# mhw32/multimodal-vae-public

Measured on AMD Instinct MI355X. Metric: images/sec (MVAE train step), higher is better.
Workload: dtype f32; 1 GPU; mnist MVAE train step, n-latents 64, batch 512 per GPU; global_batch=512, parallelism=dp1, launch=hipGraph replay

## Files before the change

### include/mvae_hip.h

```cpp
#ifndef MVAE_HIP_H
#define MVAE_HIP_H

#include <stddef.h>
#include <stdint.h>

#ifdef __cplusplus
extern "C" {
#endif

#define MVAE_OK          0
#define MVAE_ERR_ARG    (-1)
#define MVAE_ERR_LAUNCH (-2)
#define MVAE_ERR_WS     (-3)
#define MVAE_ERR_COMM   (-4)

#define MVAE_ACT_SWISH   1
#define MVAE_ACCUMULATE  2

#define MVAE_POE_VARIANT_A 0
#define MVAE_POE_VARIANT_B 1
#define MVAE_POE_NO_PRIOR  4
#define MVAE_MAX_EXPERTS  32

typedef void *mvae_stream_t;

int mvae_abi_version(void);
size_t mvae_gemm_ws_bytes(int rows_out, int cols_out, int reduce_len);
int mvae_linear_fwd(const float *x, int ldx, const float *w, const float *bias,
                    float *pre, float *act, int ldy,
                    const float *mask, float mask_scale,
                    int M, int N, int K, void *ws, size_t ws_bytes, mvae_stream_t stream);
int mvae_linear_dgrad(const float *dy, int lddy, const float *w,
                      float *dx, int lddx,
                      const float *pre_in, const float *mask, float mask_scale,
                      int M, int N, int K, int flags, void *ws, size_t ws_bytes,
                      mvae_stream_t stream);
int mvae_linear_wgrad(const float *dy, int lddy, const float *x, int ldx,
                      float *dw, float *db, int M, int N, int K, int flags,
                      void *ws, size_t ws_bytes, mvae_stream_t stream);

#define MVAE_WGRAD_BATCH_MAX 16
typedef struct {
    const float *dy; int lddy;
    const float *x; int ldx;
    float *dw;
    float *db;
    int M, N, K;
    int flags;
} mvae_wgrad_item;
int mvae_linear_wgrad_batched(const mvae_wgrad_item *items, int n_items, mvae_stream_t stream);

typedef struct {
    const float *grad_base;
    float *param_base;
    float *exp_avg_base;
    float *exp_avg_sq_base;
    const float *coef2;
    double beta1, beta2, eps;
    float grad_scale;
} mvae_adam_fuse;
int mvae_linear_wgrad_batched_adam(const mvae_wgrad_item *items, int n_items, const mvae_adam_fuse *adam,
                                   mvae_stream_t stream);

int mvae_linear_fwd_grouped(const float *x, int ldx, size_t x_gs, const float *w, size_t w_gs,
                            const float *bias, size_t bias_gs, float *pre, float *act, int ldy,
                            size_t y_gs, int G, int M, int N, int K, void *ws, size_t ws_bytes,
                            mvae_stream_t stream);
int mvae_linear_dgrad_grouped(const float *dy, int lddy, size_t dy_gs, const float *w, size_t w_gs,
                              float *dx, int lddx, size_t dx_gs, const float *pre_in, size_t pre_gs,
                              int G, int M, int N, int K, int flags, void *ws, size_t ws_bytes,
                              mvae_stream_t stream);
int mvae_linear_wgrad_grouped(const float *dy, int lddy, size_t dy_gs, const float *x, int ldx,
                              size_t x_gs, float *dw, size_t dw_gs, float *db, size_t db_gs, int G,
                              int M, int N, int K, int flags, void *ws, size_t ws_bytes,
                              mvae_stream_t stream);

int mvae_conv2d_k4_fwd(const float *x, const float *w, float *pre, float *act,
                       int B, int Cin, int H, int W, int Cout, int stride, int pad,
                       mvae_stream_t stream);
int mvae_conv2d_k4_dgrad(const float *dy, const float *w, float *dx, const float *pre_in,
                         int B, int Cin, int H, int W, int Cout, int stride, int pad,
                         void *ws, size_t ws_bytes, mvae_stream_t stream);
int mvae_conv2d_k4_wgrad(const float *dy, const float *x, float *dw,
                         int B, int Cin, int H, int W, int Cout, int stride, int pad,
                         int flags, void *ws, size_t ws_bytes, mvae_stream_t stream);
int mvae_convT2d_k4_fwd(const float *x, const float *w, float *pre, float *act,
                        int B, int Cin, int H, int W, int Cout, int stride, int pad,
                        void *ws, size_t ws_bytes, mvae_stream_t stream);
int mvae_convT2d_k4_dgrad(const float *dy, const float *w, float *dx, const float *pre_in,
                          int B, int Cin, int H, int W, int Cout, int stride, int pad,
                          mvae_stream_t stream);
int mvae_convT2d_k4_wgrad(const float *dy, const float *x, float *dw,
                          int B, int Cin, int H, int W, int Cout, int stride, int pad,
                          int flags, void *ws, size_t ws_bytes, mvae_stream_t stream);

typedef struct {
    const float *w; float *wr;
    int transposed, Cin, Cout, stride, pad;
} mvae_repack_item;
size_t mvae_conv_k4_repack_floats(int transposed, const float *w, int B, int Cin, int H, int W, int Cout,
                                  int stride, int pad);
int mvae_conv_k4_repack_batched(const mvae_repack_item *items, int n_items, mvae_stream_t stream);

#define MVAE_STATS_TILE_ELEMS 512
size_t mvae_convT2d_k4_stats_tiles(int B, int Cin, int H, int W, int Cout, int stride, int pad);
int mvae_convT2d_k4_fwd_stats(const float *x, const float *w, float *part, size_t part_floats,
                              int B, int Cin, int H, int W, int Cout, int stride, int pad,
                              void *ws, size_t ws_bytes, mvae_stream_t stream);

size_t mvae_bn_ws_bytes(int G, int C, int n_per_group);
int mvae_bn_train_fwd(const float *x, const float *gamma, const float *beta, float *y,
                      float *save_mean, float *save_invstd,
                      float *running_mean, float *running_var,
                      int G, int B, int C, int HW, float eps, float momentum,
                      int n_updates, const int *n_updates_dev ,
                      int flags, void *ws, size_t ws_bytes, mvae_stream_t stream);
int mvae_bn_train_bwd(const float *dy, const float *x, const float *gamma, const float *beta,
                      const float *save_mean, const float *save_invstd,
                      float *dx, float *dgamma, float *dbeta,
                      int G, int B, int C, int HW, int flags,
                      void *ws, size_t ws_bytes, mvae_stream_t stream);
int mvae_bn_stats_merge(const float *part, int tiles, int elems_per_tile, int G, int C,
                        float *save_mean, float *save_invstd, float *running_mean, float *running_var,
                        float eps, float momentum, int n_updates, const int *n_updates_dev, mvae_stream_t stream);
int mvae_bn_eval_fwd(const float *x, const float *gamma, const float *beta, float *y,
                     const float *running_mean, const float *running_var,
                     int N, int C, int HW, float eps, int flags, mvae_stream_t stream);

int mvae_swish_fwd(const float *x, float *y, size_t n, mvae_stream_t stream);
int mvae_swish_bwd(const float *dy, const float *x, float *dx, size_t n, mvae_stream_t stream);
int mvae_sigmoid_fwd(const float *x, float *y, size_t n, mvae_stream_t stream);
int mvae_affine_fwd(const float *x, const float *scale, const float *shift, float *y, size_t n, size_t period,
                    mvae_stream_t stream);
int mvae_embedding_swish_fwd(const void *idx, int idx_is_float, const float *w, float *act,
                             int R, int n_classes, int width, mvae_stream_t stream);
int mvae_embedding_swish_bwd(const void *idx, int idx_is_float, const float *w,
                             const float *dact, float *dw,
                             int R, int n_classes, int width, int flags, mvae_stream_t stream);
int mvae_embedding_swish_fwd_grouped(const void *idx, int idx_is_float, size_t idx_gs, const float *w,
                                     size_t w_gs, float *act, size_t act_gs, int G, int R,
                                     int n_classes, int width, mvae_stream_t stream);
int mvae_embedding_swish_bwd_grouped(const void *idx, int idx_is_float, size_t idx_gs, const float *w,
                                     size_t w_gs, const float *dact, size_t dact_gs, float *dw, int G,
                                     int R, int n_classes, int width, int flags, mvae_stream_t stream);

typedef struct {
    const float *mu[MVAE_MAX_EXPERTS];
    const float *logvar[MVAE_MAX_EXPERTS];
} mvae_experts_t;
typedef struct {
    float *dmu[MVAE_MAX_EXPERTS];
    float *dlogvar[MVAE_MAX_EXPERTS];
} mvae_expert_grads_t;

int mvae_poe_fwd(const mvae_experts_t *experts, int ld, int E,
                 const uint32_t *masks_dev, int T,
                 const float *noise, float *mu, float *logvar, float *z, float *kl,
                 int B, int D, int variant, mvae_stream_t stream);
int mvae_poe_fwd_draw(const mvae_experts_t *experts, int ld, int E,
                      const uint32_t *masks_dev, int T,
                      float *noise_out, uint64_t seed, const uint64_t *counter_dev, uint64_t counter_offset,
                      float *mu, float *logvar, float *z, float *kl,
                      int B, int D, int variant, mvae_stream_t stream);
int mvae_poe_bwd(const mvae_experts_t *experts, int ld, int E,
                 const uint32_t *masks_dev, int T,
                 const float *noise, const float *mu, const float *logvar,
                 const float *dz, const float *dmu, const float *dlogvar,
                 const float *dkl, int dkl_per_term ,
                 const mvae_expert_grads_t *grads, int ldg,
                 int B, int D, int variant, mvae_stream_t stream);

int mvae_poe_bwd_split(const mvae_experts_t *experts, int ld, int E,
                       const uint32_t *masks_dev, int T,
                       const float *noise, const float *mu, const float *logvar,
                       const float *dz_a, const int *slot_a, const float *dz_b, const int *slot_b,
                       const float *dkl, int dkl_per_term,
                       const mvae_expert_grads_t *grads, int ldg,
                       int B, int D, int variant, mvae_stream_t stream);

int mvae_reparam_fwd(const float *mu, const float *logvar, const float *eps, float *z, size_t n,
                     mvae_stream_t stream);
int mvae_reparam_bwd(const float *dz, const float *logvar, const float *eps,
                     float *dmu, float *dlogvar, size_t n, mvae_stream_t stream);

int mvae_kl_rows_fwd(const float *mu, const float *logvar, float *kl, int B, int D,
                     mvae_stream_t stream);
int mvae_kl_rows_bwd(const float *mu, const float *logvar, const float *dkl,
                     float *dmu, float *dlogvar, int B, int D, mvae_stream_t stream);

int mvae_bce_rowsum_fwd(const float *logits, const float *target, const float *colw,
                        float *rowsum, const float *drow_dev, float *dlogits ,
                        int R, int P, int rows_per_group, int target_rows,
                        int target_div, int target_row_stride, int target_col_stride,
                        mvae_stream_t stream);
int mvae_bce_rowsum_bwd(const float *logits, const float *target, const float *colw,
                        const float *drow_dev, float *dlogits,
                        int R, int P, int rows_per_group, int target_rows,
                        int target_div, int target_row_stride, int target_col_stride,
                        mvae_stream_t stream);
int mvae_ce_fwd(const float *logits, const int64_t *label, float *row,
                const float *drow_dev, float *dlogits ,
                int R, int K, int rows_per_group, int label_rows, mvae_stream_t stream);
int mvae_ce_bwd(const float *logits, const int64_t *label, const float *drow_dev,
                float *dlogits, int R, int K, int rows_per_group, int label_rows,
                mvae_stream_t stream);
int mvae_linear_bce_fwd(const float *x, int ldx, const float *w, const float *bias, const float *target,
                        int target_rows, int target_row_stride, const float *drow_dev, int rows_per_group,
                        float *dlogits, int ldy, float *logits, float *partial, int M, int N, int K,
                        mvae_stream_t stream);
int mvae_linear_ce_fwd(const float *x, int ldx, const float *w, const float *bias, const int64_t *label,
                       int label_rows, const float *drow_dev, int rows_per_group, float *dlogits, int ldy,
                       float *logits, float *row, int M, int N, int K, mvae_stream_t stream);
#define MVAE_ELBO_MAX_PARTS 4
#define MVAE_ELBO_MAX_TERMS 40
typedef struct {
    const float *rows;
    const float *coef;
    const int *term_of;
    int first_term, groups, rows_per_group;
} mvae_elbo_part;
int mvae_elbo_reduce(const mvae_elbo_part *parts, int n_parts, float *elbo, int T, float *zero, size_t zero_n,
                     uint64_t *counter_dev, uint64_t counter_inc, mvae_stream_t stream);
int mvae_group_sums(const float *rows, const float *coef_dev, float *out, float *total_out,
                    int G, int rows_per_group, int flags, mvae_stream_t stream);

int mvae_randn(float *out, size_t n, uint64_t seed, uint64_t *counter_dev, mvae_stream_t stream);
int mvae_bernoulli(float *out, size_t n, float keep_prob, uint64_t seed, uint64_t *counter_dev,
                   mvae_stream_t stream);
int mvae_philox_fill(float *out, size_t n, int bernoulli, float keep_prob, uint64_t seed,
                     const uint64_t *counter_dev, uint64_t counter_offset, mvae_stream_t stream);
int mvae_adam_step(float *param, const float *grad, float *exp_avg, float *exp_avg_sq,
                   size_t n, double lr, double beta1, double beta2, double eps, float grad_scale,
                   int64_t *step_dev, mvae_stream_t stream);
int mvae_adam_apply(float *param, const float *grad, float *exp_avg, float *exp_avg_sq,
                    size_t n, double lr, double beta1, double beta2, double eps, float grad_scale,
                    const int64_t *step_dev, mvae_stream_t stream);
int mvae_adam_apply_at(float *param, const float *grad, float *exp_avg, float *exp_avg_sq,
                       size_t n, double lr, double beta1, double beta2, double eps, float grad_scale,
                       const int64_t *step_dev, int64_t step_add, mvae_stream_t stream);
int mvae_adam_prepare(int64_t *step_dev, int64_t delta, double lr, double beta1, double beta2, float *coef2,
                      mvae_stream_t stream);
int mvae_counter_add(int64_t *counter_dev, int64_t delta, mvae_stream_t stream);
int mvae_adam_apply_coef(float *param, const float *grad, float *exp_avg, float *exp_avg_sq, size_t n,
                         const float *coef2, double beta1, double beta2, double eps, float grad_scale,
                         mvae_stream_t stream);

int mvae_trace_marker(int tag, mvae_stream_t stream);
int mvae_fill(float *out, size_t n, float value, mvae_stream_t stream);
int mvae_ingest(const float *image_src, float *image_dst, size_t image_floats,
                const void *label_src, void *label_dst, size_t label_bytes,
                const void *table_src_host, void *table_dst, size_t table_bytes, mvae_stream_t stream);

int mvae_block_gather(const float *src, const int *idx_dev, float *dst, int n_dst, size_t block_elems,
                      mvae_stream_t stream);
int mvae_block_scatter_add(const float *src, const int *idx_dev, float *dst, int n_src, int n_dst,
                           size_t block_elems, mvae_stream_t stream);
int mvae_scatter_sums(const float *vals, const float *coef_dev, const int *idx_dev, float *out,
                      float *total_out, int n, int flags, mvae_stream_t stream);

int mvae_dropout_fanout_fwd(const float *h, const float *masks, float *out, float scale,
                            int G, int B, int N, mvae_stream_t stream);
int mvae_dropout_fanin_bwd(const float *dout, const float *masks, float *dh, float scale,
                           int G, int B, int N, mvae_stream_t stream);
int mvae_bce_elem_fwd(const float *logits, const float *target, float *out, size_t n,
                      mvae_stream_t stream);
int mvae_bce_elem_bwd(const float *logits, const float *target, const float *g,
                      float *dlogits, float *dtarget, size_t n, mvae_stream_t stream);

int mvae_resample_ksize(int in_size, int out_size);
int mvae_resample_coeffs(int in_size, int out_size, int *kk_host, int *bounds_host);
int mvae_resize_crop_u8_to_f32(const uint8_t *src, float *dst, int B, int H, int W, int out_h,
                               int out_w, int S, int crop_top, int crop_left, const int *kx_dev,
                               const int *bx_dev, int ksx, const int *ky_dev, const int *by_dev,
                               int ksy, int y0, int y1, mvae_stream_t stream);
int mvae_u8_to_f32(const uint8_t *src, float *dst, size_t n, mvae_stream_t stream);

int mvae_gru_cell_fwd(const float *gi, int ldgi, const float *gh, int ldgh, const float *h_prev, int ldh,
                      float *h_new, int ldo, float *gates , int B, int H, mvae_stream_t stream);
int mvae_gru_cell_bwd(const float *dh_new, int lddh, const float *dh_extra , int ldde,
                      const float *gates, const float *h_prev, int ldh, float *dgi, float *dgh, float *dh_prev,
                      int B, int H, mvae_stream_t stream);
int mvae_embedding_fwd(const int64_t *idx, int idx_stride, const float *w, float *out, int ldo, int R,
                       int n_classes, int width, int flags, mvae_stream_t stream);
int mvae_embedding_bwd(const int64_t *idx, int idx_stride, const float *w, const float *dout, int ldd, float *dw,
                       int R, int n_classes, int width, int flags, mvae_stream_t stream);
int mvae_copy2d(const float *src, int lds, float *dst, int ldd, const float *mask , int ldm,
                float scale, int rows, int cols, int flags, mvae_stream_t stream);
int mvae_argmax_rows(const float *x, int ldx, int64_t *out, int R, int K, mvae_stream_t stream);

#define MVAE_COMM_ID_BYTES 128
typedef struct mvae_comm mvae_comm_t;
int mvae_comm_use_library(const char *librccl_path);
int mvae_comm_rccl_version(void);
int mvae_comm_unique_id(void *id_out, size_t id_bytes);
int mvae_comm_init(mvae_comm_t **comm, const void *id, size_t id_bytes, int rank, int world, int device);
int mvae_comm_rank(const mvae_comm_t *comm);
int mvae_comm_world(const mvae_comm_t *comm);
const char *mvae_comm_last_error(const mvae_comm_t *comm);
int mvae_comm_broadcast(mvae_comm_t *comm, void *buf, size_t bytes, int root, mvae_stream_t stream);
int mvae_comm_allreduce_async(mvae_comm_t *comm, float *buf, size_t count, mvae_stream_t stream, int *ticket);
int mvae_comm_wait(mvae_comm_t *comm, int ticket , mvae_stream_t stream);
int mvae_comm_async_error(mvae_comm_t *comm);
int mvae_comm_synchronize(mvae_comm_t *comm, mvae_stream_t stream, int timeout_ms);
int mvae_comm_destroy(mvae_comm_t *comm);

#ifdef MVAE_TUNING
void mvae_debug_set_tiling(int wm, int wn, int splits);
void mvae_debug_set_kwaves(int kw);
void mvae_debug_set_small(int off, int waves);
void mvae_debug_set_split_target(long blocks);
void mvae_debug_set_knockout(int mode);
#endif

#ifdef __cplusplus
}
#endif
#endif
```

### multimodal-vae-public_amd/_lib.py

```python
import ctypes
import os
from ctypes import c_double, c_float, c_int, c_size_t, c_uint64, c_void_p

_HERE = os.path.dirname(os.path.abspath(__file__))
LIB_PATH = os.path.join(_HERE, 'libmvae_hip.so')

MVAE_OK = 0
ERRORS = {-1: 'MVAE_ERR_ARG (bad shape / null pointer / unsupported stride)',
          -2: 'MVAE_ERR_LAUNCH (hip kernel launch failed)',
          -3: 'MVAE_ERR_WS (workspace too small)',
          -4: 'MVAE_ERR_COMM (RCCL not loadable, or an RCCL / HIP runtime call of mvae_comm_* failed)'}
COMM_ID_BYTES = 128
ACT_SWISH = 1
ACCUMULATE = 2
POE_NO_PRIOR = 4
POE_VARIANT = {'A': 0, 'B': 1, 'A-noprior': 0 | POE_NO_PRIOR, 'B-noprior': 1 | POE_NO_PRIOR}
MAX_EXPERTS = 32
STATS_TILE_ELEMS = 512
MAX_TERMS = 40


class Experts(ctypes.Structure):
    _fields_ = [('mu', c_void_p * MAX_EXPERTS), ('logvar', c_void_p * MAX_EXPERTS)]


class ElboPart(ctypes.Structure):
    _fields_ = [('rows', c_void_p), ('coef', c_void_p), ('term_of', c_void_p), ('first_term', c_int),
                ('groups', c_int), ('rows_per_group', c_int)]


ELBO_MAX_PARTS = 4


class WgradItem(ctypes.Structure):
    _fields_ = [('dy', c_void_p), ('lddy', c_int), ('x', c_void_p), ('ldx', c_int), ('dw', c_void_p),
                ('db', c_void_p), ('M', c_int), ('N', c_int), ('K', c_int), ('flags', c_int)]


WGRAD_BATCH_MAX = 16


class AdamFuse(ctypes.Structure):
    _fields_ = [('grad_base', c_void_p), ('param_base', c_void_p), ('exp_avg_base', c_void_p),
                ('exp_avg_sq_base', c_void_p), ('coef2', c_void_p), ('beta1', ctypes.c_double),
                ('beta2', ctypes.c_double), ('eps', ctypes.c_double), ('grad_scale', ctypes.c_float)]


class RepackItem(ctypes.Structure):
    _fields_ = [('w', c_void_p), ('wr', c_void_p), ('transposed', c_int), ('Cin', c_int), ('Cout', c_int),
                ('stride', c_int), ('pad', c_int)]


REPACK_MAX = 16


class ExpertGrads(ctypes.Structure):
    _fields_ = [('dmu', c_void_p * MAX_EXPERTS), ('dlogvar', c_void_p * MAX_EXPERTS)]


P = c_void_p
_SIGNATURES = {
    'mvae_abi_version': (c_int, []),
    'mvae_gemm_ws_bytes': (c_size_t, [c_int, c_int, c_int]),
    'mvae_linear_fwd': (c_int, [P, c_int, P, P, P, P, c_int, P, c_float, c_int, c_int, c_int, P, c_size_t, P]),
    'mvae_linear_bce_fwd': (c_int, [P, c_int, P, P, P, c_int, c_int, P, c_int, P, c_int, P, P, c_int, c_int, c_int, P]),
    'mvae_linear_ce_fwd': (c_int, [P, c_int, P, P, P, c_int, P, c_int, P, c_int, P, P, c_int, c_int, c_int, P]),
    'mvae_linear_dgrad': (c_int, [P, c_int, P, P, c_int, P, P, c_float, c_int, c_int, c_int, c_int, P, c_size_t, P]),
    'mvae_linear_wgrad': (c_int, [P, c_int, P, c_int, P, P, c_int, c_int, c_int, c_int, P, c_size_t, P]),
    'mvae_linear_fwd_grouped': (c_int, [P, c_int, c_size_t, P, c_size_t, P, c_size_t, P, P, c_int, c_size_t,
                                        c_int, c_int, c_int, c_int, P, c_size_t, P]),
    'mvae_linear_dgrad_grouped': (c_int, [P, c_int, c_size_t, P, c_size_t, P, c_int, c_size_t, P, c_size_t,
                                          c_int, c_int, c_int, c_int, c_int, P, c_size_t, P]),
    'mvae_linear_wgrad_grouped': (c_int, [P, c_int, c_size_t, P, c_int, c_size_t, P, c_size_t, P, c_size_t,
                                          c_int, c_int, c_int, c_int, c_int, P, c_size_t, P]),
    'mvae_conv2d_k4_fwd': (c_int, [P, P, P, P] + [c_int] * 7 + [P]),
    'mvae_conv2d_k4_dgrad': (c_int, [P, P, P, P] + [c_int] * 7 + [P, c_size_t, P]),
    'mvae_conv2d_k4_wgrad': (c_int, [P, P, P] + [c_int] * 8 + [P, c_size_t, P]),
    'mvae_convT2d_k4_fwd': (c_int, [P, P, P, P] + [c_int] * 7 + [P, c_size_t, P]),
    'mvae_convT2d_k4_dgrad': (c_int, [P, P, P, P] + [c_int] * 7 + [P]),
    'mvae_convT2d_k4_wgrad': (c_int, [P, P, P] + [c_int] * 8 + [P, c_size_t, P]),
    'mvae_bn_ws_bytes': (c_size_t, [c_int, c_int, c_int]),
    'mvae_bn_train_fwd': (c_int, [P] * 8 + [c_int] * 4 + [c_float, c_float, c_int, P, c_int, P, c_size_t, P]),
    'mvae_bn_train_bwd': (c_int, [P] * 9 + [c_int] * 5 + [P, c_size_t, P]),
    'mvae_bn_eval_fwd': (c_int, [P] * 6 + [c_int] * 3 + [c_float, c_int, P]),
    'mvae_swish_fwd': (c_int, [P, P, c_size_t, P]),
    'mvae_swish_bwd': (c_int, [P, P, P, c_size_t, P]),
    'mvae_sigmoid_fwd': (c_int, [P, P, c_size_t, P]),
    'mvae_affine_fwd': (c_int, [P, P, P, P, c_size_t, c_size_t, P]),
    'mvae_embedding_swish_fwd': (c_int, [P, c_int, P, P, c_int, c_int, c_int, P]),
    'mvae_embedding_swish_bwd': (c_int, [P, c_int, P, P, P, c_int, c_int, c_int, c_int, P]),
    'mvae_embedding_swish_fwd_grouped': (c_int, [P, c_int, c_size_t, P, c_size_t, P, c_size_t, c_int, c_int, c_int,
                                                 c_int, P]),
    'mvae_embedding_swish_bwd_grouped': (c_int, [P, c_int, c_size_t, P, c_size_t, P, c_size_t, P, c_int, c_int,
                                                 c_int, c_int, c_int, P]),
    'mvae_resample_ksize': (c_int, [c_int, c_int]),
    'mvae_resample_coeffs': (c_int, [c_int, c_int, P, P]),
    'mvae_resize_crop_u8_to_f32': (c_int, [P, P] + [c_int] * 8 + [P, P, c_int, P, P, c_int, c_int, c_int, P]),
    'mvae_u8_to_f32': (c_int, [P, P, c_size_t, P]),
    'mvae_poe_fwd': (c_int, [ctypes.POINTER(Experts), c_int, c_int, P, c_int, P, P, P, P, P,
                             c_int, c_int, c_int, P]),
    'mvae_poe_fwd_draw': (c_int, [ctypes.POINTER(Experts), c_int, c_int, P, c_int, P, c_uint64, P, c_uint64, P, P, P, P,
                                  c_int, c_int, c_int, P]),
    'mvae_poe_bwd': (c_int, [ctypes.POINTER(Experts), c_int, c_int, P, c_int, P, P, P, P, P, P, P, c_int,
                             ctypes.POINTER(ExpertGrads), c_int, c_int, c_int, c_int, P]),
    'mvae_poe_bwd_split': (c_int, [ctypes.POINTER(Experts), c_int, c_int, P, c_int, P, P, P, P,
                                   ctypes.POINTER(c_int), P, ctypes.POINTER(c_int), P, c_int,
                                   ctypes.POINTER(ExpertGrads), c_int, c_int, c_int, c_int, P]),
    'mvae_kl_rows_fwd': (c_int, [P, P, P, c_int, c_int, P]),
    'mvae_kl_rows_bwd': (c_int, [P, P, P, P, P, c_int, c_int, P]),
    'mvae_bce_rowsum_fwd': (c_int, [P, P, P, P, P, P] + [c_int] * 7 + [P]),
    'mvae_bce_rowsum_bwd': (c_int, [P, P, P, P, P] + [c_int] * 7 + [P]),
    'mvae_ce_fwd': (c_int, [P, P, P, P, P, c_int, c_int, c_int, c_int, P]),
    'mvae_ce_bwd': (c_int, [P, P, P, P, c_int, c_int, c_int, c_int, P]),
    'mvae_group_sums': (c_int, [P, P, P, P, c_int, c_int, c_int, P]),
    'mvae_conv_k4_repack_floats': (c_size_t, [c_int, P, c_int, c_int, c_int, c_int, c_int, c_int, c_int]),
    'mvae_conv_k4_repack_batched': (c_int, [ctypes.POINTER(RepackItem), c_int, P]),
    'mvae_convT2d_k4_stats_tiles': (c_size_t, [c_int] * 7),
    'mvae_convT2d_k4_fwd_stats': (c_int, [P, P, P, c_size_t] + [c_int] * 7 + [P, c_size_t, P]),
    'mvae_bn_stats_merge': (c_int, [P, c_int, c_int, c_int, c_int, P, P, P, P, c_float, c_float, c_int, P, P]),
    'mvae_linear_wgrad_batched': (c_int, [ctypes.POINTER(WgradItem), c_int, P]),
    'mvae_linear_wgrad_batched_adam': (c_int, [ctypes.POINTER(WgradItem), c_int, ctypes.POINTER(AdamFuse), P]),
    'mvae_adam_prepare': (c_int, [P, ctypes.c_int64, c_double, c_double, c_double, P, P]),
    'mvae_elbo_reduce': (c_int, [ctypes.POINTER(ElboPart), c_int, P, c_int, P, c_size_t, P, c_uint64, P]),
    'mvae_philox_fill': (c_int, [P, c_size_t, c_int, c_float, c_uint64, P, c_uint64, P]),
    'mvae_randn': (c_int, [P, c_size_t, c_uint64, P, P]),
    'mvae_bernoulli': (c_int, [P, c_size_t, c_float, c_uint64, P, P]),
    'mvae_adam_step': (c_int, [P, P, P, P, c_size_t, c_double, c_double, c_double, c_double, c_float, P, P]),
    'mvae_adam_apply': (c_int, [P, P, P, P, c_size_t, c_double, c_double, c_double, c_double, c_float, P, P]),
    'mvae_adam_apply_at': (c_int, [P, P, P, P, c_size_t, c_double, c_double, c_double, c_double, c_float, P,
                                   ctypes.c_int64, P]),
    'mvae_adam_apply_coef': (c_int, [P, P, P, P, c_size_t, P, c_double, c_double, c_double, c_float, P]),
    'mvae_counter_add': (c_int, [P, ctypes.c_int64, P]),
    'mvae_trace_marker': (c_int, [c_int, P]),
    'mvae_fill': (c_int, [P, c_size_t, c_float, P]),
    'mvae_ingest': (c_int, [P, P, c_size_t, P, P, c_size_t, P, P, c_size_t, P]),
    'mvae_reparam_fwd': (c_int, [P, P, P, P, c_size_t, P]),
    'mvae_reparam_bwd': (c_int, [P, P, P, P, P, c_size_t, P]),
    'mvae_dropout_fanout_fwd': (c_int, [P, P, P, c_float, c_int, c_int, c_int, P]),
    'mvae_dropout_fanin_bwd': (c_int, [P, P, P, c_float, c_int, c_int, c_int, P]),
    'mvae_block_gather': (c_int, [P, P, P, c_int, c_size_t, P]),
    'mvae_block_scatter_add': (c_int, [P, P, P, c_int, c_int, c_size_t, P]),
    'mvae_scatter_sums': (c_int, [P, P, P, P, P, c_int, c_int, P]),
    'mvae_bce_elem_fwd': (c_int, [P, P, P, c_size_t, P]),
    'mvae_bce_elem_bwd': (c_int, [P, P, P, P, P, c_size_t, P]),
    'mvae_gru_cell_fwd': (c_int, [P, c_int, P, c_int, P, c_int, P, c_int, P, c_int, c_int, P]),
    'mvae_gru_cell_bwd': (c_int, [P, c_int, P, c_int, P, P, c_int, P, P, P, c_int, c_int, P]),
    'mvae_embedding_fwd': (c_int, [P, c_int, P, P, c_int, c_int, c_int, c_int, c_int, P]),
    'mvae_embedding_bwd': (c_int, [P, c_int, P, P, c_int, P, c_int, c_int, c_int, c_int, P]),
    'mvae_copy2d': (c_int, [P, c_int, P, c_int, P, c_int, c_float, c_int, c_int, c_int, P]),
    'mvae_argmax_rows': (c_int, [P, c_int, P, c_int, c_int, P]),
    'mvae_comm_use_library': (c_int, [ctypes.c_char_p]),
    'mvae_comm_rccl_version': (c_int, []),
    'mvae_comm_unique_id': (c_int, [P, c_size_t]),
    'mvae_comm_init': (c_int, [ctypes.POINTER(P), P, c_size_t, c_int, c_int, c_int]),
    'mvae_comm_rank': (c_int, [P]),
    'mvae_comm_world': (c_int, [P]),
    'mvae_comm_last_error': (ctypes.c_char_p, [P]),
    'mvae_comm_broadcast': (c_int, [P, P, c_size_t, c_int, P]),
    'mvae_comm_allreduce_async': (c_int, [P, P, c_size_t, P, ctypes.POINTER(c_int)]),
    'mvae_comm_wait': (c_int, [P, c_int, P]),
    'mvae_comm_async_error': (c_int, [P]),
    'mvae_comm_synchronize': (c_int, [P, P, c_int]),
    'mvae_comm_destroy': (c_int, [P]),
}

_TUNING_SIGNATURES = {
    'mvae_debug_set_tiling': (None, [c_int, c_int, c_int]),
    'mvae_debug_set_kwaves': (None, [c_int]),
    'mvae_debug_set_small': (None, [c_int, c_int]),
    'mvae_debug_set_split_target': (None, [ctypes.c_long]),
    'mvae_debug_set_knockout': (None, [c_int]),
}
TUNING_LIB_PATH = os.path.join(_HERE, 'libmvae_hip_tuning.so')

_lib = None


def exported_symbols():
    return sorted(_SIGNATURES)


def lib():
    global _lib
    if _lib is None:
        path = os.environ.get('MVAE_HIP_LIB') or LIB_PATH
        if not os.path.exists(path):
            raise RuntimeError(
                'libmvae_hip.so is not built (%s missing): run `make -C %s/csrc`; there is no '
                'CPU fallback for the MVAE HIP path.' % (path, _HERE))
        handle = ctypes.CDLL(path)
        for name, (res, args) in _SIGNATURES.items():
            fn = getattr(handle, name)
            fn.restype = res
            fn.argtypes = args
        for name, (res, args) in _TUNING_SIGNATURES.items():
            fn = getattr(handle, name, None)
            if fn is not None:
                fn.restype = res
                fn.argtypes = args
        if handle.mvae_abi_version() != 6:
            raise RuntimeError('libmvae_hip.so ABI version mismatch')
        _lib = handle
    return _lib


def check(rc, what):
    if rc != MVAE_OK:
        raise RuntimeError('%s failed: %s' % (what, ERRORS.get(rc, 'error %d' % rc)))
```

### multimodal-vae-public_amd/csrc/poe.hip

```cpp
#include "common.h"
#include "philox.h"

namespace {

constexpr int POE_THREADS = 128;
constexpr int POE_MAX_TERMS = 40;
constexpr float POE_EPS = 1e-8f;

struct PoeArgs {
    mvae_experts_t ex;
    int ld, E, T, B, D, variant;
    int no_prior;
    int chunk;
    uint64_t seed; const uint64_t *counter; uint64_t counter_offset; int draw;
};

__device__ __forceinline__ float poe_precision(float lv, int variant) {
    float var = expf(lv) + POE_EPS;
    if (variant == MVAE_POE_VARIANT_A) var = var + POE_EPS;
    return 1.0f / var;
}

__global__ __launch_bounds__(POE_THREADS) void poe_fwd_kernel(PoeArgs a, const uint32_t *masks,
                                                              float *noise, float *mu, float *logvar,
                                                              float *z, float *kl) {
    extern __shared__ float lds[];
    const int lane = threadIdx.x & 63;
    const int b = blockIdx.x * (POE_THREADS / 64) + (threadIdx.x >> 6);
    if (b >= a.B) return;
    float *mine = lds + threadIdx.x;
    float *klacc = lds + (size_t)a.E * 2 * POE_THREADS + threadIdx.x;
    const float t0 = a.no_prior ? 0.f : poe_precision(0.f, a.variant);
    const int t_lo = blockIdx.y * a.chunk, t_hi = min(a.T, t_lo + a.chunk);
    uint32_t used = 0;
    for (int t = t_lo; t < t_hi; ++t) { klacc[(t - t_lo) * POE_THREADS] = 0.f; used |= masks[t]; }
    const uint64_t launch = a.draw ? *a.counter + a.counter_offset : 0;
    for (int d = lane; d < a.D; d += 64) {
        const size_t oe = (size_t)b * a.ld + d;
        for (int e = 0; e < a.E; ++e) {
            if (!((used >> e) & 1u)) continue;
            const float te = poe_precision(a.ex.logvar[e][oe], a.variant);
            mine[(e * 2 + 0) * POE_THREADS] = te;
            mine[(e * 2 + 1) * POE_THREADS] = a.ex.mu[e][oe] * te;
        }
        for (int t = t_lo; t < t_hi; ++t) {
            uint32_t mask = masks[t];
            float sum_t = t0, sum_mt = 0.f * t0;
            for (int e = 0; mask; ++e, mask >>= 1) {
                if (!(mask & 1u)) continue;
                sum_mt += mine[(e * 2 + 1) * POE_THREADS];
                sum_t += mine[(e * 2 + 0) * POE_THREADS];
            }
            const float pmu = sum_mt / sum_t;
            const float pvar = 1.0f / sum_t;
            const float plv = (a.variant == MVAE_POE_VARIANT_A) ? logf(pvar + POE_EPS) : logf(pvar);
            const size_t o = ((size_t)t * a.B + b) * a.D + d;
            mu[o] = pmu;
            logvar[o] = plv;
            if (a.draw) {
                const float eps = philox_normal_at(o, launch, a.seed);
                noise[o] = eps;
                z[o] = eps * expf(0.5f * plv) + pmu;
            } else if (z) {
                z[o] = noise ? noise[o] * expf(0.5f * plv) + pmu : pmu;
            }
            klacc[(t - t_lo) * POE_THREADS] += 1.0f + plv - pmu * pmu - expf(plv);
        }
    }
    if (kl) {
        for (int t = t_lo; t < t_hi; ++t) {
            const float s = wave_sum(klacc[(t - t_lo) * POE_THREADS]);
            if (lane == 0) kl[(size_t)t * a.B + b] = -0.5f * s;
        }
    }
}

struct PoeDzMap { signed char slot_a[MVAE_ELBO_MAX_TERMS], slot_b[MVAE_ELBO_MAX_TERMS]; };

__global__ __launch_bounds__(POE_THREADS) void poe_bwd_kernel(PoeArgs a, const uint32_t *masks,
                                                              const float *noise, const float *mu,
                                                              const float *logvar, const float *dz,
                                                              const float *dz_b, PoeDzMap dzm,
                                                              const float *dmu, const float *dlogvar,
                                                              const float *dkl, int dkl_stride,
                                                              mvae_expert_grads_t gr, int ldg) {
    extern __shared__ float lds[];
    const int lane = threadIdx.x & 63;
    const int b = blockIdx.x * (POE_THREADS / 64) + (threadIdx.x >> 6);
    if (b >= a.B) return;
    float *mine = lds + threadIdx.x;
    const int e_lo = blockIdx.y * a.chunk, e_hi = min(a.E, e_lo + a.chunk);
    const uint32_t own = (e_hi - e_lo >= 32 ? 0xffffffffu : ((1u << (e_hi - e_lo)) - 1u)) << e_lo;
    for (int d = lane; d < a.D; d += 64) {
        for (int t = 0; t < a.T; ++t) {
            if (!(masks[t] & own)) continue;
            const size_t o = ((size_t)t * a.B + b) * a.D + d;
            const float pmu = mu[o], plv = logvar[o];
            float gmu = dmu ? dmu[o] : 0.f;
            float glv = dlogvar ? dlogvar[o] : 0.f;
            if (dz) {
                float g;
                if (dz_b) {
                    const int sa = dzm.slot_a[t], sb = dzm.slot_b[t];
                    g = sa >= 0 ? dz[((size_t)sa * a.B + b) * a.D + d] : 0.f;
                    if (sb >= 0) g += dz_b[((size_t)sb * a.B + b) * a.D + d];
                } else {
                    g = dz[o];
                }
                gmu += g;
                if (noise) glv += g * noise[o] * 0.5f * expf(0.5f * plv);
            }
            if (dkl) {
                const float ks = dkl_stride ? dkl[(size_t)t * dkl_stride + b] : dkl[t];
                gmu += ks * pmu;
                glv += ks * (-0.5f) * (1.0f - expf(plv));
            }
            float s, dlv_ds;
            if (a.variant == MVAE_POE_VARIANT_A) {
                const float v = expf(plv) - POE_EPS;
                s = 1.0f / v;
                dlv_ds = -(v * v) / (v + POE_EPS);
            } else {
                s = expf(-plv);
                dlv_ds = -1.0f / s;
            }
            mine[(t * 3 + 0) * POE_THREADS] = gmu / s;
            mine[(t * 3 + 1) * POE_THREADS] = glv * dlv_ds;
            mine[(t * 3 + 2) * POE_THREADS] = pmu;
        }
        for (int e = e_lo; e < e_hi; ++e) {
            const size_t o = (size_t)b * a.ld + d;
            const float me = a.ex.mu[e][o], lve = a.ex.logvar[e][o];
            const float ex = expf(lve);
            const float te = poe_precision(lve, a.variant);
            float gm = 0.f, gt = 0.f;
            bool any = false;
            for (int t = 0; t < a.T; ++t) {
                if (!((masks[t] >> e) & 1u)) continue;
                any = true;
                const float at = mine[(t * 3 + 0) * POE_THREADS];
                gm += at * te;
                gt += at * (me - mine[(t * 3 + 2) * POE_THREADS]) + mine[(t * 3 + 1) * POE_THREADS];
            }
            const size_t og = (size_t)b * ldg + d;
            gr.dmu[e][og] = any ? gm : 0.f;
            gr.dlogvar[e][og] = any ? gt * (-(te * te) * ex) : 0.f;
        }
    }
}

__global__ __launch_bounds__(POE_THREADS) void kl_rows_fwd_kernel(const float *mu, const float *logvar, float *kl,
                                                                  int B, int D) {
    const int lane = threadIdx.x & 63;
    const int b = blockIdx.x * (POE_THREADS / 64) + (threadIdx.x >> 6);
    if (b >= B) return;
    float s = 0.f;
    for (int d = lane; d < D; d += 64) {
        const float m = mu[(size_t)b * D + d], lv = logvar[(size_t)b * D + d];
        s += 1.0f + lv - m * m - expf(lv);
    }
    s = wave_sum(s);
    if (lane == 0) kl[b] = -0.5f * s;
}

__global__ __launch_bounds__(256) void kl_rows_bwd_kernel(const float *mu, const float *logvar, const float *dkl,
                                                          float *dmu, float *dlogvar, int B, int D) {
    const size_t n = (size_t)B * D;
    for (size_t i = (size_t)blockIdx.x * 256 + threadIdx.x; i < n; i += (size_t)gridDim.x * 256) {
        const float g = dkl[i / D];
        dmu[i] = g * mu[i];
        dlogvar[i] = g * (-0.5f) * (1.0f - expf(logvar[i]));
    }
}

#ifndef MVAE_POE_CHUNK
#define MVAE_POE_CHUNK 3
#endif
#ifndef MVAE_POE_CHUNK_SMALL
#define MVAE_POE_CHUNK_SMALL 1
#endif
inline int poe_chunk(int n) {
    if (n <= 0) return 1;
    if (n <= 4) return MVAE_POE_CHUNK_SMALL > 0 ? MVAE_POE_CHUNK_SMALL : n;
    return MVAE_POE_CHUNK <= 0 ? n : MVAE_POE_CHUNK;
}

inline bool poe_args_ok(const mvae_experts_t *ex, int ld, int E, int T, int B, int D, int variant) {
    if (!ex || E < 0 || E > MVAE_MAX_EXPERTS || T <= 0 || T > POE_MAX_TERMS || B <= 0 || D <= 0 || ld < D)
        return false;
    const int base = variant & ~MVAE_POE_NO_PRIOR;
    if (base != MVAE_POE_VARIANT_A && base != MVAE_POE_VARIANT_B) return false;
    if ((variant & MVAE_POE_NO_PRIOR) && E < 1) return false;
    for (int e = 0; e < E; ++e)
        if (!ex->mu[e] || !ex->logvar[e]) return false;
    return true;
}

}

MVAE_EXPORT int mvae_poe_fwd(const mvae_experts_t *experts, int ld, int E, const uint32_t *masks_dev, int T,
                             const float *noise, float *mu, float *logvar, float *z, float *kl, int B, int D,
                             int variant, mvae_stream_t stream) {
    if (!poe_args_ok(experts, ld, E, T, B, D, variant) || !masks_dev || !mu || !logvar) return MVAE_ERR_ARG;
    PoeArgs a;
    a.ex = *experts; a.ld = ld; a.E = E; a.T = T; a.B = B; a.D = D;
    a.variant = variant & ~MVAE_POE_NO_PRIOR; a.no_prior = (variant & MVAE_POE_NO_PRIOR) ? 1 : 0;
    a.seed = 0; a.counter = nullptr; a.counter_offset = 0; a.draw = 0;
    const int rows = POE_THREADS / 64;
    a.chunk = poe_chunk(T);
    const size_t lds_bytes = ((size_t)E * 2 + a.chunk) * POE_THREADS * sizeof(float);
    hipLaunchKernelGGL(poe_fwd_kernel, dim3((B + rows - 1) / rows, (T + a.chunk - 1) / a.chunk), dim3(POE_THREADS), lds_bytes, (hipStream_t)stream, a,
                       masks_dev, const_cast<float *>(noise), mu, logvar, z, kl);
    return mvae_launch_status();
}

MVAE_EXPORT int mvae_poe_fwd_draw(const mvae_experts_t *experts, int ld, int E, const uint32_t *masks_dev, int T,
                                  float *noise_out, uint64_t seed, const uint64_t *counter_dev,
                                  uint64_t counter_offset, float *mu, float *logvar, float *z, float *kl, int B,
                                  int D, int variant, mvae_stream_t stream) {
    if (!poe_args_ok(experts, ld, E, T, B, D, variant) || !masks_dev || !mu || !logvar || !z || !noise_out ||
        !counter_dev)
        return MVAE_ERR_ARG;
    PoeArgs a;
    a.ex = *experts; a.ld = ld; a.E = E; a.T = T; a.B = B; a.D = D;
    a.variant = variant & ~MVAE_POE_NO_PRIOR; a.no_prior = (variant & MVAE_POE_NO_PRIOR) ? 1 : 0;
    a.seed = seed; a.counter = counter_dev; a.counter_offset = counter_offset; a.draw = 1;
    const int rows = POE_THREADS / 64;
    a.chunk = poe_chunk(T);
    const size_t lds_bytes = ((size_t)E * 2 + a.chunk) * POE_THREADS * sizeof(float);
    hipLaunchKernelGGL(poe_fwd_kernel, dim3((B + rows - 1) / rows, (T + a.chunk - 1) / a.chunk), dim3(POE_THREADS), lds_bytes, (hipStream_t)stream, a,
                       masks_dev, noise_out, mu, logvar, z, kl);
    return mvae_launch_status();
}

MVAE_EXPORT int mvae_poe_bwd(const mvae_experts_t *experts, int ld, int E, const uint32_t *masks_dev, int T,
                             const float *noise, const float *mu, const float *logvar, const float *dz,
                             const float *dmu, const float *dlogvar, const float *dkl, int dkl_per_term,
                             const mvae_expert_grads_t *grads, int ldg, int B, int D, int variant,
                             mvae_stream_t stream) {
    const int dkl_stride = dkl_per_term ? 0 : B;
    if (!poe_args_ok(experts, ld, E, T, B, D, variant) || !masks_dev || !mu || !logvar || !grads || ldg < D)
        return MVAE_ERR_ARG;
    for (int e = 0; e < E; ++e)
        if (!grads->dmu[e] || !grads->dlogvar[e]) return MVAE_ERR_ARG;
    PoeArgs a;
    a.ex = *experts; a.ld = ld; a.E = E; a.T = T; a.B = B; a.D = D;
    a.variant = variant & ~MVAE_POE_NO_PRIOR; a.no_prior = (variant & MVAE_POE_NO_PRIOR) ? 1 : 0;
    a.seed = 0; a.counter = nullptr; a.counter_offset = 0; a.draw = 0;
    const int rows = POE_THREADS / 64;
    const size_t lds_bytes = (size_t)T * 3 * POE_THREADS * sizeof(float);
    PoeDzMap none = {};
    a.chunk = poe_chunk(E);
    hipLaunchKernelGGL(poe_bwd_kernel, dim3((B + rows - 1) / rows, E ? (E + a.chunk - 1) / a.chunk : 1), dim3(POE_THREADS), lds_bytes,
                       (hipStream_t)stream, a, masks_dev, noise, mu, logvar, dz, (const float *)nullptr, none, dmu,
                       dlogvar, dkl, dkl_stride, *grads, ldg);
    return mvae_launch_status();
}

MVAE_EXPORT int mvae_poe_bwd_split(const mvae_experts_t *experts, int ld, int E, const uint32_t *masks_dev, int T,
                                   const float *noise, const float *mu, const float *logvar, const float *dz_a,
                                   const int *slot_a, const float *dz_b, const int *slot_b, const float *dkl,
                                   int dkl_per_term, const mvae_expert_grads_t *grads, int ldg, int B, int D,
                                   int variant, mvae_stream_t stream) {
    const int dkl_stride = dkl_per_term ? 0 : B;
    if (!poe_args_ok(experts, ld, E, T, B, D, variant) || !masks_dev || !mu || !logvar || !grads || ldg < D ||
        !dz_a || !dz_b || !slot_a || !slot_b || T > MVAE_ELBO_MAX_TERMS)
        return MVAE_ERR_ARG;
    for (int e = 0; e < E; ++e)
        if (!grads->dmu[e] || !grads->dlogvar[e]) return MVAE_ERR_ARG;
    PoeDzMap m;
    for (int t = 0; t < T; ++t) {
        if (slot_a[t] < -1 || slot_a[t] >= T || slot_b[t] < -1 || slot_b[t] >= T) return MVAE_ERR_ARG;
        m.slot_a[t] = (signed char)slot_a[t]; m.slot_b[t] = (signed char)slot_b[t];
    }
    PoeArgs a;
    a.ex = *experts; a.ld = ld; a.E = E; a.T = T; a.B = B; a.D = D;
    a.variant = variant & ~MVAE_POE_NO_PRIOR; a.no_prior = (variant & MVAE_POE_NO_PRIOR) ? 1 : 0;
    a.seed = 0; a.counter = nullptr; a.counter_offset = 0; a.draw = 0;
    const int rows = POE_THREADS / 64;
    const size_t lds_bytes = (size_t)T * 3 * POE_THREADS * sizeof(float);
    a.chunk = poe_chunk(E);
    hipLaunchKernelGGL(poe_bwd_kernel, dim3((B + rows - 1) / rows, E ? (E + a.chunk - 1) / a.chunk : 1), dim3(POE_THREADS), lds_bytes,
                       (hipStream_t)stream, a, masks_dev, noise, mu, logvar, dz_a, dz_b, m, (const float *)nullptr,
                       (const float *)nullptr, dkl, dkl_stride, *grads, ldg);
    return mvae_launch_status();
}

MVAE_EXPORT int mvae_kl_rows_fwd(const float *mu, const float *logvar, float *kl, int B, int D,
                                 mvae_stream_t stream) {
    if (!mu || !logvar || !kl || B <= 0 || D <= 0) return MVAE_ERR_ARG;
    const int rows = POE_THREADS / 64;
    hipLaunchKernelGGL(kl_rows_fwd_kernel, dim3((B + rows - 1) / rows), dim3(POE_THREADS), 0, (hipStream_t)stream,
                       mu, logvar, kl, B, D);
    return mvae_launch_status();
}

MVAE_EXPORT int mvae_kl_rows_bwd(const float *mu, const float *logvar, const float *dkl, float *dmu,
                                 float *dlogvar, int B, int D, mvae_stream_t stream) {
    if (!mu || !logvar || !dkl || !dmu || !dlogvar || B <= 0 || D <= 0) return MVAE_ERR_ARG;
    size_t blocks = ((size_t)B * D + 255) / 256;
    if (blocks > 4096) blocks = 4096;
    hipLaunchKernelGGL(kl_rows_bwd_kernel, dim3((int)blocks), dim3(256), 0, (hipStream_t)stream, mu, logvar, dkl,
                       dmu, dlogvar, B, D);
    return mvae_launch_status();
}
```

### multimodal-vae-public_amd/engine.py

```python
import contextlib
import os

import torch

from . import kernels as K
from . import layers as L

KEEP = 0.9


def _snapshot(model, optimizer, counter):
    bufs = [b.clone() for b in model.buffers()]
    pend = [(m, m._nbt_pending) for m in model.modules() if isinstance(m, L._BatchNormMixin)]
    opt = None
    if getattr(optimizer, '_arena', None) is not None:
        opt = (optimizer._m.clone(), optimizer._v.clone(), optimizer._step_dev.clone(), optimizer._host_step)
    return (model.arena.flat.clone(), bufs, pend, opt, counter.clone())


def _restore(model, optimizer, counter, snap):
    flat, bufs, pend, opt, ctr = snap
    model.arena.flat.copy_(flat)
    for b, s in zip(model.buffers(), bufs):
        b.copy_(s)
    for m, n in pend:
        m._nbt_pending = n
    counter.copy_(ctr)
    if getattr(optimizer, '_arena', None) is not None:
        if opt is None:
            optimizer._m.zero_(); optimizer._v.zero_(); optimizer._step_dev.zero_()
            optimizer._host_step = 0
        else:
            optimizer._m.copy_(opt[0]); optimizer._v.copy_(opt[1]); optimizer._step_dev.copy_(opt[2])
            optimizer._host_step = opt[3]


class StepTables(object):

    def __init__(self, n_words, device, slots=4):
        import numpy as np
        self.dev = torch.zeros(n_words, dtype=torch.int32, device=device)
        self._host, self._np, self._events = [], [], []
        for _ in range(slots):
            h = torch.zeros(n_words, dtype=torch.int32)
            if torch.cuda.is_available():
                h = h.pin_memory()
            self._host.append(h)
            self._np.append(h.numpy())
            self._events.append(None)
        self._i = 0
        self.defer = False
        self._pending = False
        self._np_float = [a.view(np.float32) for a in self._np]

    def ints(self, lo, n):
        return self.dev[lo:lo + n]

    def floats(self, lo, n):
        return self.dev[lo:lo + n].view(torch.float32)

    def begin(self):
        k = self._i % len(self._host)
        if self._events[k] is not None:
            self._events[k].synchronize()
        return self._np[k], self._np_float[k]

    def commit(self):
        if self.defer:
            self._pending = True
            return
        k = self._i % len(self._host)
        self.dev.copy_(self._host[k], non_blocking=True)
        self._mark(k)

    def _mark(self, k):
        if torch.cuda.is_available():
            if self._events[k] is None:
                self._events[k] = torch.cuda.Event()
            self._events[k].record()
        self._i += 1
        self._pending = False

    def pending_slot(self):
        return self._host[self._i % len(self._host)] if self._pending else None

    def sent(self):
        self._mark(self._i % len(self._host))


class _StepBase(object):

    def _init_common(self, model, batch_size, seed):
        model.finalize()
        self.model = model
        self.B = int(batch_size)
        self.D = model.n_latents
        self.dev = next(model.parameters()).device
        self.seed = int(seed) or 1
        self.counter = torch.zeros(1, dtype=torch.int64, device=self.dev)
        self.on_bucket_ready = None
        self.n_buckets = 2
        self._graphs = None
        self._comm = None
        self._bucket0_done = False
        n_streams = os.environ.get('MVAE_STREAMS', 'auto')
        wg_batched_auto = False
        if n_streams == 'auto':
            mods = list(model.modules())
            has_conv = any(isinstance(m, (L.Conv2d, L.ConvTranspose2d)) for m in mods)
            has_bn = any(isinstance(m, L._BatchNormMixin) for m in mods)
            n_streams = 4 if (has_conv and not has_bn and os.environ.get('MVAE_FUSE_ADAM', '0') != '1') else 2
            if n_streams == 2 and os.environ.get('MVAE_FUSE_ADAM', '0') != '1' and os.environ.get('MVAE_PAIR_ENC', '0') != '1':
                n_streams, wg_batched_auto = 3, True
        self._streams_auto = os.environ.get('MVAE_STREAMS', 'auto') == 'auto' and int(n_streams) > 2
        n_streams = int(n_streams)
        self.side = torch.cuda.Stream(device=self.dev) if n_streams >= 2 else None
        self.batch_wgrad = os.environ.get('MVAE_BATCH_WGRAD', '1') != '0'
        self.poe_draw = os.environ.get('MVAE_POE_DRAW', '1') != '0'
        self.wgrad_on_side = os.environ.get('MVAE_WGRAD_SIDE', '1') != '0' and self.side is not None
        self.use_ingest = os.environ.get('MVAE_INGEST', '1') != '0'
        self.main_first = os.environ.get('MVAE_MAIN_FIRST', '1') != '0'
        self.main_first_dec = os.environ.get('MVAE_MAIN_FIRST_DEC', '1')
        fold = os.environ.get('MVAE_LOSS_FOLD', '1')
        self.fold_image = fold in ('1', 'image')
        self.fold_label = fold in ('1', 'label')
        self.dp_side_launch = os.environ.get('MVAE_DP_SIDE_LAUNCH', '1') != '0'
        self._bucket1_done = False
        self._draw_in_poe = False
        self.batch_repack = os.environ.get('MVAE_BATCH_REPACK', '1') != '0'
        self._conv_mods = [m for m in model.modules() if isinstance(m, (L.Conv2d, L.ConvTranspose2d))]
        self.wg_main = torch.cuda.Stream(device=self.dev) if n_streams >= 3 else None
        self.wg_batched = os.environ.get('MVAE_WG_BATCHED', '1' if wg_batched_auto else '0') == '1'
        self.wg_side = torch.cuda.Stream(device=self.dev) if n_streams >= 4 else self.wg_main
        self._wg_pending = []
        self._forked = False
        self.fuse_adam = False
        self._fusion = None

    @contextlib.contextmanager
    def _branch(self, after=None):
        if self.side is None:
            yield
            return
        if after is None:
            self.side.wait_stream(torch.cuda.current_stream(self.dev))
        else:
            self.side.wait_event(after)
        self._forked = True
        with torch.cuda.stream(self.side):
            yield

    def _fork_point(self):
        if self.side is None or not self.main_first:
            return None
        ev = torch.cuda.Event()
        ev.record()
        self._carry.setdefault('fork_events', []).append(ev)
        return ev

    def _deferred(self):
        if self.wg_main is not None and not self.wg_batched:
            return []
        return L.WgradBatch(adam=self._fusion) if self.batch_wgrad else None

    def _launch_deferred(self, fns, stream):
        if isinstance(fns, L.WgradBatch) and not (self.wg_batched and stream is not None and len(fns)
                                                 and self._comm is None and self.on_bucket_ready is None):
            fns.flush()
            return
        if not fns:
            return
        stream.wait_stream(torch.cuda.current_stream(self.dev))
        with torch.cuda.stream(stream):
            if isinstance(fns, L.WgradBatch):
                fns.flush()
            else:
                for fn in fns:
                    fn()
        self._carry.setdefault('deferred', []).append(fns)
        if stream not in self._wg_pending:
            self._wg_pending.append(stream)

    def _join_wgrad(self):
        main = torch.cuda.current_stream(self.dev)
        for s in self._wg_pending:
            main.wait_stream(s)
        self._wg_pending = []

    def _join(self):
        if self._forked:
            main = torch.cuda.current_stream(self.dev)
            main.wait_stream(self.side)
            self._forked = False

    def configure_buckets(self, n):
        if n not in (1, 2, 3):
            raise ValueError('1, 2 or 3 gradient buckets')
        if n == 3 and self.model.arena.tail_range is None:
            raise ValueError('three buckets need an arena tail')
        self.n_buckets = n

    def _phases_b(self):
        if self.n_buckets == 3:
            return [lambda: self._phase_b('upper'), lambda: self._phase_b('lower')]
        return [lambda: self._phase_b('all')]

    def forward_backward(self, image, label):
        self._step_begin()
        try:
            self._phase_a(image, label)
            if self.on_bucket_ready is not None and self.n_buckets > 1:
                self.on_bucket_ready(0)
            for k, part in enumerate(self._phases_b()):
                part()
                if self.on_bucket_ready is not None:
                    self.on_bucket_ready(k + 1 if self.n_buckets > 1 else 0)
        finally:
            self._step_end()
        return self.elbo

    def _step_begin(self):
        if self.batch_repack:
            L.repack_weights(self._conv_mods)

    def _step_end(self):
        if self.batch_repack:
            L.repack_done(self._conv_mods)

    def step(self, image, label, annealing_factor, noise=None):
        self.model.zero_grad(set_to_none=True)
        self.set_coefficients(annealing_factor)
        if noise is not None:
            self.set_noise(noise)
        else:
            self.draw_noise()
        return self.forward_backward(image, label)

    def capture(self, optimizer, image_shape, label_example, warmup=3, comm=None):
        if comm is not None and getattr(self, '_streams_auto', False) and self.wg_main is not None:
            self.wg_main = self.wg_side = None

        dev = self.dev
        self.static_image = torch.zeros((self.B,) + tuple(image_shape), dtype=torch.float32, device=dev)
        self.static_label = torch.zeros_like(label_example, device=dev)
        self.set_coefficients(1.0)
        self._comm = comm
        hook, self.on_bucket_ready = self.on_bucket_ready, None
        snap = _snapshot(self.model, optimizer, self.counter)
        side = torch.cuda.Stream(device=dev)
        side.wait_stream(torch.cuda.current_stream())
        bns = [m for m in self.model.modules() if isinstance(m, L._BatchNormMixin)]
        in_graph = comm is not None and getattr(comm, 'in_graph', False)
        with torch.cuda.stream(side):
            for it in range(warmup):
                before = [m._nbt_pending for m in bns]
                if in_graph:
                    self._dp_step(optimizer)
                else:
                    self._single_gpu_step(optimizer)
                self._bn_inc = [(m, m._nbt_pending - b) for m, b in zip(bns, before)]
        torch.cuda.current_stream().wait_stream(side)
        torch.cuda.synchronize(dev)
        if comm is None:
            g = torch.cuda.CUDAGraph()
            with torch.cuda.graph(g):
                self._single_gpu_step(optimizer)
            self._graphs = (g,)
        elif in_graph:
            g = torch.cuda.CUDAGraph()
            with torch.cuda.graph(g):
                self._dp_step(optimizer)
            self._graphs = (g,)
            self._optimizer = optimizer
        else:
            pool = torch.cuda.graph_pool_handle()
            graphs = [torch.cuda.CUDAGraph()]
            try:
                with torch.cuda.graph(graphs[0], pool=pool):
                    self._body_a()
                for part in self._phases_b():
                    g = torch.cuda.CUDAGraph()
                    with torch.cuda.graph(g, pool=pool):
                        part()
                    graphs.append(g)
            finally:
                self._step_end()
            self._graphs = tuple(graphs)
            self._optimizer = optimizer
        _restore(self.model, optimizer, self.counter, snap)
        torch.cuda.synchronize(dev)
        self.on_bucket_ready = hook
        return self._graphs

    def _single_gpu_step(self, optimizer):
        early = (os.environ.get('MVAE_EARLY_COUNTER', '1') != '0' and self.side is not None
                 and hasattr(optimizer, 'step_counted'))
        self._adam_counter = optimizer.step_counter() if early else None
        self._optimizer_early = optimizer if early else None
        fuse = (early and self.fuse_adam and self.batch_wgrad and self.wg_main is None
                and hasattr(optimizer, 'fusion') and optimizer.grad_scale == 1.0)
        self._fusion = optimizer.fusion() if fuse else None
        if self._fusion is not None:
            self._fusion.begin()
            self._adam_prepare = lambda: optimizer.prepare_counted(self._fusion)
        self._adam_split = None
        if (early and self._fusion is None and os.environ.get('MVAE_SPLIT_ADAM', '0') == '1'
                and hasattr(optimizer, 'step_counted_range') and getattr(self, 'supports_split_adam', False)):
            from .parallel import bucket_ranges
            ranges = bucket_ranges(self.model, self.model.arena)
            if len(ranges) >= 2:
                self._adam_split = (optimizer, ranges[0][1], self.model.arena.numel)
        try:
            self._body_a()
            self._phase_b('all')
            if self._adam_split is not None and self._carry.get('adam_dec_done'):
                optimizer.step_counted_range(self._adam_split[1], self._adam_split[2], last=True)
            elif early:
                optimizer.step_counted(self._fusion) if self._fusion is not None else optimizer.step_counted()
            else:
                optimizer.step()
        finally:
            self._step_end()
            self._adam_counter = None
            self._fusion = None
            self._adam_split = None

    def _dp_step(self, optimizer):
        comm = self._comm
        self._adam_counter = None
        self._bucket0_done = self._bucket1_done = False
        if hasattr(comm, 'reset'):
            comm.reset()
        try:
            self._body_a()
            if self.n_buckets > 1 and not self._bucket0_done:
                comm.launch(0)
            for k, part in enumerate(self._phases_b()):
                part()
                bucket = k + 1 if self.n_buckets > 1 else 0
                if not (bucket == 1 and self._bucket1_done):
                    comm.launch(bucket)
        finally:
            self._step_end()
        self._join()
        comm.finish(optimizer)

    def _poe_forward(self, mus, lvs, mu, lv, z, kl):
        if self._draw_in_poe:
            K.poe_fwd_draw(mus, lvs, self.masks_dev, self.noise, self.seed, self.counter, 0, mu, lv, z, kl,
                           self.model.POE_VARIANT)
        else:
            K.poe_fwd(mus, lvs, self.masks_dev, self.noise, mu, lv, z, kl, self.model.POE_VARIANT)

    def _side_launch_ok(self):
        return (self.dp_side_launch and self.side is not None and self._comm is not None
                and getattr(self._comm, 'in_graph', False) and self.on_bucket_ready is None)

    def _upper_done(self):
        if self._side_launch_ok() and self.n_buckets == 3:
            ev = torch.cuda.Event()
            ev.record()
            with torch.cuda.stream(self.side):
                self.side.wait_event(ev)
                self._comm.launch(1)
            self._carry.setdefault('events', ())
            self._carry['events'] += (ev,)
            self._bucket1_done = True
            self._forked = True
        else:
            self._join()

    def _early_counter(self):
        if getattr(self, '_adam_counter', None) is not None:
            if self._fusion is not None:
                self._adam_prepare()
            elif hasattr(self._optimizer_early, 'prepare_plain'):
                self._optimizer_early.prepare_plain()
            else:
                K.counter_add(self._adam_counter, 1)

    def _body_a(self):
        self.model.zero_grad(set_to_none=True)
        self._step_begin()
        self.draw_noise()
        self._phase_a(self.static_image, self.static_label)

    def _bump_bn_counters(self):
        for m, inc in self._bn_inc:
            m._nbt_pending += inc

    def replay(self, image, label, annealing_factor):
        self._bump_bn_counters()
        if self.use_ingest and K.ingest_ok(image, self.static_image, label, self.static_label):
            self.tables.defer = True
            try:
                self.set_coefficients(annealing_factor)
            finally:
                self.tables.defer = False
            slot = self.tables.pending_slot()
            K.ingest(image, self.static_image, label, self.static_label, slot, self.tables.dev)
            self.tables.sent()
        else:
            self.static_image.copy_(image, non_blocking=True)
            self.static_label.copy_(label, non_blocking=True)
            self.set_coefficients(annealing_factor)
        if self._comm is None or getattr(self._comm, 'in_graph', False):
            self._graphs[0].replay()
        else:
            for k, g in enumerate(self._graphs):
                g.replay()
                if self.n_buckets > 1:
                    self._comm.launch(k)
                elif k == len(self._graphs) - 1:
                    self._comm.launch(0)
            self._comm.finish(self._optimizer)
        return self.elbo


class BimodalStep(_StepBase):
    supports_split_adam = True
    """Fused step for ``mnist`` / ``fashionmnist`` / ``celeba`` MVAEs."""

    def __init__(self, model, batch_size, lambda_image=1.0, lambda_label=1.0, seed=0):
        self._init_common(model, batch_size, seed)
        self.lambda_image = float(lambda_image)
        self.lambda_label = float(lambda_label)
        self.has_dropout = L.n_dropout(model.image_encoder.plan()) > 0
        self.has_bn = bool(model.HAS_BN)
        B, dev = self.B, self.dev
        if self.has_dropout:
            self.term_masks = [0b101, 0b010, 0b100]
            self.ref_order = [0, 1, 2]
            self.trunk = L.compile_plan(model.image_encoder.trunk_modules())
            self.head = L.compile_plan(model.image_encoder.head_modules())
        else:
            self.term_masks = [0b01, 0b11, 0b10]
            self.ref_order = [1, 0, 2]
        self.T = 3
        if self.has_bn:
            self.img_terms, self.lbl_terms = (0, 2), (0, 3)
            self.img_has_loss = [1, 1, 0]
            self.lbl_has_loss = [1, 0, 1]
        else:
            self.img_terms, self.lbl_terms = (0, 2), (1, 2)
            self.img_has_loss = [1, 1, 0]
            self.lbl_has_loss = [0, 1, 1]
        self.masks_dev = torch.tensor(self.term_masks, dtype=torch.int32, device=dev)
        self.pair_dec = self._pairable_decoder_layers() if os.environ.get('MVAE_PAIR', '0') == '1' else 0
        self.pair_enc = self._pairable_encoder_layers() if os.environ.get('MVAE_PAIR_ENC', '0') == '1' else 0
        self.split_dz = os.environ.get('MVAE_SPLIT_DZ', '1') != '0'
        self.counter_rides = os.environ.get('MVAE_COUNTER_RIDES', 'encoder')
        self.fuse_adam = (os.environ.get('MVAE_FUSE_ADAM', '0') == '1' and self.split_dz and not self.pair_dec)
        self.tables = StepTables(3 * self.T, dev)
        self.coef = self.tables.floats(0, 3 * self.T).reshape(3, self.T)
        self.noise = torch.empty(self.T, B, self.D, dtype=torch.float32, device=dev)
        self.drop_masks = torch.empty(2, B, 512, dtype=torch.float32, device=dev) if self.has_dropout else None
        self.elbo = torch.zeros(self.T + 1, dtype=torch.float32, device=dev)

    def _pairable_decoder_layers(self):
        if self.has_bn or self.img_terms[1] != self.lbl_terms[1]:
            return 0
        pi, pl = self.model.image_decoder.plan(), self.model.label_decoder.plan()
        n = 0
        for a, b in zip(pi, pl):
            if not (a.kind == 'lin' and b.kind == 'lin' and a.act and b.act and a.drop == 0 and b.drop == 0
                    and a.mod.weight.shape == b.mod.weight.shape
                    and (a.mod.bias is None) == (b.mod.bias is None)):
                break
            n += 1
        return n if n < min(len(pi), len(pl)) else 0

    def _pairable_encoder_layers(self):
        if self.has_bn or self.has_dropout or self.side is None or not self.batch_wgrad or self.wg_main is not None:
            return 0
        pi, pl = self.model.image_encoder.plan(), self.model.label_encoder.plan()
        n = 0
        while n < min(len(pi), len(pl)):
            a, b = pi[-1 - n], pl[-1 - n]
            if not (a.kind == b.kind and a.kind in ('lin', 'lin2') and a.act == b.act and a.drop == 0 and b.drop == 0):
                break
            wa, ba = L._lin_weights(a)
            wb, bb = L._lin_weights(b)
            if wa.shape != wb.shape or (ba is None) != (bb is None):
                break
            n += 1
        head_i = [op for op in pi[:len(pi) - n] if op.kind != 'view']
        head_l = pl[:len(pl) - n]
        ok = (n >= 1 and len(head_i) == 1 and head_i[0].kind == 'lin' and head_i[0].act and head_i[0].drop == 0
              and len(head_l) == 1 and head_l[0].kind == 'emb')
        return n if ok else 0

    def _pair_enc_now(self):
        return self.pair_enc and self.n_buckets != 3

    def _encoders_paired_fwd(self, image, lbl_in):
        m, B, P, dev, c = self.model, self.B, self.pair_enc, self.dev, self._carry
        pi, pl = m.image_encoder.plan(), m.label_encoder.plan()
        ni, nl = len(pi) - P, len(pl) - P
        h_l, tape_l = L.forward_tape(pl[:nl], lbl_in)
        h_i, tape_i = L.forward_tape(pi[:ni], image)
        h, layers = (h_i, h_l), []
        for j in range(P):
            wbs = [L._lin_weights(pi[ni + j]), L._lin_weights(pl[nl + j])]
            w = (wbs[0][0].detach(), wbs[1][0].detach())
            b = (None, None) if wbs[0][1] is None else (wbs[0][1].detach(), wbs[1][1].detach())
            N = w[0].shape[0]
            pre = torch.empty(2, B, N, dtype=torch.float32, device=dev)
            if pi[ni + j].act:
                act = torch.empty(2, B, N, dtype=torch.float32, device=dev)
                K.linear_fwd_pair(h, w, b, (pre[0], pre[1]), (act[0], act[1]))
                layers.append((h, pre, w))
                h = (act[0], act[1])
            else:
                K.linear_fwd_pair(h, w, b, (pre[0], pre[1]), (None, None))
                layers.append((h, None, w))
                h = (pre[0], pre[1])
        c['enc_pair'] = (layers, tape_i, tape_l, ni, nl)
        return h

    def _encoders_paired_bwd(self, g_img, g_lbl):
        m, B, P, dev, c = self.model, self.B, self.pair_enc, self.dev, self._carry
        pi, pl = m.image_encoder.plan(), m.label_encoder.plan()
        layers, tape_i, tape_l, ni, nl = c['enc_pair']
        wb = L.WgradBatch(adam=self._fusion)
        g = (g_img, g_lbl)
        keep = [g]
        first_i = [k for k, op in enumerate(pi[:ni]) if op.kind == 'lin'][0]
        for j in range(P - 1, -1, -1):
            x, _, w = layers[j]
            wb.add_linear(pi[ni + j], g[0], x[0])
            wb.add_linear(pl[nl + j], g[1], x[1])
            K_in = w[0].shape[1]
            dx = torch.empty(2, B, K_in, dtype=torch.float32, device=dev)
            if j > 0:
                pre_in = layers[j - 1][1]
                pin = (pre_in[0], pre_in[1])
            else:
                if getattr(self, '_unit_pre', None) is None or self._unit_pre.shape != (B, K_in):
                    self._unit_pre = torch.full((B, K_in), 1e4, dtype=torch.float32, device=dev)
                pin = (tape_i[first_i][1], self._unit_pre)
            K.linear_dgrad_pair(g, w, (dx[0], dx[1]), pin)
            g = (dx[0], dx[1])
            keep.append(dx)
        wb.add_linear(pi[first_i], g[0], tape_i[first_i][0])
        wb.flush()
        emb = pl[0].mod
        dw, acc = L.grad_target(emb.weight)
        K.embedding_swish_bwd(tape_l[0][0], emb.weight.detach(), g[1].contiguous(), dw, accumulate=acc)
        c['enc_pair_keep'] = (keep, wb)

    def _decoders_paired(self, z, image, label, lbl_in):
        m, B, D, P = self.model, self.B, self.D, self.pair_dec
        dev = self.dev
        (i0, ni), (l0, nl) = self.img_terms, self.lbl_terms
        R = ni * B
        plans = (m.image_decoder.plan(), m.label_decoder.plan())
        h = (z[i0:i0 + ni].reshape(R, D), z[l0:l0 + nl].reshape(R, D))
        layers = []
        for j in range(P):
            wb = [L._lin_weights(pl[j]) for pl in plans]
            w = (wb[0][0].detach(), wb[1][0].detach())
            b = (None, None) if wb[0][1] is None else (wb[0][1].detach(), wb[1][1].detach())
            N = w[0].shape[0]
            pre = torch.empty(2, R, N, dtype=torch.float32, device=dev)
            act = torch.empty(2, R, N, dtype=torch.float32, device=dev)
            K.linear_fwd_pair(h, w, b, (pre[0], pre[1]), (act[0], act[1]))
            layers.append((h, pre, w))
            h = (act[0], act[1])
        N_last = h[0].shape[1]
        gbuf = torch.empty(2, R, N_last, dtype=torch.float32, device=dev)
        with self._branch():
            logits_lbl, tape_tl = L.forward_tape(plans[1][P:], h[1], groups=nl)
            rows_lbl = torch.empty(nl * B, dtype=torch.float32, device=dev)
            dlog_lbl = torch.empty_like(logits_lbl)
            if m.LABEL_KIND == 'class':
                K.ce_fwd(logits_lbl, label, rows_lbl, drow=self.coef[1, l0:l0 + nl], dlogits=dlog_lbl,
                         rows_per_group=B, label_rows=B)
            else:
                K.bce_rowsum_fwd(logits_lbl, lbl_in, rows_lbl, drow=self.coef[1, l0:l0 + nl],
                                 dlogits=dlog_lbl, rows_per_group=B, target_rows=B)
            L.backward_tape(plans[1][P:], tape_tl, dlog_lbl, need_input_grad=True, groups=nl,
                            input_grad_out=gbuf[1], input_grad_accumulate=False)
        logits_img, tape_ti = L.forward_tape(plans[0][P:], h[0], groups=ni)
        npix = logits_img[0].numel()
        li = logits_img.reshape(ni * B, npix)
        rows_img = torch.empty(ni * B, dtype=torch.float32, device=dev)
        dlog_img = torch.empty_like(li)
        K.bce_rowsum_fwd(li, image.reshape(B, npix), rows_img, drow=self.coef[0, i0:i0 + ni], dlogits=dlog_img,
                         rows_per_group=B, target_rows=B)
        L.backward_tape(plans[0][P:], tape_ti, dlog_img.reshape(logits_img.shape), need_input_grad=True,
                        groups=ni, input_grad_out=gbuf[0], input_grad_accumulate=False)
        self._join()
        g = torch.empty_like(gbuf)
        K.swish_bwd(gbuf, layers[P - 1][1], g)
        keep = [layers, gbuf, logits_lbl, tape_tl, dlog_lbl, logits_img, tape_ti, dlog_img, g]
        for j in range(P - 1, -1, -1):
            x, _, w = layers[j]
            targets = []
            for pl in plans:
                mod = pl[j].mod
                dw, acc = L.grad_target(mod.weight)
                db, acc_b = (None, acc) if mod.bias is None else L.grad_target(mod.bias)
                if acc != acc_b:
                    raise RuntimeError('Linear weight/bias gradients out of sync')
                targets.append((dw, db, acc))
            if targets[0][2] != targets[1][2]:
                raise RuntimeError('paired gradients out of sync')
            K.linear_wgrad_pair((g[0], g[1]), x, (targets[0][0], targets[1][0]), (targets[0][1], targets[1][1]),
                                accumulate=targets[0][2])
            if j > 0:
                pre_in = layers[j - 1][1]
                dx = torch.empty(2, R, w[0].shape[1], dtype=torch.float32, device=dev)
                K.linear_dgrad_pair((g[0], g[1]), w, (dx[0], dx[1]), (pre_in[0], pre_in[1]))
                keep.append(g)
                g = dx
        keep.append(g)
        return g[0], g[1], rows_img, rows_lbl, keep

    def _fold_plan(self, plan, kind):
        op = plan[-1]
        if not (op.kind == 'lin' and not op.act and op.drop == 0):
            return False
        return kind == 'bce' or op.mod.weight.shape[0] <= 32

    def _decode_with_loss(self, plan, zin, groups, kind, target, drow, which):
        B = self.B
        N = plan[-1].mod.weight.shape[0]
        if kind == 'bce':
            nparts = K.bce_partials(N)
            rows = torch.empty(groups * B * nparts, dtype=torch.float32, device=self.dev)
            tgt = target.reshape(B, N)

            def fold(x, w, b, out, logits=None, rows=rows):
                K.linear_bce_fwd(x, w, b, tgt, drow, out, rows, B, B, logits=logits)
            rpg = B * nparts
        else:
            rows = torch.empty(groups * B, dtype=torch.float32, device=self.dev)

            def fold(x, w, b, out, logits=None, rows=rows):
                K.linear_ce_fwd(x, w, b, target, drow, out, rows, B, B, logits=logits)
            rpg = B
        dlog, tape = L.forward_tape(plan, zin, groups=groups, loss_fold=fold)
        self._carry.setdefault('folded', {})[which] = (fold, plan[-1], tape[-1][0], dlog.shape, rows.numel())
        return dlog, tape, rows, rpg

    def recon_logits(self):
        logits_lbl, _, _, logits_img, _, _ = self._carry['keep'][-1]
        out = {'image': logits_img, 'label': logits_lbl}
        for which, (fold, op, x, shape, nrows) in self._carry.get('folded', {}).items():
            w, b = L._lin_weights(op)
            lg = torch.empty(shape, dtype=torch.float32, device=self.dev)
            fold(x, w.detach(), None if b is None else b.detach(), torch.empty_like(lg), logits=lg,
                 rows=torch.empty(nrows, dtype=torch.float32, device=self.dev))
            out[which] = lg
        return out['image'], out['label']

    def set_coefficients(self, annealing_factor):
        B = float(self.B)
        _, c = self.tables.begin()
        c = c.reshape(3, self.T)
        for t in range(self.T):
            c[0, t] = self.lambda_image / B if self.img_has_loss[t] else 0.0
            c[1, t] = self.lambda_label / B if self.lbl_has_loss[t] else 0.0
            c[2, t] = float(annealing_factor) / B
        self.tables.commit()

    def set_noise(self, noise):
        self._draw_in_poe = False
        for t in range(self.T):
            self.noise[t].copy_(noise['eps'][self.ref_order[t]].to(self.dev, non_blocking=True))
        if self.has_dropout:
            self.drop_masks[0].copy_(noise['mask'][0].to(self.dev))
            self.drop_masks[1].copy_(noise['mask'][1].to(self.dev))

    def draw_noise(self):
        self._draw_in_poe = self.poe_draw
        if not self.poe_draw:
            K.philox_fill(self.noise, self.seed, self.counter, 0)
        if self.has_dropout:
            K.philox_fill(self.drop_masks, self.seed ^ 0x9E3779B97F4A7C15, self.counter, 1, keep_prob=KEEP)

    def terms_in_reference_order(self, elbo):
        idx = [self.ref_order.index(r) for r in range(self.T)] + [self.T]
        return elbo[idx]

    def _phase_a(self, image, label):
        m, B, D, T = self.model, self.B, self.D, self.T
        if image.shape[0] != B:
            raise ValueError('engine was built for batch %d, got %d' % (B, image.shape[0]))
        c = self._carry = {}
        image = image.contiguous()
        n_up = 2
        lbl_in = label if m.LABEL_KIND == 'class' else label.float().contiguous()

        def encode_label(after=None):
            with self._branch(after):
                heads, c['tape_lbl'] = L.forward_tape(m.label_encoder.plan(), lbl_in, bn_updates=n_up)
                if self.counter_rides == 'encoder' or self.pair_dec:
                    self._early_counter()
            return heads
        paired = self._pair_enc_now()
        fork = None if paired else self._fork_point()
        if paired:
            heads_img, heads_lbl = self._encoders_paired_fwd(image, lbl_in)
            img_experts = [heads_img]
        elif fork is None:
            heads_lbl = encode_label()
        if paired:
            pass
        elif self.has_dropout:
            h, c['tape_trunk'] = L.forward_tape(self.trunk, image, groups=1, bn_updates=n_up)
            hd = torch.empty(2 * B, h.shape[1], dtype=torch.float32, device=self.dev)
            K.dropout_fanout_fwd(h, self.drop_masks, hd, 1.0 / KEEP)
            heads_img, c['tape_head'] = L.forward_tape(self.head, hd)
            img_experts = [heads_img[:B], heads_img[B:]]
        else:
            heads_img, c['tape_img'] = L.forward_tape(m.image_encoder.plan(), image, bn_updates=n_up)
            img_experts = [heads_img]
        if fork is not None:
            heads_lbl = encode_label(fork)
        self._join()
        experts = img_experts + [heads_lbl]
        mus = [e[:, :D] for e in experts]
        lvs = [e[:, D:] for e in experts]
        mu = torch.empty(T, B, D, dtype=torch.float32, device=self.dev)
        lv = torch.empty_like(mu)
        z = torch.empty_like(mu)
        kl = torch.empty(T, B, dtype=torch.float32, device=self.dev)
        self._poe_forward(mus, lvs, mu, lv, z, kl)
        self.last_latents = (mu, lv, z)
        i0, ni = self.img_terms
        l0, nl = self.lbl_terms
        if self.pair_dec:
            g_img, g_lbl, rows_img, rows_lbl, keep_dec = self._decoders_paired(z, image, label, lbl_in)
            rpg_img = rpg_lbl = B
        else:
            def label_branch(after=None):
                with self._branch(after):
                    if paired or self.counter_rides == 'decoder':
                        self._early_counter()
                    zl = z[l0:l0 + nl].reshape(nl * B, D)
                    lbl_kind = 'class' if m.LABEL_KIND == 'class' else 'bce'
                    rpg_lbl = B
                    if self.fold_label and self._fold_plan(m.label_decoder.plan(), lbl_kind):
                        logits_lbl = None
                        dlog_lbl, tape_dl, rows_lbl, rpg_lbl = self._decode_with_loss(
                            m.label_decoder.plan(), zl, nl, lbl_kind, label if lbl_kind == 'class' else lbl_in,
                            self.coef[1, l0:l0 + nl], 'label')
                    else:
                        logits_lbl, tape_dl = L.forward_tape(m.label_decoder.plan(), zl, groups=nl)
                        rows_lbl = torch.empty(nl * B, dtype=torch.float32, device=self.dev)
                        dlog_lbl = torch.empty_like(logits_lbl)
                        if m.LABEL_KIND == 'class':
                            K.ce_fwd(logits_lbl, label, rows_lbl, drow=self.coef[1, l0:l0 + nl], dlogits=dlog_lbl,
                                     rows_per_group=B, label_rows=B)
                        else:
                            K.bce_rowsum_fwd(logits_lbl, lbl_in, rows_lbl, drow=self.coef[1, l0:l0 + nl],
                                             dlogits=dlog_lbl, rows_per_group=B, target_rows=B)
                    wl = self._deferred()
                    if self.split_dz:
                        dz_lbl = torch.empty(nl * B, D, dtype=torch.float32, device=self.dev)
                        L.backward_tape(m.label_decoder.plan(), tape_dl, dlog_lbl, groups=nl, need_input_grad=True,
                                        input_grad_out=dz_lbl, deferred=wl)
                        g_lbl = dz_lbl
                    else:
                        g_lbl = L.backward_tape(m.label_decoder.plan(), tape_dl, dlog_lbl, groups=nl,
                                                defer_input_grad=True, deferred=wl)
                    ev_lbl = None
                    dp_side = self._side_launch_ok() and self.n_buckets >= 2
                    if self.wgrad_on_side and self.side is not None and isinstance(wl, L.WgradBatch) \
                            and (dp_side or (self._comm is None and self.on_bucket_ready is None)):
                        ev_lbl = torch.cuda.Event()
                        ev_lbl.record()
                    self._launch_deferred(wl, self.wg_side)
                return logits_lbl, tape_dl, dlog_lbl, rows_lbl, rpg_lbl, g_lbl, ev_lbl, dp_side

            def image_branch():
                zi = z[i0:i0 + ni].reshape(ni * B, D)
                fold_img = self.fold_image and self._fold_plan(m.image_decoder.plan(), 'bce')
                rpg_img = B
                if fold_img:
                    logits_img = None
                    dlog_img, tape_di, rows_img, rpg_img = self._decode_with_loss(
                        m.image_decoder.plan(), zi, ni, 'bce', image, self.coef[0, i0:i0 + ni], 'image')
                else:
                    logits_img, tape_di = L.forward_tape(m.image_decoder.plan(), zi, groups=ni)
                if self.has_bn and ni < T:
                    L.forward_tape(m.image_decoder.plan(), z[i0 + ni:].reshape((T - ni) * B, D), groups=T - ni,
                                   stats_only=True)
                if not fold_img:
                    P = logits_img[0].numel()
                    li = logits_img.reshape(ni * B, P)
                    rows_img = torch.empty(ni * B, dtype=torch.float32, device=self.dev)
                    dlog_img = torch.empty_like(li)
                    K.bce_rowsum_fwd(li, image.reshape(B, P), rows_img, drow=self.coef[0, i0:i0 + ni], dlogits=dlog_img,
                                     rows_per_group=B, target_rows=B)
                    dlog_img = dlog_img.reshape(logits_img.shape)
                wi = self._deferred()
                if self.split_dz:
                    dz_img = torch.empty(ni * B, D, dtype=torch.float32, device=self.dev)
                    L.backward_tape(m.image_decoder.plan(), tape_di, dlog_img, groups=ni,
                                    need_input_grad=True, input_grad_out=dz_img, deferred=wi)
                    g_img = dz_img
                else:
                    g_img = L.backward_tape(m.image_decoder.plan(), tape_di, dlog_img,
                                            groups=ni, defer_input_grad=True, deferred=wi)
                return logits_img, tape_di, dlog_img, rows_img, rpg_img, g_img, wi

            dec_first = self.main_first_dec == '1' or (self.main_first_dec == 'auto' and any(
                op.kind in ('conv', 'convT') for op in m.image_decoder.plan()))
            fork = self._fork_point() if dec_first else None
            if fork is None:
                logits_lbl, tape_dl, dlog_lbl, rows_lbl, rpg_lbl, g_lbl, ev_lbl, dp_side = label_branch()
            logits_img, tape_di, dlog_img, rows_img, rpg_img, g_img, wi = image_branch()
            if fork is not None:
                logits_lbl, tape_dl, dlog_lbl, rows_lbl, rpg_lbl, g_lbl, ev_lbl, dp_side = label_branch(fork)
            if ev_lbl is not None and isinstance(wi, L.WgradBatch):
                ev_img = torch.cuda.Event()
                ev_img.record()
                c['wgrad_on_side_keep'] = list(wi)
                with torch.cuda.stream(self.side):
                    self.side.wait_event(ev_img)
                    wi.flush()
                    if getattr(self, '_adam_split', None) is not None:
                        ev_dec = torch.cuda.Event()
                        ev_dec.record()
                        c['ev_dec_grads'] = ev_dec
                    if dp_side:
                        self._comm.launch(0)
                        self._bucket0_done = True
                torch.cuda.current_stream(self.dev).wait_event(ev_lbl)
                c['events'] = (ev_lbl, ev_img)
            else:
                self._launch_deferred(wi, self.wg_main)
                self._join()
            keep_dec = (logits_lbl, tape_dl, dlog_lbl, logits_img, tape_di, dlog_img)
        elbo_parts = [(kl, self.coef[2], None, 0, T, B),
                      (rows_img, self.coef[0, i0:i0 + ni], None, i0, ni, rpg_img),
                      (rows_lbl, self.coef[1, l0:l0 + nl], None, l0, nl, rpg_lbl)]
        counter_inc = 2 if self.has_dropout else 1
        if self.split_dz and not self.pair_dec:
            dz = None
            c['dz_split'] = (g_img, [t - i0 if i0 <= t < i0 + ni else -1 for t in range(T)],
                             g_lbl, [t - l0 if l0 <= t < l0 + nl else -1 for t in range(T)])
            c['elbo_late'] = (elbo_parts, counter_inc)
        else:
            dz = torch.empty(T, B, D, dtype=torch.float32, device=self.dev)
            K.elbo_reduce(elbo_parts, self.elbo, T, zero=dz, counter_dev=self.counter, counter_inc=counter_inc)
            L.first_linear_dgrad(m.image_decoder.plan(), g_img, dz[i0:i0 + ni].reshape(ni * B, D), True)
            L.first_linear_dgrad(m.label_decoder.plan(), g_lbl, dz[l0:l0 + nl].reshape(nl * B, D), True)
        c.update(mus=mus, lvs=lvs, mu=mu, lv=lv, dz=dz, heads_img=heads_img, heads_lbl=heads_lbl,
                 keep=(z, kl, rows_lbl, g_lbl, rows_img, g_img, lbl_in, keep_dec))
        if self._comm is not None or self.on_bucket_ready is not None:
            self._join_wgrad()

    def _late_elbo(self):
        late = self._carry.pop('elbo_late', None)
        if late is not None:
            K.elbo_reduce(late[0], self.elbo, self.T, counter_dev=self.counter, counter_inc=late[1])

    def _phase_b(self, part='all'):
        m, B, D = self.model, self.B, self.D
        c = self._carry
        if part in ('all', 'upper'):
            heads_img, heads_lbl = c['heads_img'], c['heads_lbl']
            g_heads_img = torch.empty_like(heads_img)
            g_heads_lbl = torch.empty_like(heads_lbl)
            g_list = ([g_heads_img[:B], g_heads_img[B:]] if self.has_dropout else [g_heads_img]) + [g_heads_lbl]
            if c.get('dz_split') is not None:
                dza, sa, dzb, sb = c['dz_split']
                K.poe_bwd_split(c['mus'], c['lvs'], self.masks_dev, self.noise, c['mu'], c['lv'], dza, sa, dzb, sb,
                                self.coef[2], [gg[:, :D] for gg in g_list], [gg[:, D:] for gg in g_list],
                                m.POE_VARIANT, dkl_per_term=True)
            else:
                K.poe_bwd(c['mus'], c['lvs'], self.masks_dev, self.noise, c['mu'], c['lv'], c['dz'], None, None,
                          self.coef[2], [gg[:, :D] for gg in g_list], [gg[:, D:] for gg in g_list], m.POE_VARIANT,
                          dkl_per_term=True)
            c['keep_b'] = (g_heads_img, g_heads_lbl)
        if part == 'all' and 'enc_pair' in c:
            self._encoders_paired_bwd(*c['keep_b'])
            self._late_elbo()
            self._join()
            self._join_wgrad()
            return
        if part == 'all':
            wl, wi = self._deferred(), self._deferred()

            def label_encoder_backward(after=None):
                with self._branch(after):
                    L.backward_tape(m.label_encoder.plan(), c['tape_lbl'], g_heads_lbl, deferred=wl)
                    if isinstance(wl, L.WgradBatch):
                        wl.flush()
            fork = self._fork_point()
            if fork is None:
                label_encoder_backward()
            if self.has_dropout:
                d_hd = L.backward_tape(self.head, c['tape_head'], g_heads_img, need_input_grad=True, deferred=wi)
                d_h = torch.empty(B, d_hd.shape[1], dtype=torch.float32, device=self.dev)
                K.dropout_fanin_bwd(d_hd, self.drop_masks, d_h, 1.0 / KEEP)
                L.backward_tape(self.trunk, c['tape_trunk'], d_h, deferred=wi)
            else:
                L.backward_tape(m.image_encoder.plan(), c['tape_img'], g_heads_img, deferred=wi)
            if isinstance(wi, L.WgradBatch):
                if (os.environ.get('MVAE_TAIL_LANES', '1') == '1' and self.wg_batched and self.wg_main is not None
                        and self._comm is None and self.on_bucket_ready is None):
                    lane, keep, k = L.WgradBatch(adam=wi.adam), [], 0
                    for e in list(wi):
                        if not isinstance(e, tuple):
                            (lane if k % 2 else keep).append(e)
                            k += 1
                        else:
                            keep.append(e)
                    wi[:] = keep
                    self._launch_deferred(lane, self.wg_main)
                wi.flush()
                wi = None
            if fork is not None:
                label_encoder_backward(fork)
            self._late_elbo()
            if getattr(self, '_adam_split', None) is not None and c.get('ev_dec_grads') is not None:
                opt, split, _ = self._adam_split
                torch.cuda.current_stream(self.dev).wait_event(c['ev_dec_grads'])
                opt.step_counted_range(0, split)
                c['adam_dec_done'] = True
            self._join()
            if wi is not None:
                fns = wi + wl
                n = len(fns)
                self._launch_deferred(fns[:n // 3], self.wg_main)
                self._launch_deferred(fns[n // 3:2 * n // 3], self.wg_side)
                for fn in fns[2 * n // 3:]:
                    fn()
                c.setdefault('deferred', []).append(fns)
            self._join_wgrad()
            return
        plan, tape = (self.trunk, c['tape_trunk']) if self.has_dropout else (m.image_encoder.plan(), c['tape_img'])
        cut = L.tail_cut(plan, m.arena_tail())
        if part == 'upper':
            with self._branch():
                L.backward_tape(m.label_encoder.plan(), c['tape_lbl'], c['keep_b'][1])
            g = c['keep_b'][0]
            if self.has_dropout:
                d_hd = L.backward_tape(self.head, c['tape_head'], g, need_input_grad=True)
                g = torch.empty(B, d_hd.shape[1], dtype=torch.float32, device=self.dev)
                K.dropout_fanin_bwd(d_hd, self.drop_masks, g, 1.0 / KEEP)
                c['keep_b'] += (d_hd,)
            c['g_cut'] = L.backward_tape(plan[cut:], tape[cut:], g, need_input_grad=True)
            self._late_elbo()
            self._upper_done()
        else:
            L.backward_tape(plan[:cut], tape[:cut], c['g_cut'])


N_ATTRS = 18


def unrank_combination(n, k, index):
    from math import comb
    if not 0 <= index < comb(n, k):
        raise IndexError('combination index %d out of range for C(%d,%d)' % (index, n, k))
    members, first = [], 0
    for slot in range(k, 0, -1):
        while True:
            block = comb(n - first - 1, slot - 1)
            if index < block:
                break
            index -= block
            first += 1
        members.append(first)
        first += 1
    return members


def sample_subsets(rng, n_modalities=19, size=1):
    import numpy as np
    from math import comb
    n = int(n_modalities)
    if size <= 0:
        return np.zeros((0, n), dtype=bool)
    sizes = rng.choice(np.arange(2, n), size, replace=True)
    counts = np.bincount(sizes, minlength=n)
    out = []
    for k in range(n):
        if counts[k] > 0:
            for r in rng.choice(comb(n, k), size=int(counts[k]), replace=False):
                row = np.zeros(n, dtype=bool)
                row[unrank_combination(n, k, int(r))] = True
                out.append(row)
    return np.stack(out)


class Celeba19Step(_StepBase):

    def __init__(self, model, batch_size, lambda_image=1.0, lambda_attrs=1.0, approx_m=1, seed=0,
                 combo_seed=681307, faithful_bn_stats=True, rng=None):
        import numpy as np
        self._init_common(model, batch_size, seed)
        self.lambda_image, self.lambda_attrs = float(lambda_image), float(lambda_attrs)
        self.M = int(approx_m)
        self.T = 2 + N_ATTRS + self.M
        self.n_img = 2 + self.M
        self.S = self.M + 2
        if self.n_img + N_ATTRS >= 32 or self.T > 40:
            raise ValueError('approx_m too large for the PoE kernel limits (experts <= 31, terms <= 40): approx_m <= 11')
        self.faithful = bool(faithful_bn_stats)
        self.rng = rng if rng is not None else np.random.RandomState(combo_seed)
        B, D, dev, T, S = self.B, self.D, self.dev, self.T, self.S
        enc = model.image_encoder
        self.trunk = L.compile_plan(enc.trunk_modules())
        self.head = L.compile_plan(enc.head_modules())
        self.enc_plans = [e.plan() for e in model.attr_encoders]
        self.dec_plans = [d.plan() for d in model.attr_decoders]
        self.grouped = os.environ.get('MVAE_GROUPED', '1') != '0'
        if self.grouped:
            self.enc_group = L.GroupedPlans(self.enc_plans)
            self.dec_group = L.GroupedPlans(self.dec_plans)
        self.tables = tb = StepTables(T + 1 + 3 * T + N_ATTRS * S, dev)
        self._off = (0, T, T + 1, T + 1 + 3 * T)
        self.masks_dev = tb.ints(0, T)
        self.nimg_dev = tb.ints(T, 1)
        self.coef = tb.floats(T + 1, 3 * T).reshape(3, T)
        self.coef_attr = tb.floats(T + 1 + 3 * T, N_ATTRS * S)
        self._beta = 1.0
        term_of = torch.zeros(N_ATTRS, S, dtype=torch.int32)
        for i in range(N_ATTRS):
            term_of[i, 0] = 0
            for j in range(self.M):
                term_of[i, 1 + j] = 2 + N_ATTRS + j
            term_of[i, S - 1] = 2 + i
        self.term_of_slot = term_of.reshape(-1).to(dev)
        self.noise = torch.empty(T, B, D, dtype=torch.float32, device=dev)
        self.drop_masks = torch.ones(self.n_img, B, 512, dtype=torch.float32, device=dev)
        self.elbo = torch.zeros(T + 1, dtype=torch.float32, device=dev)
        self.combos = None
        first = np.zeros((self.M, 1 + N_ATTRS), dtype=bool)
        first[:, 0] = True
        first[np.arange(self.M), 1 + np.arange(self.M) % N_ATTRS] = True
        self.set_terms(first)

    def set_terms(self, combos, commit=True):
        import numpy as np
        self.combos = np.asarray(combos, dtype=bool).reshape(self.M, 1 + N_ATTRS)
        self.n_img_present = 2 + int(self.combos[:, 0].sum())
        if commit:
            self.set_coefficients(self._beta)

    def set_coefficients(self, annealing_factor):
        import numpy as np
        B, T, S, M, n_img = float(self.B), self.T, self.S, self.M, self.n_img
        combos = self.combos
        self._beta = float(annealing_factor)
        wi, wf = self.tables.begin()
        o_mask, o_nimg, o_coef, o_attr = self._off
        attr_bits = (combos[:, 1:].astype(np.int64) << (n_img + np.arange(N_ATTRS))).sum(axis=1)
        m = np.zeros(T, dtype=np.int64)
        m[0] = 1 | (((1 << N_ATTRS) - 1) << n_img)
        m[1] = 1 << 1
        m[2:2 + N_ATTRS] = 1 << (n_img + np.arange(N_ATTRS))
        m[2 + N_ATTRS:] = attr_bits + np.where(combos[:, 0], 1 << (2 + np.arange(M)), 0)
        wi[o_mask:o_mask + T] = m.astype(np.int32)
        wi[o_nimg] = self.n_img_present
        c = wf[o_coef:o_coef + 3 * T].reshape(3, T)
        c[:] = 0.0
        c[0, 0] = c[0, 1] = self.lambda_image / B
        c[0, 2 + N_ATTRS:] = np.where(combos[:, 0], 1.0 / B, 0.0)
        c[2, :] = self._beta / B
        ca = wf[o_attr:o_attr + N_ATTRS * S].reshape(N_ATTRS, S)
        ca[:, 0] = self.lambda_attrs / B
        ca[:, 1:1 + M] = np.where(combos[:, 1:].T, 1.0 / B, 0.0)
        ca[:, S - 1] = 1.0 / B
        self.tables.commit()

    def set_noise(self, noise):
        self._draw_in_poe = False
        for t in range(self.T):
            self.noise[t].copy_(noise['eps'][t].to(self.dev, non_blocking=True))
        img_terms = [0, 1] + [2 + N_ATTRS + j for j in range(self.M)]
        for k, t in enumerate(img_terms):
            mk = noise['mask'][t]
            if mk is not None:
                self.drop_masks[k].copy_(mk.to(self.dev))
            else:
                self.drop_masks[k].fill_(1.0)

    def draw_noise(self):
        self._draw_in_poe = self.poe_draw
        if not self.poe_draw:
            K.philox_fill(self.noise, self.seed, self.counter, 0)
        K.philox_fill(self.drop_masks, self.seed ^ 0x9E3779B97F4A7C15, self.counter, 1, keep_prob=KEEP)

    def step(self, image, attrs, annealing_factor, noise=None, combos=None):
        self.set_terms(combos if combos is not None else sample_subsets(self.rng, 1 + N_ATTRS, self.M), commit=False)
        return _StepBase.step(self, image, attrs, annealing_factor, noise=noise)

    def replay(self, image, attrs, annealing_factor, combos=None):
        self.set_terms(combos if combos is not None else sample_subsets(self.rng, 1 + N_ATTRS, self.M), commit=False)
        return _StepBase.replay(self, image, attrs, annealing_factor)

    def terms_in_reference_order(self, elbo):
        return elbo

    def _bump_bn_counters(self):
        trunk = set(id(op.mod) for op in self.trunk if op.kind == 'bn')
        for m, inc in self._bn_inc:
            m._nbt_pending += self.n_img_present if id(m) in trunk else inc

    def _phase_a(self, image, attrs):
        m, B, D, T, S, M, n_img = self.model, self.B, self.D, self.T, self.S, self.M, self.n_img
        dev = self.dev
        c = self._carry = {}
        image = image.contiguous()
        attrs = attrs.float().contiguous()
        heads_attr, c['tape_enc'] = [], []
        with self._branch():
            if self.grouped:
                heads_all, c['tape_enc'] = L.forward_tape_grouped(self.enc_group, attrs)
                heads_attr = [heads_all[i] for i in range(N_ATTRS)]
            else:
                for i in range(N_ATTRS):
                    ha, tp = L.forward_tape(self.enc_plans[i], attrs[:, i])
                    heads_attr.append(ha); c['tape_enc'].append(tp)
            self._early_counter()
        h, c['tape_trunk'] = L.forward_tape(self.trunk, image, bn_updates=self.n_img_present,
                                            bn_updates_dev=self.nimg_dev)
        hd = torch.empty(n_img * B, h.shape[1], dtype=torch.float32, device=dev)
        K.dropout_fanout_fwd(h, self.drop_masks, hd, 1.0 / KEEP)
        heads_img, c['tape_head'] = L.forward_tape(self.head, hd)
        self._join()
        experts = [heads_img[k * B:(k + 1) * B] for k in range(n_img)] + heads_attr
        mus = [e[:, :D] for e in experts]
        lvs = [e[:, D:] for e in experts]
        mu = torch.empty(T, B, D, dtype=torch.float32, device=dev)
        lv = torch.empty_like(mu); z = torch.empty_like(mu)
        kl = torch.empty(T, B, dtype=torch.float32, device=dev)
        self._poe_forward(mus, lvs, mu, lv, z, kl)
        self.last_latents = (mu, lv, z)
        t_s = 2 + N_ATTRS
        with self._branch():
            zcat = torch.empty(N_ATTRS, S * B, D, dtype=torch.float32, device=dev)
            K.block_gather(z, self.term_of_slot, zcat, B * D)
            logits_attr = torch.empty(N_ATTRS * S, B, dtype=torch.float32, device=dev)
            tape_dec = []
            if self.grouped:
                _, tape_dec = L.forward_tape_grouped(self.dec_group, zcat, final_out=logits_attr)
            else:
                for i in range(N_ATTRS):
                    _, tp = L.forward_tape(self.dec_plans[i], zcat[i], final_out=logits_attr[i * S:(i + 1) * S])
                    tape_dec.append(tp)
            rows_attr = torch.empty(N_ATTRS * S, dtype=torch.float32, device=dev)
            dlog_attr = torch.empty_like(logits_attr)
            K.bce_rowsum_fwd(logits_attr, attrs, rows_attr, drow=self.coef_attr, dlogits=dlog_attr,
                             rows_per_group=1, target_rows=N_ATTRS, target_div=S, target_strides=(1, N_ATTRS))
            dzcat = torch.empty_like(zcat)
            if self.grouped:
                L.backward_tape_grouped(self.dec_group, tape_dec, dlog_attr.reshape(N_ATTRS, S * B, 1),
                                        need_input_grad=True, input_grad_out=dzcat)
            else:
                for i in range(N_ATTRS):
                    L.backward_tape(self.dec_plans[i], tape_dec[i], dlog_attr[i * S:(i + 1) * S].reshape(S * B, 1),
                                    need_input_grad=True, input_grad_out=dzcat[i], input_grad_accumulate=False)
        dplan = m.image_decoder.plan()
        logit_a, tape_a = L.forward_tape(dplan, z[0:2].reshape(2 * B, D), groups=2)
        if self.faithful:
            L.forward_tape(dplan, z[2:t_s].reshape(N_ATTRS * B, D), groups=N_ATTRS, stats_only=True)
        if M > 0:
            logit_c, tape_c = L.forward_tape(dplan, z[t_s:T].reshape(M * B, D), groups=M)
        P = logit_a[0].numel()
        img_flat = image.reshape(B, P)
        rows_a = torch.empty(2 * B, dtype=torch.float32, device=dev)
        dlog_a = torch.empty(2 * B, P, dtype=torch.float32, device=dev)
        K.bce_rowsum_fwd(logit_a.reshape(2 * B, P), img_flat, rows_a, drow=self.coef[0, 0:2], dlogits=dlog_a,
                         rows_per_group=B, target_rows=B)
        rows_c = dlog_c = None
        if M > 0:
            rows_c = torch.empty(M * B, dtype=torch.float32, device=dev)
            dlog_c = torch.empty(M * B, P, dtype=torch.float32, device=dev)
            K.bce_rowsum_fwd(logit_c.reshape(M * B, P), img_flat, rows_c, drow=self.coef[0, t_s:T],
                             dlogits=dlog_c, rows_per_group=B, target_rows=B)
        dz = torch.empty(T, B, D, dtype=torch.float32, device=dev)
        K.fill_(dz, 0.0)
        L.backward_tape(dplan, tape_a, dlog_a.reshape(logit_a.shape), need_input_grad=True, groups=2,
                        input_grad_out=dz[0:2].reshape(2 * B, D), input_grad_accumulate=True)
        if M > 0:
            L.backward_tape(dplan, tape_c, dlog_c.reshape(logit_c.shape), need_input_grad=True, groups=M,
                            input_grad_out=dz[t_s:T].reshape(M * B, D), input_grad_accumulate=True)
        self._join()
        K.block_scatter_add(dzcat, self.term_of_slot, dz, T, B * D)
        parts = [(kl, self.coef[2], None, 0, T, B), (rows_a, self.coef[0, 0:2], None, 0, 2, B)]
        if M > 0:
            parts.append((rows_c, self.coef[0, t_s:T], None, t_s, M, B))
        parts.append((rows_attr, self.coef_attr, self.term_of_slot, 0, N_ATTRS * S, 1))
        K.elbo_reduce(parts, self.elbo, T, counter_dev=self.counter, counter_inc=2)
        c.update(mus=mus, lvs=lvs, mu=mu, lv=lv, dz=dz, heads_img=heads_img, heads_attr=heads_attr,
                 keep=(z, kl, zcat, logits_attr, tape_dec, rows_attr, dlog_attr, dzcat, attrs, image,
                       rows_a, rows_c, dlog_a, dlog_c))

    def _phase_b(self, part='all'):
        m, B, D, n_img = self.model, self.B, self.D, self.n_img
        c = self._carry
        if part in ('all', 'upper'):
            g_img = torch.empty_like(c['heads_img'])
            g_attr_all = torch.empty(N_ATTRS, B, 2 * D, dtype=torch.float32, device=self.dev)
            g_attr = [g_attr_all[i] for i in range(N_ATTRS)]
            g_list = [g_img[k * B:(k + 1) * B] for k in range(n_img)] + g_attr
            K.poe_bwd(c['mus'], c['lvs'], self.masks_dev, self.noise, c['mu'], c['lv'], c['dz'], None, None,
                      self.coef[2], [g[:, :D] for g in g_list], [g[:, D:] for g in g_list], m.POE_VARIANT,
                      dkl_per_term=True)
            with self._branch():
                if self.grouped:
                    L.backward_tape_grouped(self.enc_group, c['tape_enc'], g_attr_all)
                else:
                    for i in range(N_ATTRS):
                        L.backward_tape(self.enc_plans[i], c['tape_enc'][i], g_attr[i])
            d_hd = L.backward_tape(self.head, c['tape_head'], g_img, need_input_grad=True)
            d_h = torch.empty(B, d_hd.shape[1], dtype=torch.float32, device=self.dev)
            K.dropout_fanin_bwd(d_hd, self.drop_masks, d_h, 1.0 / KEEP)
            c['keep_b'] = (g_img, g_attr_all, d_hd, d_h)
            if part == 'all':
                L.backward_tape(self.trunk, c['tape_trunk'], d_h)
            else:
                cut = L.tail_cut(self.trunk, m.arena_tail())
                c['g_cut'] = L.backward_tape(self.trunk[cut:], c['tape_trunk'][cut:], d_h, need_input_grad=True)
            if part == 'upper':
                self._upper_done()
            else:
                self._join()
        else:
            cut = L.tail_cut(self.trunk, m.arena_tail())
            L.backward_tape(self.trunk[:cut], c['tape_trunk'][:cut], c['g_cut'])
```

### multimodal-vae-public_amd/kernels.py

```python
import ctypes

import torch

from . import _lib
from ._lib import ACCUMULATE, ACT_SWISH, check

_WS = {}
_WS_MIN_BYTES = 64 << 20


def _stream():
    return ctypes.c_void_p(torch.cuda.current_stream().cuda_stream)


def _ptr(t):
    return ctypes.c_void_p(t.data_ptr()) if t is not None else None


def _need_gpu(*tensors):
    for t in tensors:
        if t is not None and not t.is_cuda:
            raise RuntimeError('multimodal-vae-public_amd: the HIP path needs GPU tensors (got %s); '
                               'there is no CPU fallback' % t.device)

# ... 196 lines not shown
    if _pair_stride(pre, 'pre') != _pair_stride(act, 'act') and pre[0] is not None and act[0] is not None:
        raise RuntimeError('pre and act pairs must be laid out alike')
    ws, wsb = _ws_args(2 * _lib.lib().mvae_gemm_ws_bytes(M, N, K), x[0].device)
    check(_lib.lib().mvae_linear_fwd_grouped(_ptr(x[0]), x[0].stride(0), _pair_stride(x, 'x'), _ptr(w[0]),
                                             _pair_stride(w, 'w'), _ptr(b[0]), _pair_stride(b, 'bias'),
                                             _ptr(pre[0]), _ptr(act[0]), _rows2d(out[0], 'out').stride(0),
                                             _pair_stride(out, 'out'), 2, M, N, K, ws, wsb, _stream()),
          'mvae_linear_fwd_grouped')


def linear_dgrad_pair(dy, w, dx, pre_in=(None, None), accumulate=False):
    _need_gpu(*dy, *w, *dx, *pre_in)
    M, N = _rows2d(dy[0], 'dy').shape
    K = w[0].shape[1]
    if pre_in[0] is not None and not (pre_in[0].is_contiguous() and pre_in[0].shape == (M, K)):
        raise RuntimeError('pre_in must be contiguous [M, K]')
    ws, wsb = _ws_args(2 * _lib.lib().mvae_gemm_ws_bytes(M, K, N), dy[0].device)
    check(_lib.lib().mvae_linear_dgrad_grouped(_ptr(dy[0]), dy[0].stride(0), _pair_stride(dy, 'dy'), _ptr(w[0]),
                                               _pair_stride(w, 'w'), _ptr(dx[0]), _rows2d(dx[0], 'dx').stride(0),
                                               _pair_stride(dx, 'dx'), _ptr(pre_in[0]), _pair_stride(pre_in, 'pre_in'),
                                               2, M, N, K, ACCUMULATE if accumulate else 0, ws, wsb, _stream()),
          'mvae_linear_dgrad_grouped')


def linear_wgrad_pair(dy, x, dw, db=(None, None), accumulate=False):
    _need_gpu(*dy, *x, *dw, *db)
    M, N = _rows2d(dy[0], 'dy').shape
    K = _rows2d(x[0], 'x').shape[1]
    ws, wsb = _ws_args(2 * _lib.lib().mvae_gemm_ws_bytes(N, K, M), dy[0].device)
    check(_lib.lib().mvae_linear_wgrad_grouped(_ptr(dy[0]), dy[0].stride(0), _pair_stride(dy, 'dy'), _ptr(x[0]),
                                               x[0].stride(0), _pair_stride(x, 'x'), _ptr(dw[0]),
                                               _pair_stride(dw, 'dw'), _ptr(db[0]), _pair_stride(db, 'db'), 2, M, N, K,
                                               ACCUMULATE if accumulate else 0, ws, wsb, _stream()),
          'mvae_linear_wgrad_grouped')


def embedding_swish_fwd_grouped(idx, w0, w_gs, act):
    _need_gpu(idx, w0, act)
    if idx.dtype != torch.float32 or idx.dim() != 2 or idx.stride(1) != 1 or not act.is_contiguous():
        raise RuntimeError('grouped embedding wants a float [rows, groups] index and a contiguous output')
    R, G = idx.shape
    check(_lib.lib().mvae_embedding_swish_fwd_grouped(_ptr(idx), idx.stride(0), 1, _ptr(w0), w_gs, _ptr(act),
                                                      act.stride(0), G, R, w0.shape[0], w0.shape[1], _stream()),
          'mvae_embedding_swish_fwd_grouped')


def embedding_swish_bwd_grouped(idx, w0, w_gs, dact, dw0, accumulate=False):
    _need_gpu(idx, w0, dact, dw0)
    if idx.dtype != torch.float32 or idx.dim() != 2 or idx.stride(1) != 1 or not dact.is_contiguous():
        raise RuntimeError('grouped embedding wants a float [rows, groups] index and a contiguous gradient')
    R, G = idx.shape
    check(_lib.lib().mvae_embedding_swish_bwd_grouped(_ptr(idx), idx.stride(0), 1, _ptr(w0), w_gs, _ptr(dact),
                                                      dact.stride(0), _ptr(dw0), G, R, w0.shape[0], w0.shape[1],
                                                      ACCUMULATE if accumulate else 0, _stream()),
          'mvae_embedding_swish_bwd_grouped')


def _conv_call(name, a, b, c, d, B, Cin, H, W, Cout, stride, pad, repack=False, wr=None):
    if repack and wr is not None:
        _need_gpu(wr); _f32c(wr)
        check(getattr(_lib.lib(), name)(_ptr(a), None, _ptr(c), _ptr(d), B, Cin, H, W, Cout, stride, pad,
                                        _ptr(wr), wr.numel() * 4, _stream()), name)
    elif repack:
        ws, wsb = _ws_args(Cout * Cin * 16 * 4, a.device)
        check(getattr(_lib.lib(), name)(_ptr(a), _ptr(b), _ptr(c), _ptr(d), B, Cin, H, W, Cout, stride, pad,
                                        ws, wsb, _stream()), name)
    else:
        check(getattr(_lib.lib(), name)(_ptr(a), _ptr(b), _ptr(c), _ptr(d), B, Cin, H, W, Cout, stride, pad,
                                        _stream()), name)


def conv2d_fwd(x, w, pre, act, stride, pad):
    _need_gpu(x, w, pre, act); _f32c(x, w, pre, act)
    B, Cin, H, W = x.shape
    _conv_call('mvae_conv2d_k4_fwd', x, w, pre, act, B, Cin, H, W, w.shape[0], stride, pad)


def conv2d_dgrad(dy, w, dx, pre_in, stride, pad, wr=None):
    _need_gpu(dy, w, dx, pre_in); _f32c(dy, w, dx, pre_in)
    B, Cin, H, W = dx.shape
    _conv_call('mvae_conv2d_k4_dgrad', dy, w, dx, pre_in, B, Cin, H, W, w.shape[0], stride, pad, repack=True, wr=wr)


def conv_repack_floats(transposed, w, B, Cin, H, W, Cout, stride, pad):
    return int(_lib.lib().mvae_conv_k4_repack_floats(1 if transposed else 0, _ptr(w), B, Cin, H, W, Cout, stride, pad))


def conv_repack_batched(items):
    items = list(items)
    for lo in range(0, len(items), _lib.REPACK_MAX):
        chunk = items[lo:lo + _lib.REPACK_MAX]
        arr = (_lib.RepackItem * len(chunk))()
        for q, (w, wr, tr, Cin, Cout, s, p) in enumerate(chunk):
            _need_gpu(w, wr); _f32c(w, wr)
            if wr.numel() < Cin * Cout * 16:
                raise RuntimeError('repack buffer too small')
            arr[q] = _lib.RepackItem(_ptr(w), _ptr(wr), 1 if tr else 0, Cin, Cout, s, p)
        check(_lib.lib().mvae_conv_k4_repack_batched(arr, len(chunk), _stream()), 'mvae_conv_k4_repack_batched')


def conv2d_wgrad(dy, x, dw, stride, pad, accumulate=False):
    _need_gpu(dy, x, dw); _f32c(dy, x, dw)
    B, Cin, H, W = x.shape
    Cout = dw.shape[0]
    nbytes = _lib.lib().mvae_gemm_ws_bytes(Cout, Cin * 16, B * dy.shape[2] * dy.shape[3])
    ws, wsb = _ws_args(nbytes, dy.device)
    check(_lib.lib().mvae_conv2d_k4_wgrad(_ptr(dy), _ptr(x), _ptr(dw), B, Cin, H, W, Cout, stride, pad,
                                          ACCUMULATE if accumulate else 0, ws, wsb, _stream()),
          'mvae_conv2d_k4_wgrad')


def convT2d_fwd(x, w, pre, act, stride, pad, wr=None):
    _need_gpu(x, w, pre, act); _f32c(x, w, pre, act)
    B, Cin, H, W = x.shape
    _conv_call('mvae_convT2d_k4_fwd', x, w, pre, act, B, Cin, H, W, w.shape[1], stride, pad, repack=True, wr=wr)


def convT2d_stats_tiles(x, w, stride, pad):
    B, Cin, H, W = x.shape
    return int(_lib.lib().mvae_convT2d_k4_stats_tiles(B, Cin, H, W, w.shape[1], stride, pad))


def convT2d_fwd_stats(x, w, stride, pad, wr=None):
    _need_gpu(x, w, wr); _f32c(x, w, wr)
    B, Cin, H, W = x.shape
    Cout = w.shape[1]
    tiles = convT2d_stats_tiles(x, w, stride, pad)
    if tiles <= 0:
        raise RuntimeError('statistics-only transposed conv: shape %s -> %d channels not covered' % (tuple(x.shape), Cout))
    part = torch.empty(tiles, Cout, 2, dtype=torch.float32, device=x.device)
    if wr is not None:
        ws, wsb, wp = _ptr(wr), wr.numel() * 4, None
    else:
        ws, wsb = _ws_args(Cin * Cout * 16 * 4, x.device)
        wp = _ptr(w)
    check(_lib.lib().mvae_convT2d_k4_fwd_stats(_ptr(x), wp, _ptr(part), part.numel(), B, Cin, H, W, Cout, stride, pad,
                                               ws, wsb, _stream()), 'mvae_convT2d_k4_fwd_stats')
    return part


def bn_stats_merge(part, G, save_mean, save_invstd, running_mean, running_var, eps=1e-5, momentum=0.1, n_updates=1,
                   n_updates_dev=None):
    _need_gpu(part, save_mean, save_invstd, running_mean, running_var)
    _f32c(part, save_mean, save_invstd, running_mean, running_var)
    tiles, C = part.shape[0], part.shape[1]
    check(_lib.lib().mvae_bn_stats_merge(_ptr(part), tiles, _lib.STATS_TILE_ELEMS, G, C, _ptr(save_mean), _ptr(save_invstd),
                                         _ptr(running_mean), _ptr(running_var), eps, momentum, n_updates,
                                         _ptr(n_updates_dev), _stream()), 'mvae_bn_stats_merge')


def convT2d_dgrad(dy, w, dx, pre_in, stride, pad):
    _need_gpu(dy, w, dx, pre_in); _f32c(dy, w, dx, pre_in)
    B, Cin, H, W = dx.shape
    _conv_call('mvae_convT2d_k4_dgrad', dy, w, dx, pre_in, B, Cin, H, W, w.shape[1], stride, pad)


def convT2d_wgrad(dy, x, dw, stride, pad, accumulate=False):
    _need_gpu(dy, x, dw); _f32c(dy, x, dw)
    B, Cin, H, W = x.shape
    Cout = dw.shape[1]
    nbytes = _lib.lib().mvae_gemm_ws_bytes(Cin, Cout * 16, B * H * W)
    ws, wsb = _ws_args(nbytes, dy.device)
    check(_lib.lib().mvae_convT2d_k4_wgrad(_ptr(dy), _ptr(x), _ptr(dw), B, Cin, H, W, Cout, stride, pad,
                                           ACCUMULATE if accumulate else 0, ws, wsb, _stream()),
          'mvae_convT2d_k4_wgrad')


def bn_train_fwd(x, gamma, beta, y, save_mean, save_invstd, running_mean, running_var, G,
                 eps=1e-5, momentum=0.1, n_updates=1, swish=True, n_updates_dev=None):
    _need_gpu(x, gamma, beta, y, save_mean, save_invstd, running_mean, running_var)
    _f32c(x, gamma, beta, y, save_mean, save_invstd, running_mean, running_var)
    GB, C = x.shape[0], x.shape[1]
    HW = x.numel() // (GB * C)
    B = GB // G
    nbytes = _lib.lib().mvae_bn_ws_bytes(G, C, B * HW)
    ws, wsb = _ws_args(nbytes, x.device)
    check(_lib.lib().mvae_bn_train_fwd(_ptr(x), _ptr(gamma), _ptr(beta), _ptr(y), _ptr(save_mean),
                                       _ptr(save_invstd), _ptr(running_mean), _ptr(running_var),
                                       G, B, C, HW, eps, momentum, n_updates, _ptr(n_updates_dev),
                                       ACT_SWISH if swish else 0,
                                       ws, wsb, _stream()), 'mvae_bn_train_fwd')


def bn_train_bwd(dy, x, gamma, beta, save_mean, save_invstd, dx, dgamma, dbeta, G, swish=True,
                 accumulate=False):
    _need_gpu(dy, x, gamma, beta, save_mean, save_invstd, dx, dgamma, dbeta)
    _f32c(dy, x, gamma, beta, save_mean, save_invstd, dx, dgamma, dbeta)
    GB, C = x.shape[0], x.shape[1]
    HW = x.numel() // (GB * C)
    B = GB // G
    nbytes = _lib.lib().mvae_bn_ws_bytes(G, C, B * HW)
    ws, wsb = _ws_args(nbytes, x.device)
    flags = (ACT_SWISH if swish else 0) | (ACCUMULATE if accumulate else 0)
    check(_lib.lib().mvae_bn_train_bwd(_ptr(dy), _ptr(x), _ptr(gamma), _ptr(beta), _ptr(save_mean),
                                       _ptr(save_invstd), _ptr(dx), _ptr(dgamma), _ptr(dbeta),
                                       G, B, C, HW, flags, ws, wsb, _stream()), 'mvae_bn_train_bwd')


def bn_eval_fwd(x, gamma, beta, y, running_mean, running_var, eps=1e-5, swish=True):
    _need_gpu(x, gamma, beta, y, running_mean, running_var)
    _f32c(x, gamma, beta, y, running_mean, running_var)
    N, C = x.shape[0], x.shape[1]
    HW = x.numel() // (N * C)
    check(_lib.lib().mvae_bn_eval_fwd(_ptr(x), _ptr(gamma), _ptr(beta), _ptr(y), _ptr(running_mean),
                                      _ptr(running_var), N, C, HW, eps, ACT_SWISH if swish else 0,
                                      _stream()), 'mvae_bn_eval_fwd')


def reparam_fwd(mu, logvar, eps, z):
    _need_gpu(mu, logvar, eps, z); _f32c(mu, logvar, eps, z)
    check(_lib.lib().mvae_reparam_fwd(_ptr(mu), _ptr(logvar), _ptr(eps), _ptr(z), mu.numel(), _stream()),
          'mvae_reparam_fwd')


def sigmoid_fwd(x, y):
    _need_gpu(x, y); _f32c(x, y)
    check(_lib.lib().mvae_sigmoid_fwd(_ptr(x), _ptr(y), x.numel(), _stream()), 'mvae_sigmoid_fwd')


def affine_fwd(x, scale, shift, y):
    _need_gpu(x, scale, shift, y); _f32c(x, scale, shift, y)
    if scale.numel() != shift.numel() or x.numel() % scale.numel():
        raise RuntimeError('affine_fwd: scale/shift must have equal sizes dividing x')
    check(_lib.lib().mvae_affine_fwd(_ptr(x), _ptr(scale), _ptr(shift), _ptr(y), x.numel(), scale.numel(),
                                     _stream()), 'mvae_affine_fwd')


def swish_fwd(x, y):
    _need_gpu(x, y); _f32c(x, y)
    check(_lib.lib().mvae_swish_fwd(_ptr(x), _ptr(y), x.numel(), _stream()), 'mvae_swish_fwd')


def swish_bwd(dy, x, dx):
    _need_gpu(dy, x, dx); _f32c(dy, x, dx)
    check(_lib.lib().mvae_swish_bwd(_ptr(dy), _ptr(x), _ptr(dx), x.numel(), _stream()), 'mvae_swish_bwd')


def _index_kind(idx):
    if idx.dim() != 1:
        raise RuntimeError('embedding index must be 1-D')
    if idx.dtype == torch.int64:
        if idx.numel() > 1 and idx.stride(0) != 1:
            raise RuntimeError('int64 embedding index must be contiguous')
        return 0
    if idx.dtype == torch.float32:
        return max(int(idx.stride(0)), 1)
    raise RuntimeError('embedding index must be int64 or float32, got %s' % idx.dtype)


def block_gather(src, idx_dev, dst, block_elems):
    _need_gpu(src, idx_dev, dst); _f32c(src, dst)
    check(_lib.lib().mvae_block_gather(_ptr(src), _ptr(idx_dev), _ptr(dst), idx_dev.numel(), block_elems,
                                       _stream()), 'mvae_block_gather')


def block_scatter_add(src, idx_dev, dst, n_dst, block_elems):
    _need_gpu(src, idx_dev, dst); _f32c(src, dst)
    check(_lib.lib().mvae_block_scatter_add(_ptr(src), _ptr(idx_dev), _ptr(dst), idx_dev.numel(), n_dst,
                                            block_elems, _stream()), 'mvae_block_scatter_add')


def scatter_sums(vals, coef, idx_dev, out, total, accumulate_total=True):
    _need_gpu(vals, coef, idx_dev, out, total); _f32c(vals, coef, out, total)
    check(_lib.lib().mvae_scatter_sums(_ptr(vals), _ptr(coef), _ptr(idx_dev), _ptr(out), _ptr(total),
                                       vals.numel(), ACCUMULATE if accumulate_total else 0, _stream()),
          'mvae_scatter_sums')


def embedding_swish_fwd(idx, w, act):
    _need_gpu(idx, w, act); _f32c(w, act)
    check(_lib.lib().mvae_embedding_swish_fwd(_ptr(idx), _index_kind(idx), _ptr(w), _ptr(act), idx.numel(),
                                              w.shape[0], w.shape[1], _stream()),
          'mvae_embedding_swish_fwd')


def embedding_swish_bwd(idx, w, dact, dw, accumulate=False):
    _need_gpu(idx, w, dact, dw); _f32c(w, dact, dw)
    check(_lib.lib().mvae_embedding_swish_bwd(_ptr(idx), _index_kind(idx), _ptr(w), _ptr(dact), _ptr(dw),
                                              idx.numel(), w.shape[0], w.shape[1],
                                              ACCUMULATE if accumulate else 0, _stream()),
          'mvae_embedding_swish_bwd')


def _experts(mus, lvs):
    ex = _lib.Experts()
    for i, (m, v) in enumerate(zip(mus, lvs)):
        ex.mu[i] = m.data_ptr()
        ex.logvar[i] = v.data_ptr()
    return ex


def _expert_ld(mus, lvs):
    if len(mus) > _lib.MAX_EXPERTS:
        raise RuntimeError('at most %d experts' % _lib.MAX_EXPERTS)
    ld = mus[0].stride(0) if mus else 0
    for t in list(mus) + list(lvs):
        _need_gpu(t)
        if t.dtype != torch.float32 or t.dim() != 2 or t.stride(1) != 1 or t.stride(0) != ld:
            raise RuntimeError('expert mu/logvar must be fp32 [B,D] views with unit column stride and '
                               'a common row stride')
    return ld


_ALL_EXPERTS = {}


def all_experts_mask(n_experts, device):
    if not 1 <= n_experts <= _lib.MAX_EXPERTS:
        raise RuntimeError('1..%d experts, got %d' % (_lib.MAX_EXPERTS, n_experts))
    capturing = torch.cuda.is_current_stream_capturing()
    key = (n_experts, str(device))
    if not capturing and key in _ALL_EXPERTS:
        return _ALL_EXPERTS[key]
    bits = (1 << n_experts) - 1
    m = torch.full((1,), bits - (1 << 32) if bits >= (1 << 31) else bits, dtype=torch.int32, device=device)
    m._mvae_mask_ok = m._version
    if not capturing:
        _ALL_EXPERTS[key] = m
    return m


def _check_no_prior_masks(masks_dev, variant, n_experts):
    if not str(variant).endswith('-noprior') or masks_dev.numel() > 64 or torch.cuda.is_current_stream_capturing():
        return
    if getattr(masks_dev, '_mvae_mask_ok', None) == masks_dev._version:
        return
    live = (1 << n_experts) - 1
    for t, m in enumerate(masks_dev.tolist()):
        if (m & live) == 0:
            raise RuntimeError('PoE without the built-in prior: term %d selects no expert (mask %#x)' % (t, m & 0xffffffff))
    try:
        masks_dev._mvae_mask_ok = masks_dev._version
    except AttributeError:
        pass


def poe_fwd(mus, lvs, masks_dev, noise, mu, logvar, z, kl, variant):
    ld = _expert_ld(mus, lvs)
    _need_gpu(masks_dev, noise, mu, logvar, z, kl); _f32c(noise, mu, logvar, z, kl)
    T, B, D = mu.shape
    ex = _experts(mus, lvs)
    _check_no_prior_masks(masks_dev, variant, len(mus))
    check(_lib.lib().mvae_poe_fwd(ctypes.byref(ex), ld, len(mus), _ptr(masks_dev), T, _ptr(noise), _ptr(mu),
                                  _ptr(logvar), _ptr(z), _ptr(kl), B, D, _lib.POE_VARIANT[variant],
                                  _stream()), 'mvae_poe_fwd')


def poe_fwd_draw(mus, lvs, masks_dev, noise_out, seed, counter_dev, counter_offset, mu, logvar, z, kl, variant):
    ld = _expert_ld(mus, lvs)
    _need_gpu(masks_dev, noise_out, counter_dev, mu, logvar, z, kl); _f32c(noise_out, mu, logvar, z, kl)
    T, B, D = mu.shape
    ex = _experts(mus, lvs)
    check(_lib.lib().mvae_poe_fwd_draw(ctypes.byref(ex), ld, len(mus), _ptr(masks_dev), T, _ptr(noise_out), seed,
                                       _ptr(counter_dev), int(counter_offset), _ptr(mu), _ptr(logvar), _ptr(z),
                                       _ptr(kl), B, D, _lib.POE_VARIANT[variant], _stream()), 'mvae_poe_fwd_draw')


def poe_bwd(mus, lvs, masks_dev, noise, mu, logvar, dz, dmu, dlogvar, dkl, g_mus, g_lvs, variant,
            dkl_per_term=False):
    ld = _expert_ld(mus, lvs)
    ldg = _expert_ld(g_mus, g_lvs)
    _need_gpu(masks_dev, noise, mu, logvar, dz, dmu, dlogvar, dkl)
    _f32c(noise, mu, logvar, dz, dmu, dlogvar, dkl)
    T, B, D = mu.shape
    ex = _experts(mus, lvs)
    gr = _lib.ExpertGrads()
    for i, (m, v) in enumerate(zip(g_mus, g_lvs)):
        gr.dmu[i] = m.data_ptr()
        gr.dlogvar[i] = v.data_ptr()
    check(_lib.lib().mvae_poe_bwd(ctypes.byref(ex), ld, len(mus), _ptr(masks_dev), T, _ptr(noise), _ptr(mu),
                                  _ptr(logvar), _ptr(dz), _ptr(dmu), _ptr(dlogvar), _ptr(dkl),
                                  1 if dkl_per_term else 0, ctypes.byref(gr), ldg, B, D, _lib.POE_VARIANT[variant], _stream()),
          'mvae_poe_bwd')


def poe_bwd_split(mus, lvs, masks_dev, noise, mu, logvar, dz_a, slots_a, dz_b, slots_b, dkl, g_mus, g_lvs, variant,
                  dkl_per_term=False):
    ld = _expert_ld(mus, lvs)
    ldg = _expert_ld(g_mus, g_lvs)
    _need_gpu(masks_dev, noise, mu, logvar, dz_a, dz_b, dkl)
    _f32c(noise, mu, logvar, dz_a, dz_b, dkl)
    T, B, D = mu.shape
    if len(slots_a) != T or len(slots_b) != T:
        raise RuntimeError('one slot per term')
    for dz, slots in ((dz_a, slots_a), (dz_b, slots_b)):
        if dz.numel() != (max(slots) + 1) * B * D:
            raise RuntimeError('latent-gradient buffer does not match its slots')
    ex = _experts(mus, lvs)
    gr = _lib.ExpertGrads()
    for i, (m, v) in enumerate(zip(g_mus, g_lvs)):
        gr.dmu[i] = m.data_ptr()
        gr.dlogvar[i] = v.data_ptr()
    sa = (ctypes.c_int * T)(*[int(x) for x in slots_a])
    sb = (ctypes.c_int * T)(*[int(x) for x in slots_b])
    check(_lib.lib().mvae_poe_bwd_split(ctypes.byref(ex), ld, len(mus), _ptr(masks_dev), T, _ptr(noise), _ptr(mu),
                                        _ptr(logvar), _ptr(dz_a), sa, _ptr(dz_b), sb, _ptr(dkl),
                                        1 if dkl_per_term else 0, ctypes.byref(gr), ldg, B, D,
                                        _lib.POE_VARIANT[variant], _stream()), 'mvae_poe_bwd_split')


def kl_rows_fwd(mu, logvar, kl):
    _need_gpu(mu, logvar, kl); _f32c(mu, logvar, kl)
    check(_lib.lib().mvae_kl_rows_fwd(_ptr(mu), _ptr(logvar), _ptr(kl), mu.shape[0], mu.shape[1], _stream()),
          'mvae_kl_rows_fwd')


def kl_rows_bwd(mu, logvar, dkl, dmu, dlogvar):
    _need_gpu(mu, logvar, dkl, dmu, dlogvar); _f32c(mu, logvar, dkl, dmu, dlogvar)
    check(_lib.lib().mvae_kl_rows_bwd(_ptr(mu), _ptr(logvar), _ptr(dkl), _ptr(dmu), _ptr(dlogvar),
                                      mu.shape[0], mu.shape[1], _stream()), 'mvae_kl_rows_bwd')


def bce_rowsum_fwd(logits, target, rowsum, colw=None, drow=None, dlogits=None, rows_per_group=None,
                   target_rows=None, target_div=1, target_strides=None):
    _need_gpu(logits, target, rowsum, colw, drow, dlogits); _f32c(logits, target, rowsum, colw, drow, dlogits)
    R, P = logits.shape
    t_rs, t_cs = target_strides if target_strides is not None else (P, 1)
    check(_lib.lib().mvae_bce_rowsum_fwd(_ptr(logits), _ptr(target), _ptr(colw), _ptr(rowsum), _ptr(drow),
                                         _ptr(dlogits), R, P, rows_per_group or R,
                                         target_rows or target.shape[0], target_div, t_rs, t_cs, _stream()),
          'mvae_bce_rowsum_fwd')


def bce_rowsum_bwd(logits, target, drow, dlogits, colw=None, rows_per_group=None, target_rows=None,
                   target_div=1, target_strides=None):
    _need_gpu(logits, target, drow, dlogits, colw); _f32c(logits, target, drow, dlogits, colw)
    R, P = logits.shape
    t_rs, t_cs = target_strides if target_strides is not None else (P, 1)
    check(_lib.lib().mvae_bce_rowsum_bwd(_ptr(logits), _ptr(target), _ptr(colw), _ptr(drow), _ptr(dlogits),
                                         R, P, rows_per_group or R, target_rows or target.shape[0],
                                         target_div, t_rs, t_cs, _stream()), 'mvae_bce_rowsum_bwd')


def ce_fwd(logits, label, row, drow=None, dlogits=None, rows_per_group=None, label_rows=None):
    _need_gpu(logits, label, row, drow, dlogits); _f32c(logits, row, drow, dlogits)
    if label.dtype != torch.int64 or not label.is_contiguous():
        raise RuntimeError('labels must be contiguous int64')
    R, K = logits.shape
    check(_lib.lib().mvae_ce_fwd(_ptr(logits), _ptr(label), _ptr(row), _ptr(drow), _ptr(dlogits), R, K,
                                 rows_per_group or R, label_rows or label.shape[0], _stream()),
          'mvae_ce_fwd')


def ce_bwd(logits, label, drow, dlogits, rows_per_group=None, label_rows=None):
    _need_gpu(logits, label, drow, dlogits); _f32c(logits, drow, dlogits)
    R, K = logits.shape
    check(_lib.lib().mvae_ce_bwd(_ptr(logits), _ptr(label), _ptr(drow), _ptr(dlogits), R, K,
                                 rows_per_group or R, label_rows or label.shape[0], _stream()),
          'mvae_ce_bwd')


def group_sums(rows, coef, out, total, G, rows_per_group, accumulate=False):
    _need_gpu(rows, coef, out, total); _f32c(rows, coef, out, total)
    check(_lib.lib().mvae_group_sums(_ptr(rows), _ptr(coef), _ptr(out), _ptr(total), G, rows_per_group,
                                     ACCUMULATE if accumulate else 0, _stream()), 'mvae_group_sums')


def elbo_reduce(parts, elbo, T, zero=None, counter_dev=None, counter_inc=0):
    if not 0 < len(parts) <= _lib.ELBO_MAX_PARTS:
        raise RuntimeError('1..%d ELBO parts per launch' % _lib.ELBO_MAX_PARTS)
    arr = (_lib.ElboPart * len(parts))()
    for q, (rows, coef, term_of, first, groups, rpg) in enumerate(parts):
        _need_gpu(rows, coef, term_of); _f32c(rows, coef)
        if rows.numel() < groups * rpg:
            raise RuntimeError('ELBO part %d: %d values for %d x %d' % (q, rows.numel(), groups, rpg))
        arr[q] = _lib.ElboPart(_ptr(rows), _ptr(coef), _ptr(term_of), int(first), int(groups), int(rpg))
    _need_gpu(elbo, zero, counter_dev); _f32c(elbo, zero)
    check(_lib.lib().mvae_elbo_reduce(arr, len(parts), _ptr(elbo), int(T), _ptr(zero),
                                      0 if zero is None else zero.numel(), _ptr(counter_dev), int(counter_inc),
                                      _stream()), 'mvae_elbo_reduce')


def philox_fill(out, seed, counter_dev, offset=0, keep_prob=None):
    _need_gpu(out, counter_dev); _f32c(out)
    check(_lib.lib().mvae_philox_fill(_ptr(out), out.numel(), 0 if keep_prob is None else 1,
                                      0.0 if keep_prob is None else float(keep_prob), seed, _ptr(counter_dev),
                                      int(offset), _stream()), 'mvae_philox_fill')



def randn_(out, seed, counter_dev):
    _need_gpu(out, counter_dev); _f32c(out)
    check(_lib.lib().mvae_randn(_ptr(out), out.numel(), seed, _ptr(counter_dev), _stream()), 'mvae_randn')


def bernoulli_(out, keep_prob, seed, counter_dev):
    _need_gpu(out, counter_dev); _f32c(out)
    check(_lib.lib().mvae_bernoulli(_ptr(out), out.numel(), keep_prob, seed, _ptr(counter_dev), _stream()),
          'mvae_bernoulli')


def adam_step(param, grad, exp_avg, exp_avg_sq, step_dev, lr, beta1=0.9, beta2=0.999, eps=1e-8,
              grad_scale=1.0):
    _need_gpu(param, grad, exp_avg, exp_avg_sq, step_dev); _f32c(param, grad, exp_avg, exp_avg_sq)
    check(_lib.lib().mvae_adam_step(_ptr(param), _ptr(grad), _ptr(exp_avg), _ptr(exp_avg_sq), param.numel(),
                                    lr, beta1, beta2, eps, grad_scale, _ptr(step_dev), _stream()),
          'mvae_adam_step')


def adam_apply(param, grad, exp_avg, exp_avg_sq, step_dev, lr, beta1=0.9, beta2=0.999, eps=1e-8, grad_scale=1.0):
    _need_gpu(param, grad, exp_avg, exp_avg_sq, step_dev); _f32c(param, grad, exp_avg, exp_avg_sq)
    check(_lib.lib().mvae_adam_apply(_ptr(param), _ptr(grad), _ptr(exp_avg), _ptr(exp_avg_sq), param.numel(),
                                     lr, beta1, beta2, eps, grad_scale, _ptr(step_dev), _stream()),
          'mvae_adam_apply')


def adam_apply_at(param, grad, exp_avg, exp_avg_sq, step_dev, step_add, lr, beta1=0.9, beta2=0.999, eps=1e-8,
                  grad_scale=1.0):
    _need_gpu(param, grad, exp_avg, exp_avg_sq, step_dev); _f32c(param, grad, exp_avg, exp_avg_sq)
    check(_lib.lib().mvae_adam_apply_at(_ptr(param), _ptr(grad), _ptr(exp_avg), _ptr(exp_avg_sq), param.numel(),
                                        lr, beta1, beta2, eps, grad_scale, _ptr(step_dev), int(step_add), _stream()),
          'mvae_adam_apply_at')


def adam_apply_coef(param, grad, exp_avg, exp_avg_sq, coef2, beta1=0.9, beta2=0.999, eps=1e-8, grad_scale=1.0):
    _need_gpu(param, grad, exp_avg, exp_avg_sq, coef2); _f32c(param, grad, exp_avg, exp_avg_sq, coef2)
    check(_lib.lib().mvae_adam_apply_coef(_ptr(param), _ptr(grad), _ptr(exp_avg), _ptr(exp_avg_sq), param.numel(),
                                          _ptr(coef2), beta1, beta2, eps, grad_scale, _stream()), 'mvae_adam_apply_coef')


def adam_prepare(step_dev, delta, lr, beta1, beta2, coef2):
    _need_gpu(step_dev, coef2); _f32c(coef2)
    check(_lib.lib().mvae_adam_prepare(_ptr(step_dev), int(delta), lr, beta1, beta2, _ptr(coef2), _stream()),
          'mvae_adam_prepare')


def trace_marker(tag=0):
    check(_lib.lib().mvae_trace_marker(int(tag), _stream()), 'mvae_trace_marker')


def counter_add(counter_dev, delta):
    _need_gpu(counter_dev)
    check(_lib.lib().mvae_counter_add(_ptr(counter_dev), int(delta), _stream()), 'mvae_counter_add')


def fill_(out, value):
    _need_gpu(out); _f32c(out)
    check(_lib.lib().mvae_fill(_ptr(out), out.numel(), float(value), _stream()), 'mvae_fill')


def ingest(image_src, image_dst, label_src, label_dst, table_host, table_dst):
    _need_gpu(image_src, image_dst, label_src, label_dst, table_dst)
    if not table_host.is_pinned():
        raise RuntimeError('ingest: the table source must be pinned host memory')
    for a, b in ((image_src, image_dst), (label_src, label_dst), (table_host, table_dst)):
        if a.dtype != b.dtype or a.numel() != b.numel() or not (a.is_contiguous() and b.is_contiguous()):
            raise RuntimeError('ingest: source and destination must be contiguous and alike')
    check(_lib.lib().mvae_ingest(_ptr(image_src), _ptr(image_dst), image_src.numel(),
                                 _ptr(label_src), _ptr(label_dst), label_src.numel() * label_src.element_size(),
                                 _ptr(table_host), _ptr(table_dst), table_host.numel() * table_host.element_size(),
                                 _stream()), 'mvae_ingest')


def ingest_ok(image_src, image_dst, label_src, label_dst):
    return (image_src.is_cuda and label_src.is_cuda and image_src.dtype == torch.float32 == image_dst.dtype
            and label_src.dtype == label_dst.dtype and image_src.is_contiguous() and label_src.is_contiguous()
            and image_src.numel() == image_dst.numel() and label_src.numel() == label_dst.numel()
            and image_src.numel() % 4 == 0 and (label_src.numel() * label_src.element_size()) % 4 == 0
            and image_src.data_ptr() % 16 == 0 and image_dst.data_ptr() % 16 == 0)


def dropout_fanout_fwd(h, masks, out, scale):
    _need_gpu(h, masks, out); _f32c(h, masks, out)
    G, B, N = masks.shape
    check(_lib.lib().mvae_dropout_fanout_fwd(_ptr(h), _ptr(masks), _ptr(out), scale, G, B, N, _stream()),
          'mvae_dropout_fanout_fwd')


def dropout_fanin_bwd(dout, masks, dh, scale):
    _need_gpu(dout, masks, dh); _f32c(dout, masks, dh)
    G, B, N = masks.shape
    check(_lib.lib().mvae_dropout_fanin_bwd(_ptr(dout), _ptr(masks), _ptr(dh), scale, G, B, N, _stream()),
          'mvae_dropout_fanin_bwd')


def bce_elem_fwd(logits, target, out):
    _need_gpu(logits, target, out); _f32c(logits, target, out)
    check(_lib.lib().mvae_bce_elem_fwd(_ptr(logits), _ptr(target), _ptr(out), logits.numel(), _stream()),
          'mvae_bce_elem_fwd')


def bce_elem_bwd(logits, target, g, dlogits, dtarget=None):
    _need_gpu(logits, target, g, dlogits, dtarget); _f32c(logits, target, g, dlogits, dtarget)
    check(_lib.lib().mvae_bce_elem_bwd(_ptr(logits), _ptr(target), _ptr(g), _ptr(dlogits), _ptr(dtarget),
                                       logits.numel(), _stream()), 'mvae_bce_elem_bwd')


def _rows(t, what, width=None):
    if not (t.is_cuda and t.dtype == torch.float32 and t.dim() == 2 and t.stride(1) == 1):
        raise RuntimeError('%s must be a float32 [rows, width] GPU view with unit column stride' % what)
    if width is not None and t.shape[1] != width:
        raise RuntimeError('%s: width %d, expected %d' % (what, t.shape[1], width))
    return t


def gru_cell_fwd(gi, gh, h_prev, h_new, gates=None):
    B, H = _rows(h_prev, 'h_prev').shape
    _rows(gi, 'gi', 3 * H); _rows(gh, 'gh', 3 * H); _rows(h_new, 'h_new', H)
    if gates is not None:
        _need_gpu(gates); _f32c(gates)
    check(_lib.lib().mvae_gru_cell_fwd(_ptr(gi), gi.stride(0), _ptr(gh), gh.stride(0), _ptr(h_prev), h_prev.stride(0),
                                       _ptr(h_new), h_new.stride(0), _ptr(gates), B, H, _stream()), 'mvae_gru_cell_fwd')


def gru_cell_bwd(dh_new, dh_extra, gates, h_prev, dgi, dgh, dh_prev):
    B, H = _rows(h_prev, 'h_prev').shape
    _rows(dh_new, 'dh_new', H)
    if dh_extra is not None:
        _rows(dh_extra, 'dh_extra', H)
    _need_gpu(gates, dgi, dgh, dh_prev); _f32c(gates, dgi, dgh, dh_prev)
    check(_lib.lib().mvae_gru_cell_bwd(_ptr(dh_new), dh_new.stride(0), _ptr(dh_extra),
                                       0 if dh_extra is None else dh_extra.stride(0), _ptr(gates), _ptr(h_prev),
                                       h_prev.stride(0), _ptr(dgi), _ptr(dgh), _ptr(dh_prev), B, H, _stream()),
          'mvae_gru_cell_bwd')


def _idx64(idx):
    if not (idx.is_cuda and idx.dtype == torch.int64 and idx.dim() == 1):
        raise RuntimeError('embedding index must be a 1-D int64 GPU tensor (a column of text[B, L] is fine)')
    return max(int(idx.stride(0)), 1)


def embedding_fwd(idx, w, out, swish=False):
    _need_gpu(w); _f32c(w)
    R, width = _rows(out, 'out', w.shape[1]).shape
    check(_lib.lib().mvae_embedding_fwd(_ptr(idx), _idx64(idx), _ptr(w), _ptr(out), out.stride(0), idx.numel(),
                                        w.shape[0], width, ACT_SWISH if swish else 0, _stream()), 'mvae_embedding_fwd')


def embedding_bwd(idx, w, dout, dw, swish=False, accumulate=False):
    _need_gpu(w, dw); _f32c(w, dw)
    _rows(dout, 'dout', w.shape[1])
    flags = (ACT_SWISH if swish else 0) | (ACCUMULATE if accumulate else 0)
    check(_lib.lib().mvae_embedding_bwd(_ptr(idx), _idx64(idx), _ptr(w), _ptr(dout), dout.stride(0), _ptr(dw),
                                        idx.numel(), w.shape[0], w.shape[1], flags, _stream()), 'mvae_embedding_bwd')


def copy2d(src, dst, mask=None, scale=1.0, accumulate=False):
    rows, cols = _rows(src, 'src').shape
    _rows(dst, 'dst', cols)
    if mask is not None:
        _rows(mask, 'mask', cols)
    check(_lib.lib().mvae_copy2d(_ptr(src), src.stride(0), _ptr(dst), dst.stride(0), _ptr(mask),
                                 0 if mask is None else mask.stride(0), float(scale), rows, cols,
                                 ACCUMULATE if accumulate else 0, _stream()), 'mvae_copy2d')


def argmax_rows(x, out):
    R, K_ = _rows(x, 'x').shape
    if not (out.is_cuda and out.dtype == torch.int64 and out.is_contiguous() and out.numel() == R):
        raise RuntimeError('argmax_rows wants a contiguous int64 GPU output of one entry per row')
    check(_lib.lib().mvae_argmax_rows(_ptr(x), x.stride(0), _ptr(out), R, K_, _stream()), 'mvae_argmax_rows')
```

### multimodal-vae-public_amd/profiler.py

```python
import glob
import hashlib
import os

import torch

from . import kernels as K

MFMA_F32_PEAK_TFLOPS = 157.3
HBM_PEAK_GBS = 8000.0


def code_stamp():
    here = os.path.dirname(os.path.abspath(__file__))
    files = sorted(glob.glob(os.path.join(here, 'csrc', '*.hip')) + glob.glob(os.path.join(here, 'csrc', '*.h')))
    files.append(os.path.join(os.path.dirname(here), 'include', 'mvae_hip.h'))
    h = hashlib.sha256()
    for f in files:
        h.update(os.path.basename(f).encode())
        with open(f, 'rb') as fh:
            h.update(fh.read())
    return {'csrc_sha16': h.hexdigest()[:16], 'head': os.environ.get('MVAE_GIT_HEAD', 'unknown')}


def _numel_bytes(args, kwargs):
    n = 0
    for a in list(args) + list(kwargs.values()):
        if torch.is_tensor(a):
            n += a.numel() * a.element_size()
        elif isinstance(a, (list, tuple)):
            n += sum(t.numel() * t.element_size() for t in a if torch.is_tensor(t))
    return n


def _lin_cost(which):
    def cost(*a, **kw):
        if which == 'fwd':
            (M, Kd), N = a[0].shape, a[1].shape[0]
        elif which == 'dgrad':
            (M, N), Kd = a[0].shape, a[1].shape[1]
        else:
            (M, N), Kd = a[0].shape, a[1].shape[1]
        return 2.0 * M * N * Kd, 'M%d N%d K%d' % (M, N, Kd)
    return cost


def _conv_cost(kind):
    def cost(*a, **kw):
        if kind == 'conv2d_fwd':
            out = a[2] if a[2] is not None else a[3]
            fl = 2.0 * out.numel() * a[1].shape[1] * 16
            shape = tuple(out.shape)
        elif kind == 'convT2d_dgrad':
            fl = 2.0 * a[2].numel() * a[1].shape[1] * 16
            shape = tuple(a[2].shape)
        elif kind == 'conv2d_dgrad':
            dy, w = a[0], a[1]
            fl = 2.0 * dy.numel() * w.shape[1] * 16
            shape = tuple(a[2].shape)
        elif kind == 'convT2d_fwd':
            x, w = a[0], a[1]
            fl = 2.0 * x.numel() * w.shape[1] * 16
            shape = tuple((a[2] if a[2] is not None else a[3]).shape)
        elif kind == 'conv2d_wgrad':
            dy, x, dw = a[0], a[1], a[2]
            fl = 2.0 * dy.numel() * dw.shape[1] * 16
            shape = tuple(dw.shape)
        else:
            dy, x, dw = a[0], a[1], a[2]
            fl = 2.0 * x.numel() * dw.shape[1] * 16
            shape = tuple(dw.shape)
        return fl, 'x'.join(str(s) for s in shape)
    return cost


def _lin_grouped_cost(which):
    def cost(*a, **kw):
        if which == 'fwd':
            (G, M, Kd), N = a[0].shape, a[1].shape[0]
        elif which == 'dgrad':
            (G, M, N), Kd = a[0].shape, a[1].shape[1]
        else:
            (G, M, N), Kd = a[0].shape, a[1].shape[2]
        return 2.0 * G * M * N * Kd, 'G%d M%d N%d K%d' % (G, M, N, Kd)
    return cost


def _wgrad_batched_cost(items, *a, **kw):
    fl = sum(2.0 * dy.shape[0] * dy.shape[1] * x.shape[1] for dy, x, _, _, _ in items)
    return fl, '%d layers' % len(items)


def _convT_stats_cost(x, w, stride, pad, *a, **kw):
    B, Cin, H, W = x.shape
    OH, OW = (H - 1) * stride - 2 * pad + 4, (W - 1) * stride - 2 * pad + 4
    return 2.0 * x.numel() * w.shape[1] * 16, '%dx%dx%dx%d' % (B, w.shape[1], OH, OW)


GEMM_COSTS = {
    'convT2d_fwd_stats': _convT_stats_cost,
    'linear_wgrad_batched': _wgrad_batched_cost,
    'linear_fwd_grouped': _lin_grouped_cost('fwd'), 'linear_dgrad_grouped': _lin_grouped_cost('dgrad'),
    'linear_wgrad_grouped': _lin_grouped_cost('wgrad'),
    'linear_fwd': _lin_cost('fwd'), 'linear_dgrad': _lin_cost('dgrad'), 'linear_wgrad': _lin_cost('wgrad'),
    'linear_bce_fwd': _lin_cost('fwd'), 'linear_ce_fwd': _lin_cost('fwd'),
    'conv2d_fwd': _conv_cost('conv2d_fwd'), 'conv2d_dgrad': _conv_cost('conv2d_dgrad'),
    'conv2d_wgrad': _conv_cost('conv2d_wgrad'), 'convT2d_fwd': _conv_cost('convT2d_fwd'),
    'convT2d_dgrad': _conv_cost('convT2d_dgrad'), 'convT2d_wgrad': _conv_cost('convT2d_wgrad'),
}
def _bn_fwd_bytes(x, gamma, beta, y, *a, **kw):
    return (3 if y is not None else 1) * x.numel() * 4


def _bn_bwd_bytes(dy, x, *a, **kw):
    return 5 * x.numel() * 4


def _adam_bytes(param, *a, **kw):
    return 28 * param.numel()


def _bce_rows_bytes(logits, target, rowsum, colw=None, drow=None, dlogits=None, *a, **kw):
    return 2 * logits.numel() * 4 + rowsum.numel() * 4 + (logits.numel() * 4 if dlogits is not None else 0)


def _poe_fwd_bytes(mus, lvs, masks_dev, noise, mu, logvar, z, kl, *a, **kw):
    T, B, D = mu.shape
    E = len(mus)
    return (2 * E + (T if noise is not None else 0)) * B * D * 4 + 3 * T * B * D * 4 + T * B * 4


def _poe_draw_bytes(mus, lvs, masks_dev, noise_out, seed, counter_dev, counter_offset, mu, logvar, z, kl, *a, **kw):
    T, B, D = mu.shape
    return 2 * len(mus) * B * D * 4 + 4 * T * B * D * 4 + T * B * 4


def _poe_bwd_bytes(mus, lvs, masks_dev, noise, mu, logvar, *a, **kw):
    T, B, D = mu.shape
    E = len(mus)
    return (2 * E + 4 * T) * B * D * 4 + 2 * E * B * D * 4


HBM_COSTS = {
    'bn_train_fwd': _bn_fwd_bytes, 'bn_train_bwd': _bn_bwd_bytes,
    'adam_step': _adam_bytes, 'adam_apply': _adam_bytes, 'adam_apply_at': _adam_bytes,
    'bce_rowsum_fwd': _bce_rows_bytes,
    'poe_fwd': _poe_fwd_bytes, 'poe_fwd_draw': _poe_draw_bytes, 'poe_bwd': _poe_bwd_bytes, 'poe_bwd_split': _poe_bwd_bytes,
}

HBM_OPS = ['bn_train_fwd', 'bn_train_bwd', 'bn_eval_fwd', 'swish_fwd', 'swish_bwd', 'embedding_swish_fwd',
           'embedding_swish_bwd', 'poe_fwd', 'poe_bwd', 'kl_rows_fwd', 'kl_rows_bwd', 'bce_rowsum_fwd',
           'bce_rowsum_bwd', 'ce_fwd', 'ce_bwd', 'group_sums', 'randn_', 'bernoulli_', 'adam_step', 'fill_',
           'dropout_fanout_fwd', 'dropout_fanin_bwd', 'bce_elem_fwd', 'bce_elem_bwd', 'embedding_swish_fwd_grouped',
           'embedding_swish_bwd_grouped', 'block_gather', 'block_scatter_add', 'elbo_reduce', 'philox_fill',
           'adam_apply', 'sigmoid_fwd', 'affine_fwd', 'scatter_sums', 'poe_fwd_draw', 'poe_bwd_split', 'adam_apply_at',
           'counter_add', 'conv_repack_batched', 'bn_stats_merge']


class KernelProfile(object):
    def __init__(self, marker=False, timed=True):
        self.marker = marker
        self.timed = timed
        self.sequence = []
        self.records = []
        self.last_call = {}
        self._saved = {}

    def _wrap(self, name, fn, cost):
        def wrapped(*a, **kw):
            if self.marker:
                K.trace_marker(len(self.sequence))
            e0 = e1 = None
            if self.timed:
                e0 = torch.cuda.Event(enable_timing=True)
                e1 = torch.cuda.Event(enable_timing=True)
                e0.record()
            out = fn(*a, **kw)
            if self.timed:
                e1.record()
            if cost is not None:
                flops, key = cost(*a, **kw)
                nbytes = 0
            else:
                by = HBM_COSTS.get(name)
                flops, key, nbytes = 0.0, '', (by(*a, **kw) if by is not None else _numel_bytes(a, kw))
                if by is not None:
                    first = next((t for t in a if torch.is_tensor(t)), None)
                    key = 'x'.join(str(s) for s in first.shape) if first is not None else '%d B' % nbytes
            self.sequence.append((name, key, flops, nbytes))
            if not self.timed:
                return out
            self.records.append((name, key, flops, nbytes, e0, e1))
            self.last_call[(name, key)] = (fn, a, kw)
            return out
        return wrapped

    def __enter__(self):
        for name in list(GEMM_COSTS) + HBM_OPS:
            fn = getattr(K, name)
            self._saved[name] = fn
            setattr(K, name, self._wrap(name, fn, GEMM_COSTS.get(name)))
        return self

    def __exit__(self, *exc):
        for name, fn in self._saved.items():
            setattr(K, name, fn)
        self._saved = {}
        return False

    def steady_state_ms(self, name, key, launches=20, replays=5):
        fn, a, kw = self.last_call[(name, key)]
        st = torch.cuda.Stream()
        st.wait_stream(torch.cuda.current_stream())
        with torch.cuda.stream(st):
            fn(*a, **kw)
        st.synchronize()
        g = torch.cuda.CUDAGraph()
        with torch.cuda.graph(g, stream=st):
            for _ in range(launches):
                fn(*a, **kw)
        e0, e1 = torch.cuda.Event(enable_timing=True), torch.cuda.Event(enable_timing=True)
        with torch.cuda.stream(st):
            g.replay()
            e0.record()
            for _ in range(replays):
                g.replay()
            e1.record()
        st.synchronize()
        torch.cuda.current_stream().wait_stream(st)
        return e0.elapsed_time(e1) / (launches * replays)

    def summary(self):
        torch.cuda.synchronize()
        agg = {}
        for name, key, flops, nbytes, e0, e1 in self.records:
            a = agg.setdefault((name, key), [0, 0.0, 0.0, 0.0])
            a[0] += 1
            a[1] += e0.elapsed_time(e1)
            a[2] += flops
            a[3] += nbytes
        rows = []
        for (name, key), (calls, ms, flops, nbytes) in agg.items():
            rows.append(dict(name=name, key=key, calls=calls, ms_total=ms, ms_avg=ms / calls,
                             flops=flops / calls, bytes=nbytes / calls,
                             tflops=(flops / (ms * 1e-3) / 1e12) if ms > 0 else 0.0,
                             gbs=(nbytes / (ms * 1e-3) / 1e9) if ms > 0 else 0.0))
        rows.sort(key=lambda r: -r['ms_total'])
        return rows
```

Measured before the change: 1.948 million images/sec.

## Compute label encoder on per-class table and gather PoE experts by row index

Adds kernels for a small-M 'table' linear path (fwd, dgrad, wgrad) and a class_sum reduction. The label encoder can then run once per class (10 rows) instead of once per batch row, with gradients folded back per class. New PoE variants read expert rows through an index array, so the per-class table is gathered on the fly instead of being materialised at batch size. This is meant to remove redundant GEMM work and memory traffic on the label branch, at the cost of extra kernels and indexed loads in PoE.

```diff
diff --git a/include/mvae_hip.h b/include/mvae_hip.h
--- a/include/mvae_hip.h
+++ b/include/mvae_hip.h
@@ -177,6 +177,42 @@
                        const float *dkl, int dkl_per_term,
                        const mvae_expert_grads_t *grads, int ldg,
                        int B, int D, int variant, mvae_stream_t stream);
+
+typedef struct {
+    const int64_t *idx[MVAE_MAX_EXPERTS];
+    int rows[MVAE_MAX_EXPERTS];
+} mvae_expert_rows_t;
+int mvae_poe_fwd_rows(const mvae_experts_t *experts, const mvae_expert_rows_t *rows, int ld, int E,
+                      const uint32_t *masks_dev, int T,
+                      const float *noise, float *mu, float *logvar, float *z, float *kl,
+                      int B, int D, int variant, mvae_stream_t stream);
+int mvae_poe_fwd_draw_rows(const mvae_experts_t *experts, const mvae_expert_rows_t *rows, int ld, int E,
+                           const uint32_t *masks_dev, int T,
+                           float *noise_out, uint64_t seed, const uint64_t *counter_dev, uint64_t counter_offset,
+                           float *mu, float *logvar, float *z, float *kl,
+                           int B, int D, int variant, mvae_stream_t stream);
+int mvae_poe_bwd_rows(const mvae_experts_t *experts, const mvae_expert_rows_t *rows, int ld, int E,
+                      const uint32_t *masks_dev, int T,
+                      const float *noise, const float *mu, const float *logvar,
+                      const float *dz, const float *dmu, const float *dlogvar,
+                      const float *dkl, int dkl_per_term,
+                      const mvae_expert_grads_t *grads, int ldg,
+                      int B, int D, int variant, mvae_stream_t stream);
+int mvae_poe_bwd_split_rows(const mvae_experts_t *experts, const mvae_expert_rows_t *rows, int ld, int E,
+                            const uint32_t *masks_dev, int T,
+                            const float *noise, const float *mu, const float *logvar,
+                            const float *dz_a, const int *slot_a, const float *dz_b, const int *slot_b,
+                            const float *dkl, int dkl_per_term,
+                            const mvae_expert_grads_t *grads, int ldg,
+                            int B, int D, int variant, mvae_stream_t stream);
+
+int mvae_class_sum(const int64_t *idx, const float *g, int ldg, float *out, int R, int n_classes, int width,
+                   mvae_stream_t stream);
+int mvae_table_linear_fwd(const float *x, int x_swish, float *x_act, const float *w, const float *bias,
+                          float *pre, float *act, int M, int N, int K, mvae_stream_t stream);
+int mvae_table_linear_dgrad(const float *dy, const float *w, const float *pre_in, float *dx,
+                            int M, int N, int K, int flags, mvae_stream_t stream);
+int mvae_table_linear_wgrad(const mvae_wgrad_item *items, int n_items, mvae_stream_t stream);
 
 int mvae_reparam_fwd(const float *mu, const float *logvar, const float *eps, float *z, size_t n,
                      mvae_stream_t stream);
diff --git a/multimodal-vae-public_amd/_lib.py b/multimodal-vae-public_amd/_lib.py
--- a/multimodal-vae-public_amd/_lib.py
+++ b/multimodal-vae-public_amd/_lib.py
@@ -52,6 +52,10 @@
 
 
 REPACK_MAX = 16
+
+
+class ExpertRows(ctypes.Structure):
+    _fields_ = [('idx', c_void_p * MAX_EXPERTS), ('rows', c_int * MAX_EXPERTS)]
 
 
 class ExpertGrads(ctypes.Structure):
@@ -106,6 +110,19 @@
     'mvae_poe_bwd_split': (c_int, [ctypes.POINTER(Experts), c_int, c_int, P, c_int, P, P, P, P,
                                    ctypes.POINTER(c_int), P, ctypes.POINTER(c_int), P, c_int,
                                    ctypes.POINTER(ExpertGrads), c_int, c_int, c_int, c_int, P]),
+    'mvae_poe_fwd_rows': (c_int, [ctypes.POINTER(Experts), ctypes.POINTER(ExpertRows), c_int, c_int, P, c_int, P, P, P, P, P,
+                                  c_int, c_int, c_int, P]),
+    'mvae_poe_fwd_draw_rows': (c_int, [ctypes.POINTER(Experts), ctypes.POINTER(ExpertRows), c_int, c_int, P, c_int, P,
+                                       c_uint64, P, c_uint64, P, P, P, P, c_int, c_int, c_int, P]),
+    'mvae_poe_bwd_rows': (c_int, [ctypes.POINTER(Experts), ctypes.POINTER(ExpertRows), c_int, c_int, P, c_int, P, P, P, P,
+                                  P, P, P, c_int, ctypes.POINTER(ExpertGrads), c_int, c_int, c_int, c_int, P]),
+    'mvae_poe_bwd_split_rows': (c_int, [ctypes.POINTER(Experts), ctypes.POINTER(ExpertRows), c_int, c_int, P, c_int, P, P,
+                                        P, P, ctypes.POINTER(c_int), P, ctypes.POINTER(c_int), P, c_int,
+                                        ctypes.POINTER(ExpertGrads), c_int, c_int, c_int, c_int, P]),
+    'mvae_class_sum': (c_int, [P, P, c_int, P, c_int, c_int, c_int, P]),
+    'mvae_table_linear_fwd': (c_int, [P, c_int, P, P, P, P, P, c_int, c_int, c_int, P]),
+    'mvae_table_linear_dgrad': (c_int, [P, P, P, P, c_int, c_int, c_int, c_int, P]),
+    'mvae_table_linear_wgrad': (c_int, [ctypes.POINTER(WgradItem), c_int, P]),
     'mvae_kl_rows_fwd': (c_int, [P, P, P, c_int, c_int, P]),
     'mvae_kl_rows_bwd': (c_int, [P, P, P, P, P, c_int, c_int, P]),
     'mvae_bce_rowsum_fwd': (c_int, [P, P, P, P, P, P] + [c_int] * 7 + [P]),
diff --git a/multimodal-vae-public_amd/csrc/label_table.hip b/multimodal-vae-public_amd/csrc/label_table.hip
--- /dev/null
+++ b/multimodal-vae-public_amd/csrc/label_table.hip
@@ -0,0 +1,279 @@
+#include "common.h"
+
+namespace {
+
+constexpr int TBL_MAX_ROWS = 16;
+constexpr int TBL_LDS_FLOATS = 16384;
+
+template <int V> struct Vec { float v[V]; };
+template <int V> __device__ __forceinline__ Vec<V> vload(const float *p) {
+    Vec<V> r;
+    if constexpr (V == 4) {
+        const float4 t = *reinterpret_cast<const float4 *>(p);
+        r.v[0] = t.x; r.v[1] = t.y; r.v[2] = t.z; r.v[3] = t.w;
+    } else {
+        r.v[0] = *p;
+    }
+    return r;
+}
+template <int V> __device__ __forceinline__ void vstore(float *p, const Vec<V> &r) {
+    if constexpr (V == 4) *reinterpret_cast<float4 *>(p) = make_float4(r.v[0], r.v[1], r.v[2], r.v[3]);
+    else *p = r.v[0];
+}
+
+constexpr int CS_LANES = 16;
+__global__ __launch_bounds__(64 * CS_LANES) void class_sum_kernel(const int64_t *idx, const float *g, int ldg, float *out,
+                                                                  int R, int C, int W) {
+    __shared__ float part[CS_LANES][64];
+    const int tx = threadIdx.x & 63, ty = threadIdx.x >> 6;
+    const int j = blockIdx.x * 64 + tx, c = blockIdx.y;
+    float s = 0.f;
+    if (j < W) {
+        const int per = (R + CS_LANES - 1) / CS_LANES, r0 = ty * per, r1 = min(R, r0 + per);
+#pragma unroll 8
+        for (int r = r0; r < r1; ++r) {
+            const int64_t raw = idx[r];
+            const int cr = (int)(raw < 0 ? 0 : (raw > C - 1 ? C - 1 : raw));
+            const float v = g[(size_t)r * ldg + j];
+            s += (cr == c) ? v : 0.f;
+        }
+    }
+    part[ty][tx] = s;
+    __syncthreads();
+    if (ty == 0 && j < W) {
+        s = 0.f;
+#pragma unroll
+        for (int q = 0; q < CS_LANES; q += 4) s += (part[q][tx] + part[q + 1][tx]) + (part[q + 2][tx] + part[q + 3][tx]);
+        out[(size_t)c * W + j] = s;
+    }
+}
+
+constexpr int FWD_WAVES = 4;
+template <int V>
+__global__ __launch_bounds__(64 * FWD_WAVES) void table_linear_fwd_kernel(const float *x, int x_swish, float *x_act,
+                                                                          const float *w, const float *bias, float *pre,
+                                                                          float *act, int M, int N, int K) {
+    extern __shared__ float xs[];
+    const int total = M * K;
+    for (int i = threadIdx.x * V; i < total; i += 64 * FWD_WAVES * V) {
+        Vec<V> t = vload<V>(x + i);
+        if (x_swish) {
+#pragma unroll
+            for (int q = 0; q < V; ++q) t.v[q] = swishf_(t.v[q]);
+            if (x_act && blockIdx.x == 0) vstore<V>(x_act + i, t);
+        }
+        vstore<V>(xs + i, t);
+    }
+    __syncthreads();
+    const int lane = threadIdx.x & 63;
+    const int n = blockIdx.x * FWD_WAVES + (threadIdx.x >> 6);
+    if (n >= N) return;
+    float acc[TBL_MAX_ROWS];
+#pragma unroll
+    for (int m = 0; m < TBL_MAX_ROWS; ++m) acc[m] = 0.f;
+    const float *wr = w + (size_t)n * K;
+    for (int k = lane * V; k < K; k += 64 * V) {
+        const Vec<V> wv = vload<V>(wr + k);
+#pragma unroll
+        for (int m = 0; m < TBL_MAX_ROWS; ++m) {
+            if (m < M) {
+                const Vec<V> xv = vload<V>(xs + m * K + k);
+#pragma unroll
+                for (int q = 0; q < V; ++q) acc[m] = __builtin_fmaf(wv.v[q], xv.v[q], acc[m]);
+            }
+        }
+    }
+    float mine = 0.f;
+#pragma unroll
+    for (int m = 0; m < TBL_MAX_ROWS; ++m) {
+        if (m < M) {
+            const float r = wave_sum(acc[m]);
+            if (lane == m) mine = r;
+        }
+    }
+    if (lane < M) {
+        const float v = mine + (bias ? bias[n] : 0.f);
+        const size_t o = (size_t)lane * N + n;
+        if (pre) pre[o] = v;
+        if (act) act[o] = swishf_(v);
+    }
+}
+
+constexpr int DG_COLS = 16, DG_THREADS = 256;
+template <int V>
+__global__ __launch_bounds__(DG_THREADS) void table_linear_dgrad_kernel(const float *dy, const float *w, const float *pre_in,
+                                                                        float *dx, int M, int N, int K, int accumulate) {
+    constexpr int CT = DG_COLS / V, SLICES = DG_THREADS / CT;
+    extern __shared__ float sm[];
+    const int col = (threadIdx.x % CT) * V, slice = threadIdx.x / CT;
+    const int k = blockIdx.x * DG_COLS + col;
+    const int kc = k < K ? k : 0;
+    for (int i = threadIdx.x; i < M * N; i += DG_THREADS) sm[i] = dy[i];
+    __syncthreads();
+    float acc[TBL_MAX_ROWS][V];
+#pragma unroll
+    for (int m = 0; m < TBL_MAX_ROWS; ++m)
+#pragma unroll
+        for (int q = 0; q < V; ++q) acc[m][q] = 0.f;
+#pragma unroll 8
+    for (int n = slice; n < N; n += SLICES) {
+        const Vec<V> wv = vload<V>(w + (size_t)n * K + kc);
+#pragma unroll
+        for (int m = 0; m < TBL_MAX_ROWS; ++m) {
+            if (m < M) {
+                const float d = sm[m * N + n];
+#pragma unroll
+                for (int q = 0; q < V; ++q) acc[m][q] = __builtin_fmaf(d, wv.v[q], acc[m][q]);
+            }
+        }
+    }
+    __syncthreads();
+#pragma unroll
+    for (int m = 0; m < TBL_MAX_ROWS; ++m) {
+        if (m < M) {
+#pragma unroll
+            for (int q = 0; q < V; ++q) sm[(slice * M + m) * DG_COLS + col + q] = acc[m][q];
+        }
+    }
+    __syncthreads();
+    for (int o = threadIdx.x; o < M * DG_COLS; o += DG_THREADS) {
+        const int m = o / DG_COLS, c = o % DG_COLS, kk = blockIdx.x * DG_COLS + c;
+        if (kk >= K) continue;
+        float s = 0.f;
+        for (int q = 0; q < SLICES; ++q) s += sm[(q * M + m) * DG_COLS + c];
+        const size_t od = (size_t)m * K + kk;
+        if (pre_in) s *= swish_grad_(pre_in[od]);
+        dx[od] = accumulate ? dx[od] + s : s;
+    }
+}
+
+constexpr int WG_ROWS = 8, WG_THREADS = 256, WG_MAX_ITEMS = 4;
+struct TableWgradArgs {
+    mvae_wgrad_item it[WG_MAX_ITEMS];
+    int first_block[WG_MAX_ITEMS + 1];
+    int n;
+};
+template <int V>
+__global__ __launch_bounds__(WG_THREADS) void table_linear_wgrad_kernel(TableWgradArgs a) {
+    extern __shared__ float sm[];
+    int q = 0;
+    while (q + 1 < a.n && (int)blockIdx.x >= a.first_block[q + 1]) ++q;
+    const mvae_wgrad_item it = a.it[q];
+    const int M = it.M, N = it.N, K = it.K;
+    const int n0 = ((int)blockIdx.x - a.first_block[q]) * WG_ROWS;
+    float *dys = sm + M * K;
+    const int KV = K / V;
+    for (int i = threadIdx.x; i < M * KV; i += WG_THREADS) {
+        const int m = i / KV, kv = i - m * KV;
+        vstore<V>(sm + m * K + kv * V, vload<V>(it.x + (size_t)m * it.ldx + kv * V));
+    }
+    for (int i = threadIdx.x; i < M * WG_ROWS; i += WG_THREADS) {
+        const int m = i / WG_ROWS, r = i % WG_ROWS;
+        dys[i] = (n0 + r < N) ? it.dy[(size_t)m * it.lddy + n0 + r] : 0.f;
+    }
+    __syncthreads();
+    const int accumulate = it.flags & MVAE_ACCUMULATE;
+    for (int i = threadIdx.x; i < WG_ROWS * KV; i += WG_THREADS) {
+        const int r = i / KV, kv = i - r * KV, n = n0 + r;
+        if (n >= N) break;
+        Vec<V> s;
+#pragma unroll
+        for (int j = 0; j < V; ++j) s.v[j] = 0.f;
+        for (int m = 0; m < M; ++m) {
+            const float d = dys[m * WG_ROWS + r];
+            const Vec<V> xv = vload<V>(sm + m * K + kv * V);
+#pragma unroll
+            for (int j = 0; j < V; ++j) s.v[j] = __builtin_fmaf(d, xv.v[j], s.v[j]);
+        }
+        float *o = it.dw + (size_t)n * K + kv * V;
+        if (accumulate) {
+            const Vec<V> old = vload<V>(o);
+#pragma unroll
+            for (int j = 0; j < V; ++j) s.v[j] += old.v[j];
+        }
+        vstore<V>(o, s);
+    }
+    if (it.db && threadIdx.x < WG_ROWS && n0 + (int)threadIdx.x < N) {
+        float s = 0.f;
+        for (int m = 0; m < M; ++m) s += dys[m * WG_ROWS + threadIdx.x];
+        float *o = it.db + n0 + threadIdx.x;
+        *o = accumulate ? *o + s : s;
+    }
+}
+
+inline bool tbl_dims_ok(int M, int N, int K) { return M > 0 && M <= TBL_MAX_ROWS && N > 0 && K > 0; }
+
+}
+
+MVAE_EXPORT int mvae_class_sum(const int64_t *idx, const float *g, int ldg, float *out, int R, int n_classes, int width,
+                               mvae_stream_t stream) {
+    if (!idx || !g || !out || R <= 0 || n_classes <= 0 || n_classes > 65535 || width <= 0 || ldg < width)
+        return MVAE_ERR_ARG;
+    hipLaunchKernelGGL(class_sum_kernel, dim3((width + 63) / 64, n_classes), dim3(64 * CS_LANES), 0, (hipStream_t)stream,
+                       idx, g, ldg, out, R, n_classes, width);
+    return mvae_launch_status();
+}
+
+MVAE_EXPORT int mvae_table_linear_fwd(const float *x, int x_swish, float *x_act, const float *w, const float *bias,
+                                      float *pre, float *act, int M, int N, int K, mvae_stream_t stream) {
+    if (!x || !w || (!pre && !act) || !tbl_dims_ok(M, N, K) || (size_t)M * K > TBL_LDS_FLOATS) return MVAE_ERR_ARG;
+    const dim3 grid((N + FWD_WAVES - 1) / FWD_WAVES), block(64 * FWD_WAVES);
+    const size_t lds = (size_t)M * K * sizeof(float);
+    const bool vec = K % 4 == 0 && aligned16(x) && aligned16(w) && (!x_act || aligned16(x_act));
+    if (vec)
+        hipLaunchKernelGGL(table_linear_fwd_kernel<4>, grid, block, lds, (hipStream_t)stream, x, x_swish, x_act, w, bias,
+                           pre, act, M, N, K);
+    else
+        hipLaunchKernelGGL(table_linear_fwd_kernel<1>, grid, block, lds, (hipStream_t)stream, x, x_swish, x_act, w, bias,
+                           pre, act, M, N, K);
+    return mvae_launch_status();
+}
+
+MVAE_EXPORT int mvae_table_linear_dgrad(const float *dy, const float *w, const float *pre_in, float *dx, int M, int N,
+                                        int K, int flags, mvae_stream_t stream) {
+    if (!dy || !w || !dx || !tbl_dims_ok(M, N, K) || (size_t)M * N > TBL_LDS_FLOATS || (flags & ~MVAE_ACCUMULATE))
+        return MVAE_ERR_ARG;
+    const bool vec = K % 4 == 0 && aligned16(w);
+    const size_t slices = vec ? DG_THREADS / (DG_COLS / 4) : DG_THREADS / DG_COLS;
+    size_t floats = (size_t)M * N;
+    const size_t part = slices * M * DG_COLS;
+    if (floats < part) floats = part;
+    const dim3 grid((K + DG_COLS - 1) / DG_COLS), block(DG_THREADS);
+    const int acc = (flags & MVAE_ACCUMULATE) ? 1 : 0;
+    if (vec)
+        hipLaunchKernelGGL(table_linear_dgrad_kernel<4>, grid, block, floats * sizeof(float), (hipStream_t)stream, dy, w,
+                           pre_in, dx, M, N, K, acc);
+    else
+        hipLaunchKernelGGL(table_linear_dgrad_kernel<1>, grid, block, floats * sizeof(float), (hipStream_t)stream, dy, w,
+                           pre_in, dx, M, N, K, acc);
+    return mvae_launch_status();
+}
+
+MVAE_EXPORT int mvae_table_linear_wgrad(const mvae_wgrad_item *items, int n_items, mvae_stream_t stream) {
+    if (!items || n_items <= 0 || n_items > WG_MAX_ITEMS) return MVAE_ERR_ARG;
+    TableWgradArgs a = {};
+    bool vec = true;
+    size_t floats = 0;
+    int blocks = 0;
+    for (int q = 0; q < n_items; ++q) {
+        const mvae_wgrad_item &it = items[q];
+        if (!it.dy || !it.x || !it.dw || !tbl_dims_ok(it.M, it.N, it.K) || it.lddy < it.N || it.ldx < it.K ||
+            (it.flags & ~MVAE_ACCUMULATE) || (size_t)it.M * (it.K + WG_ROWS) > TBL_LDS_FLOATS)
+            return MVAE_ERR_ARG;
+        vec = vec && it.K % 4 == 0 && it.ldx % 4 == 0 && aligned16(it.x) && aligned16(it.dw);
+        const size_t f = (size_t)it.M * (it.K + WG_ROWS);
+        if (f > floats) floats = f;
+        a.it[q] = it;
+        a.first_block[q] = blocks;
+        blocks += (it.N + WG_ROWS - 1) / WG_ROWS;
+    }
+    a.first_block[n_items] = blocks;
+    a.n = n_items;
+    if (vec)
+        hipLaunchKernelGGL(table_linear_wgrad_kernel<4>, dim3(blocks), dim3(WG_THREADS), floats * sizeof(float),
+                           (hipStream_t)stream, a);
+    else
+        hipLaunchKernelGGL(table_linear_wgrad_kernel<1>, dim3(blocks), dim3(WG_THREADS), floats * sizeof(float),
+                           (hipStream_t)stream, a);
+    return mvae_launch_status();
+}
diff --git a/multimodal-vae-public_amd/csrc/poe.hip b/multimodal-vae-public_amd/csrc/poe.hip
--- a/multimodal-vae-public_amd/csrc/poe.hip
+++ b/multimodal-vae-public_amd/csrc/poe.hip
@@ -15,13 +15,28 @@
     uint64_t seed; const uint64_t *counter; uint64_t counter_offset; int draw;
 };
 
+struct RowsDirect {
+    __device__ __forceinline__ size_t operator()(int, int b) const { return (size_t)b; }
+};
+struct RowsIndexed {
+    mvae_expert_rows_t r;
+    __device__ __forceinline__ size_t operator()(int e, int b) const {
+        const int64_t *ix = r.idx[e];
+        if (!ix) return (size_t)b;
+        const int64_t c = ix[b];
+        const int64_t hi = r.rows[e] - 1;
+        return (size_t)(c < 0 ? 0 : (c > hi ? hi : c));
+    }
+};
+
 __device__ __forceinline__ float poe_precision(float lv, int variant) {
     float var = expf(lv) + POE_EPS;
     if (variant == MVAE_POE_VARIANT_A) var = var + POE_EPS;
     return 1.0f / var;
 }
 
-__global__ __launch_bounds__(POE_THREADS) void poe_fwd_kernel(PoeArgs a, const uint32_t *masks,
+template <typename Rows>
+__global__ __launch_bounds__(POE_THREADS) void poe_fwd_kernel(PoeArgs a, Rows row_of, const uint32_t *masks,
                                                               float *noise, float *mu, float *logvar,
                                                               float *z, float *kl) {
     extern __shared__ float lds[];
@@ -36,9 +51,9 @@
     for (int t = t_lo; t < t_hi; ++t) { klacc[(t - t_lo) * POE_THREADS] = 0.f; used |= masks[t]; }
     const uint64_t launch = a.draw ? *a.counter + a.counter_offset : 0;
     for (int d = lane; d < a.D; d += 64) {
-        const size_t oe = (size_t)b * a.ld + d;
         for (int e = 0; e < a.E; ++e) {
             if (!((used >> e) & 1u)) continue;
+            const size_t oe = row_of(e, b) * a.ld + d;
             const float te = poe_precision(a.ex.logvar[e][oe], a.variant);
             mine[(e * 2 + 0) * POE_THREADS] = te;
             mine[(e * 2 + 1) * POE_THREADS] = a.ex.mu[e][oe] * te;
@@ -77,7 +92,8 @@
 
 struct PoeDzMap { signed char slot_a[MVAE_ELBO_MAX_TERMS], slot_b[MVAE_ELBO_MAX_TERMS]; };
 
-__global__ __launch_bounds__(POE_THREADS) void poe_bwd_kernel(PoeArgs a, const uint32_t *masks,
+template <typename Rows>
+__global__ __launch_bounds__(POE_THREADS) void poe_bwd_kernel(PoeArgs a, Rows row_of, const uint32_t *masks,
                                                               const float *noise, const float *mu,
                                                               const float *logvar, const float *dz,
                                                               const float *dz_b, PoeDzMap dzm,
@@ -129,7 +145,7 @@
             mine[(t * 3 + 2) * POE_THREADS] = pmu;
         }
         for (int e = e_lo; e < e_hi; ++e) {
-            const size_t o = (size_t)b * a.ld + d;
+            const size_t o = row_of(e, b) * a.ld + d;
             const float me = a.ex.mu[e][o], lve = a.ex.logvar[e][o];
             const float ex = expf(lve);
             const float te = poe_precision(lve, a.variant);
@@ -196,41 +212,107 @@
     return true;
 }
 
+inline bool poe_rows_ok(const mvae_expert_rows_t *rows, int E, bool *indexed) {
+    *indexed = false;
+    if (!rows) return true;
+    for (int e = 0; e < E; ++e)
+        if (rows->idx[e]) {
+            if (rows->rows[e] <= 0) return false;
+            *indexed = true;
+        }
+    return true;
+}
+
+inline RowsIndexed poe_rows(const mvae_expert_rows_t *rows, int E) {
+    RowsIndexed r = {};
+    for (int e = 0; e < E; ++e) { r.r.idx[e] = rows->idx[e]; r.r.rows[e] = rows->rows[e]; }
+    return r;
+}
+
+inline PoeArgs poe_args(const mvae_experts_t *experts, int ld, int E, int T, int B, int D, int variant) {
+    PoeArgs a;
+    a.ex = *experts; a.ld = ld; a.E = E; a.T = T; a.B = B; a.D = D;
+    a.variant = variant & ~MVAE_POE_NO_PRIOR; a.no_prior = (variant & MVAE_POE_NO_PRIOR) ? 1 : 0;
+    a.seed = 0; a.counter = nullptr; a.counter_offset = 0; a.draw = 0; a.chunk = 1;
+    return a;
+}
+
+int poe_fwd_launch(const mvae_experts_t *experts, const mvae_expert_rows_t *rows, int ld, int E,
+                   const uint32_t *masks_dev, int T, float *noise, bool draw, uint64_t seed,
+                   const uint64_t *counter_dev, uint64_t counter_offset, float *mu, float *logvar, float *z, float *kl,
+                   int B, int D, int variant, mvae_stream_t stream) {
+    bool indexed;
+    if (!poe_args_ok(experts, ld, E, T, B, D, variant) || !masks_dev || !mu || !logvar || !poe_rows_ok(rows, E, &indexed))
+        return MVAE_ERR_ARG;
+    if (draw && (!z || !noise || !counter_dev)) return MVAE_ERR_ARG;
+    PoeArgs a = poe_args(experts, ld, E, T, B, D, variant);
+    if (draw) { a.seed = seed; a.counter = counter_dev; a.counter_offset = counter_offset; a.draw = 1; }
+    const int rpb = POE_THREADS / 64;
+    a.chunk = poe_chunk(T);
+    const size_t lds_bytes = ((size_t)E * 2 + a.chunk) * POE_THREADS * sizeof(float);
+    const dim3 grid((B + rpb - 1) / rpb, (T + a.chunk - 1) / a.chunk);
+    if (indexed)
+        hipLaunchKernelGGL(poe_fwd_kernel<RowsIndexed>, grid, dim3(POE_THREADS), lds_bytes, (hipStream_t)stream, a,
+                           poe_rows(rows, E), masks_dev, noise, mu, logvar, z, kl);
+    else
+        hipLaunchKernelGGL(poe_fwd_kernel<RowsDirect>, grid, dim3(POE_THREADS), lds_bytes, (hipStream_t)stream, a,
+                           RowsDirect(), masks_dev, noise, mu, logvar, z, kl);
+    return mvae_launch_status();
+}
+
+int poe_bwd_launch(const mvae_experts_t *experts, const mvae_expert_rows_t *rows, int ld, int E,
+                   const uint32_t *masks_dev, int T, const float *noise, const float *mu, const float *logvar,
+                   const float *dz_a, const int *slot_a, const float *dz_b, const int *slot_b, const float *dmu,
+                   const float *dlogvar, const float *dkl, int dkl_per_term, const mvae_expert_grads_t *grads, int ldg,
+                   int B, int D, int variant, mvae_stream_t stream) {
+    const int dkl_stride = dkl_per_term ? 0 : B;
+    bool indexed;
+    if (!poe_args_ok(experts, ld, E, T, B, D, variant) || !masks_dev || !mu || !logvar || !grads || ldg < D ||
+        !poe_rows_ok(rows, E, &indexed))
+        return MVAE_ERR_ARG;
+    for (int e = 0; e < E; ++e)
+        if (!grads->dmu[e] || !grads->dlogvar[e]) return MVAE_ERR_ARG;
+    PoeDzMap m = {};
+    if (slot_a) {
+        if (!dz_a || !dz_b || !slot_b || T > MVAE_ELBO_MAX_TERMS) return MVAE_ERR_ARG;
+        for (int t = 0; t < T; ++t) {
+            if (slot_a[t] < -1 || slot_a[t] >= T || slot_b[t] < -1 || slot_b[t] >= T) return MVAE_ERR_ARG;
+            m.slot_a[t] = (signed char)slot_a[t]; m.slot_b[t] = (signed char)slot_b[t];
+        }
+    } else {
+        dz_b = nullptr;
+    }
+    PoeArgs a = poe_args(experts, ld, E, T, B, D, variant);
+    const int rpb = POE_THREADS / 64;
+    const size_t lds_bytes = (size_t)T * 3 * POE_THREADS * sizeof(float);
+    a.chunk = poe_chunk(E);
+    const dim3 grid((B + rpb - 1) / rpb, E ? (E + a.chunk - 1) / a.chunk : 1);
+    if (indexed)
+        hipLaunchKernelGGL(poe_bwd_kernel<RowsIndexed>, grid, dim3(POE_THREADS), lds_bytes, (hipStream_t)stream, a,
+                           poe_rows(rows, E), masks_dev, noise, mu, logvar, dz_a, dz_b, m, dmu, dlogvar, dkl, dkl_stride,
+                           *grads, ldg);
+    else
+        hipLaunchKernelGGL(poe_bwd_kernel<RowsDirect>, grid, dim3(POE_THREADS), lds_bytes, (hipStream_t)stream, a,
+                           RowsDirect(), masks_dev, noise, mu, logvar, dz_a, dz_b, m, dmu, dlogvar, dkl, dkl_stride,
+                           *grads, ldg);
+    return mvae_launch_status();
+}
+
 }
 
 MVAE_EXPORT int mvae_poe_fwd(const mvae_experts_t *experts, int ld, int E, const uint32_t *masks_dev, int T,
                              const float *noise, float *mu, float *logvar, float *z, float *kl, int B, int D,
                              int variant, mvae_stream_t stream) {
-    if (!poe_args_ok(experts, ld, E, T, B, D, variant) || !masks_dev || !mu || !logvar) return MVAE_ERR_ARG;
-    PoeArgs a;
-    a.ex = *experts; a.ld = ld; a.E = E; a.T = T; a.B = B; a.D = D;
-    a.variant = variant & ~MVAE_POE_NO_PRIOR; a.no_prior = (variant & MVAE_POE_NO_PRIOR) ? 1 : 0;
-    a.seed = 0; a.counter = nullptr; a.counter_offset = 0; a.draw = 0;
-    const int rows = POE_THREADS / 64;
-    a.chunk = poe_chunk(T);
-    const size_t lds_bytes = ((size_t)E * 2 + a.chunk) * POE_THREADS * sizeof(float);
-    hipLaunchKernelGGL(poe_fwd_kernel, dim3((B + rows - 1) / rows, (T + a.chunk - 1) / a.chunk), dim3(POE_THREADS), lds_bytes, (hipStream_t)stream, a,
-                       masks_dev, const_cast<float *>(noise), mu, logvar, z, kl);
-    return mvae_launch_status();
+    return poe_fwd_launch(experts, nullptr, ld, E, masks_dev, T, const_cast<float *>(noise), false, 0, nullptr, 0, mu,
+                          logvar, z, kl, B, D, variant, stream);
 }
 
 MVAE_EXPORT int mvae_poe_fwd_draw(const mvae_experts_t *experts, int ld, int E, const uint32_t *masks_dev, int T,
                                   float *noise_out, uint64_t seed, const uint64_t *counter_dev,
                                   uint64_t counter_offset, float *mu, float *logvar, float *z, float *kl, int B,
                                   int D, int variant, mvae_stream_t stream) {
-    if (!poe_args_ok(experts, ld, E, T, B, D, variant) || !masks_dev || !mu || !logvar || !z || !noise_out ||
-        !counter_dev)
-        return MVAE_ERR_ARG;
-    PoeArgs a;
-    a.ex = *experts; a.ld = ld; a.E = E; a.T = T; a.B = B; a.D = D;
-    a.variant = variant & ~MVAE_POE_NO_PRIOR; a.no_prior = (variant & MVAE_POE_NO_PRIOR) ? 1 : 0;
-    a.seed = seed; a.counter = counter_dev; a.counter_offset = counter_offset; a.draw = 1;
-    const int rows = POE_THREADS / 64;
-    a.chunk = poe_chunk(T);
-    const size_t lds_bytes = ((size_t)E * 2 + a.chunk) * POE_THREADS * sizeof(float);
-    hipLaunchKernelGGL(poe_fwd_kernel, dim3((B + rows - 1) / rows, (T + a.chunk - 1) / a.chunk), dim3(POE_THREADS), lds_bytes, (hipStream_t)stream, a,
-                       masks_dev, noise_out, mu, logvar, z, kl);
-    return mvae_launch_status();
+    return poe_fwd_launch(experts, nullptr, ld, E, masks_dev, T, noise_out, true, seed, counter_dev, counter_offset, mu,
+                          logvar, z, kl, B, D, variant, stream);
 }
 
 MVAE_EXPORT int mvae_poe_bwd(const mvae_experts_t *experts, int ld, int E, const uint32_t *masks_dev, int T,
@@ -238,23 +320,8 @@
                              const float *dmu, const float *dlogvar, const float *dkl, int dkl_per_term,
                              const mvae_expert_grads_t *grads, int ldg, int B, int D, int variant,
                              mvae_stream_t stream) {
-    const int dkl_stride = dkl_per_term ? 0 : B;
-    if (!poe_args_ok(experts, ld, E, T, B, D, variant) || !masks_dev || !mu || !logvar || !grads || ldg < D)
-        return MVAE_ERR_ARG;
-    for (int e = 0; e < E; ++e)
-        if (!grads->dmu[e] || !grads->dlogvar[e]) return MVAE_ERR_ARG;
-    PoeArgs a;
-    a.ex = *experts; a.ld = ld; a.E = E; a.T = T; a.B = B; a.D = D;
-    a.variant = variant & ~MVAE_POE_NO_PRIOR; a.no_prior = (variant & MVAE_POE_NO_PRIOR) ? 1 : 0;
-    a.seed = 0; a.counter = nullptr; a.counter_offset = 0; a.draw = 0;
-    const int rows = POE_THREADS / 64;
-    const size_t lds_bytes = (size_t)T * 3 * POE_THREADS * sizeof(float);
-    PoeDzMap none = {};
-    a.chunk = poe_chunk(E);
-    hipLaunchKernelGGL(poe_bwd_kernel, dim3((B + rows - 1) / rows, E ? (E + a.chunk - 1) / a.chunk : 1), dim3(POE_THREADS), lds_bytes,
-                       (hipStream_t)stream, a, masks_dev, noise, mu, logvar, dz, (const float *)nullptr, none, dmu,
-                       dlogvar, dkl, dkl_stride, *grads, ldg);
-    return mvae_launch_status();
+    return poe_bwd_launch(experts, nullptr, ld, E, masks_dev, T, noise, mu, logvar, dz, nullptr, nullptr, nullptr, dmu,
+                          dlogvar, dkl, dkl_per_term, grads, ldg, B, D, variant, stream);
 }
 
 MVAE_EXPORT int mvae_poe_bwd_split(const mvae_experts_t *experts, int ld, int E, const uint32_t *masks_dev, int T,
@@ -262,28 +329,44 @@
                                    const int *slot_a, const float *dz_b, const int *slot_b, const float *dkl,
                                    int dkl_per_term, const mvae_expert_grads_t *grads, int ldg, int B, int D,
                                    int variant, mvae_stream_t stream) {
-    const int dkl_stride = dkl_per_term ? 0 : B;
-    if (!poe_args_ok(experts, ld, E, T, B, D, variant) || !masks_dev || !mu || !logvar || !grads || ldg < D ||
-        !dz_a || !dz_b || !slot_a || !slot_b || T > MVAE_ELBO_MAX_TERMS)
-        return MVAE_ERR_ARG;
-    for (int e = 0; e < E; ++e)
-        if (!grads->dmu[e] || !grads->dlogvar[e]) return MVAE_ERR_ARG;
-    PoeDzMap m;
-    for (int t = 0; t < T; ++t) {
-        if (slot_a[t] < -1 || slot_a[t] >= T || slot_b[t] < -1 || slot_b[t] >= T) return MVAE_ERR_ARG;
-        m.slot_a[t] = (signed char)slot_a[t]; m.slot_b[t] = (signed char)slot_b[t];
-    }
-    PoeArgs a;
-    a.ex = *experts; a.ld = ld; a.E = E; a.T = T; a.B = B; a.D = D;
-    a.variant = variant & ~MVAE_POE_NO_PRIOR; a.no_prior = (variant & MVAE_POE_NO_PRIOR) ? 1 : 0;
-    a.seed = 0; a.counter = nullptr; a.counter_offset = 0; a.draw = 0;
-    const int rows = POE_THREADS / 64;
-    const size_t lds_bytes = (size_t)T * 3 * POE_THREADS * sizeof(float);
-    a.chunk = poe_chunk(E);
-    hipLaunchKernelGGL(poe_bwd_kernel, dim3((B + rows - 1) / rows, E ? (E + a.chunk - 1) / a.chunk : 1), dim3(POE_THREADS), lds_bytes,
-                       (hipStream_t)stream, a, masks_dev, noise, mu, logvar, dz_a, dz_b, m, (const float *)nullptr,
-                       (const float *)nullptr, dkl, dkl_stride, *grads, ldg);
-    return mvae_launch_status();
+    if (!slot_a) return MVAE_ERR_ARG;
+    return poe_bwd_launch(experts, nullptr, ld, E, masks_dev, T, noise, mu, logvar, dz_a, slot_a, dz_b, slot_b, nullptr,
+                          nullptr, dkl, dkl_per_term, grads, ldg, B, D, variant, stream);
+}
+
+MVAE_EXPORT int mvae_poe_fwd_rows(const mvae_experts_t *experts, const mvae_expert_rows_t *rows, int ld, int E,
+                                  const uint32_t *masks_dev, int T, const float *noise, float *mu, float *logvar,
+                                  float *z, float *kl, int B, int D, int variant, mvae_stream_t stream) {
+    return poe_fwd_launch(experts, rows, ld, E, masks_dev, T, const_cast<float *>(noise), false, 0, nullptr, 0, mu,
+                          logvar, z, kl, B, D, variant, stream);
+}
+
+MVAE_EXPORT int mvae_poe_fwd_draw_rows(const mvae_experts_t *experts, const mvae_expert_rows_t *rows, int ld, int E,
+                                       const uint32_t *masks_dev, int T, float *noise_out, uint64_t seed,
+                                       const uint64_t *counter_dev, uint64_t counter_offset, float *mu, float *logvar,
+                                       float *z, float *kl, int B, int D, int variant, mvae_stream_t stream) {
+    return poe_fwd_launch(experts, rows, ld, E, masks_dev, T, noise_out, true, seed, counter_dev, counter_offset, mu,
+                          logvar, z, kl, B, D, variant, stream);
+}
+
+MVAE_EXPORT int mvae_poe_bwd_rows(const mvae_experts_t *experts, const mvae_expert_rows_t *rows, int ld, int E,
+                                  const uint32_t *masks_dev, int T, const float *noise, const float *mu,
+                                  const float *logvar, const float *dz, const float *dmu, const float *dlogvar,
+                                  const float *dkl, int dkl_per_term, const mvae_expert_grads_t *grads, int ldg, int B,
+                                  int D, int variant, mvae_stream_t stream) {
+    return poe_bwd_launch(experts, rows, ld, E, masks_dev, T, noise, mu, logvar, dz, nullptr, nullptr, nullptr, dmu,
+                          dlogvar, dkl, dkl_per_term, grads, ldg, B, D, variant, stream);
+}
+
+MVAE_EXPORT int mvae_poe_bwd_split_rows(const mvae_experts_t *experts, const mvae_expert_rows_t *rows, int ld, int E,
+                                        const uint32_t *masks_dev, int T, const float *noise, const float *mu,
+                                        const float *logvar, const float *dz_a, const int *slot_a, const float *dz_b,
+                                        const int *slot_b, const float *dkl, int dkl_per_term,
+                                        const mvae_expert_grads_t *grads, int ldg, int B, int D, int variant,
+                                        mvae_stream_t stream) {
+    if (!slot_a) return MVAE_ERR_ARG;
+    return poe_bwd_launch(experts, rows, ld, E, masks_dev, T, noise, mu, logvar, dz_a, slot_a, dz_b, slot_b, nullptr,
+                          nullptr, dkl, dkl_per_term, grads, ldg, B, D, variant, stream);
 }
 
 MVAE_EXPORT int mvae_kl_rows_fwd(const float *mu, const float *logvar, float *kl, int B, int D,
diff --git a/multimodal-vae-public_amd/engine.py b/multimodal-vae-public_amd/engine.py
--- a/multimodal-vae-public_amd/engine.py
+++ b/multimodal-vae-public_amd/engine.py
@@ -33,6 +33,11 @@
         else:
             optimizer._m.copy_(opt[0]); optimizer._v.copy_(opt[1]); optimizer._step_dev.copy_(opt[2])
             optimizer._host_step = opt[3]
+
+
+def label_table_switch(env=None):
+    env = os.environ if env is None else env
+    return str(env.get('MVAE_LABEL_TABLE', '0')).strip() == '1'
 
 
 class StepTables(object):
@@ -345,12 +350,12 @@
         self._join()
         comm.finish(optimizer)
 
-    def _poe_forward(self, mus, lvs, mu, lv, z, kl):
+    def _poe_forward(self, mus, lvs, mu, lv, z, kl, rows=None):
         if self._draw_in_poe:
             K.poe_fwd_draw(mus, lvs, self.masks_dev, self.noise, self.seed, self.counter, 0, mu, lv, z, kl,
-                           self.model.POE_VARIANT)
-        else:
-            K.poe_fwd(mus, lvs, self.masks_dev, self.noise, mu, lv, z, kl, self.model.POE_VARIANT)
+                           self.model.POE_VARIANT, rows=rows)
+        else:
+            K.poe_fwd(mus, lvs, self.masks_dev, self.noise, mu, lv, z, kl, self.model.POE_VARIANT, rows=rows)
 
     def _side_launch_ok(self):
         return (self.dp_side_launch and self.side is not None and self._comm is not None
@@ -448,6 +453,7 @@
         self.masks_dev = torch.tensor(self.term_masks, dtype=torch.int32, device=dev)
         self.pair_dec = self._pairable_decoder_layers() if os.environ.get('MVAE_PAIR', '0') == '1' else 0
         self.pair_enc = self._pairable_encoder_layers() if os.environ.get('MVAE_PAIR_ENC', '0') == '1' else 0
+        self.label_table = label_table_switch() and not self.pair_enc and self._label_table_ok()
         self.split_dz = os.environ.get('MVAE_SPLIT_DZ', '1') != '0'
         self.counter_rides = os.environ.get('MVAE_COUNTER_RIDES', 'encoder')
         self.fuse_adam = (os.environ.get('MVAE_FUSE_ADAM', '0') == '1' and self.split_dz and not self.pair_dec)
@@ -489,6 +495,57 @@
         ok = (n >= 1 and len(head_i) == 1 and head_i[0].kind == 'lin' and head_i[0].act and head_i[0].drop == 0
               and len(head_l) == 1 and head_l[0].kind == 'emb')
         return n if ok else 0
+
+    def _label_table_ok(self):
+        if self.model.LABEL_KIND != 'class':
+            return False
+        plan = self.model.label_encoder.plan()
+        return ([op.kind for op in plan[:2]] == ['emb', 'lin'] and len(plan) == 3 and plan[2].kind in ('lin', 'lin2')
+                and plan[1].act and not plan[2].act and plan[2].drop == 0
+                and plan[1].drop == 0 and plan[0].mod.num_embeddings <= 16)
+
+    def _label_table_forward(self):
+        emb, fc2, heads_op = self.model.label_encoder.plan()
+        table = emb.mod.weight.detach()
+        C = table.shape[0]
+        w2, b2 = L._lin_weights(fc2)
+        w3, b3 = L._lin_weights(heads_op)
+        h1 = torch.empty_like(table)
+        p2 = torch.empty(C, w2.shape[0], dtype=torch.float32, device=self.dev)
+        h2 = torch.empty_like(p2)
+        heads = torch.empty(C, w3.shape[0], dtype=torch.float32, device=self.dev)
+        K.table_linear_fwd(table, w2.detach(), None if b2 is None else b2.detach(), pre=p2, act=h2, x_swish=True, x_act=h1)
+        K.table_linear_fwd(h2, w3.detach(), None if b3 is None else b3.detach(), pre=heads)
+        return heads, (table, h1, p2, h2)
+
+    def _label_table_backward(self, label, g_heads):
+        emb, fc2, heads_op = self.model.label_encoder.plan()
+        table, h1, p2, h2 = self._carry['tape_lbl_table']
+        C = table.shape[0]
+        w2, _ = L._lin_weights(fc2)
+        w3, _ = L._lin_weights(heads_op)
+        G = torch.empty(C, g_heads.shape[1], dtype=torch.float32, device=self.dev)
+        K.class_sum(label, g_heads, G)
+        dh2 = torch.empty_like(p2)
+        K.table_linear_dgrad(G, w3.detach(), dh2, pre_in=p2)
+        d_table, acc_t = L.grad_target(emb.mod.weight)
+        K.table_linear_dgrad(dh2, w2.detach(), d_table, pre_in=table, accumulate=acc_t)
+        dw3, db3, acc3 = L._lin_wgrad_targets(heads_op)
+        dw2, db2, acc2 = L._lin_wgrad_targets(fc2)
+        K.table_linear_wgrad([(G, h2, dw3, db3, acc3), (dh2, h1, dw2, db2, acc2)])
+        fusion = self._fusion
+        if fusion is not None and not (acc_t or acc3 or acc2):
+            done = [g for g in (d_table, dw3, db3, dw2, db2) if g is not None]
+            for g in done:
+                fusion.cover(g)
+            K.linear_wgrad_batched([(None, None, g.reshape(-1), None, False) for g in done], adam=fusion.struct)
+        self._carry['keep_lbl_table'] = (G, dh2)
+
+    def _label_rows(self, n_image_experts, label):
+        if not self.label_table:
+            return None
+        C = self.model.label_encoder.plan()[0].mod.num_embeddings
+        return [None] * n_image_experts + [(label, C)]
 
     def _pair_enc_now(self):
         return self.pair_enc and self.n_buckets != 3
@@ -695,7 +752,10 @@
 
         def encode_label(after=None):
             with self._branch(after):
-                heads, c['tape_lbl'] = L.forward_tape(m.label_encoder.plan(), lbl_in, bn_updates=n_up)
+                if self.label_table:
+                    heads, c['tape_lbl_table'] = self._label_table_forward()
+                else:
+                    heads, c['tape_lbl'] = L.forward_tape(m.label_encoder.plan(), lbl_in, bn_updates=n_up)
                 if self.counter_rides == 'encoder' or self.pair_dec:
                     self._early_counter()
             return heads
@@ -727,7 +787,10 @@
         lv = torch.empty_like(mu)
         z = torch.empty_like(mu)
         kl = torch.empty(T, B, dtype=torch.float32, device=self.dev)
-        self._poe_forward(mus, lvs, mu, lv, z, kl)
+        if self.label_table:
+            label = label.contiguous()
+        c['poe_rows'] = self._label_rows(len(img_experts), label)
+        self._poe_forward(mus, lvs, mu, lv, z, kl, rows=c['poe_rows'])
         self.last_latents = (mu, lv, z)
         i0, ni = self.img_terms
         l0, nl = self.lbl_terms
@@ -865,17 +928,17 @@
         if part in ('all', 'upper'):
             heads_img, heads_lbl = c['heads_img'], c['heads_lbl']
             g_heads_img = torch.empty_like(heads_img)
-            g_heads_lbl = torch.empty_like(heads_lbl)
+            g_heads_lbl = torch.empty(B, heads_lbl.shape[1], dtype=torch.float32, device=self.dev)
             g_list = ([g_heads_img[:B], g_heads_img[B:]] if self.has_dropout else [g_heads_img]) + [g_heads_lbl]
             if c.get('dz_split') is not None:
                 dza, sa, dzb, sb = c['dz_split']
                 K.poe_bwd_split(c['mus'], c['lvs'], self.masks_dev, self.noise, c['mu'], c['lv'], dza, sa, dzb, sb,
                                 self.coef[2], [gg[:, :D] for gg in g_list], [gg[:, D:] for gg in g_list],
-                                m.POE_VARIANT, dkl_per_term=True)
+                                m.POE_VARIANT, dkl_per_term=True, rows=c.get('poe_rows'))
             else:
                 K.poe_bwd(c['mus'], c['lvs'], self.masks_dev, self.noise, c['mu'], c['lv'], c['dz'], None, None,
                           self.coef[2], [gg[:, :D] for gg in g_list], [gg[:, D:] for gg in g_list], m.POE_VARIANT,
-                          dkl_per_term=True)
+                          dkl_per_term=True, rows=c.get('poe_rows'))
             c['keep_b'] = (g_heads_img, g_heads_lbl)
         if part == 'all' and 'enc_pair' in c:
             self._encoders_paired_bwd(*c['keep_b'])
@@ -888,7 +951,10 @@
 
             def label_encoder_backward(after=None):
                 with self._branch(after):
-                    L.backward_tape(m.label_encoder.plan(), c['tape_lbl'], g_heads_lbl, deferred=wl)
+                    if self.label_table:
+                        self._label_table_backward(c['poe_rows'][-1][0], g_heads_lbl)
+                    else:
+                        L.backward_tape(m.label_encoder.plan(), c['tape_lbl'], g_heads_lbl, deferred=wl)
                     if isinstance(wl, L.WgradBatch):
                         wl.flush()
             fork = self._fork_point()
@@ -938,7 +1004,10 @@
         cut = L.tail_cut(plan, m.arena_tail())
         if part == 'upper':
             with self._branch():
-                L.backward_tape(m.label_encoder.plan(), c['tape_lbl'], c['keep_b'][1])
+                if self.label_table:
+                    self._label_table_backward(c['poe_rows'][-1][0], c['keep_b'][1])
+                else:
+                    L.backward_tape(m.label_encoder.plan(), c['tape_lbl'], c['keep_b'][1])
             g = c['keep_b'][0]
             if self.has_dropout:
                 d_hd = L.backward_tape(self.head, c['tape_head'], g, need_input_grad=True)
diff --git a/multimodal-vae-public_amd/kernels.py b/multimodal-vae-public_amd/kernels.py
--- a/multimodal-vae-public_amd/kernels.py
+++ b/multimodal-vae-public_amd/kernels.py
@@ -522,6 +522,22 @@
     return ld
 
 
+def _expert_rows(rows, n_experts, B):
+    if len(rows) != n_experts:
+        raise RuntimeError('one row entry per expert')
+    r = _lib.ExpertRows()
+    for e, item in enumerate(rows):
+        if item is None:
+            continue
+        idx, n_rows = item
+        _need_gpu(idx)
+        if idx.dtype != torch.int64 or not idx.is_contiguous() or idx.numel() != B or int(n_rows) <= 0:
+            raise RuntimeError('an expert row index is a contiguous int64 [B] tensor with a positive row count')
+        r.idx[e] = idx.data_ptr()
+        r.rows[e] = int(n_rows)
+    return r
+
+
 _ALL_EXPERTS = {}
 
 
@@ -555,29 +571,43 @@
         pass
 
 
-def poe_fwd(mus, lvs, masks_dev, noise, mu, logvar, z, kl, variant):
+def poe_fwd(mus, lvs, masks_dev, noise, mu, logvar, z, kl, variant, rows=None):
     ld = _expert_ld(mus, lvs)
     _need_gpu(masks_dev, noise, mu, logvar, z, kl); _f32c(noise, mu, logvar, z, kl)
     T, B, D = mu.shape
     ex = _experts(mus, lvs)
     _check_no_prior_masks(masks_dev, variant, len(mus))
+    if rows is not None:
+        er = _expert_rows(rows, len(mus), B)
+        check(_lib.lib().mvae_poe_fwd_rows(ctypes.byref(ex), ctypes.byref(er), ld, len(mus), _ptr(masks_dev), T,
+                                           _ptr(noise), _ptr(mu), _ptr(logvar), _ptr(z), _ptr(kl), B, D,
+                                           _lib.POE_VARIANT[variant], _stream()), 'mvae_poe_fwd_rows')
+        return
     check(_lib.lib().mvae_poe_fwd(ctypes.byref(ex), ld, len(mus), _ptr(masks_dev), T, _ptr(noise), _ptr(mu),
                                   _ptr(logvar), _ptr(z), _ptr(kl), B, D, _lib.POE_VARIANT[variant],
                                   _stream()), 'mvae_poe_fwd')
 
 
-def poe_fwd_draw(mus, lvs, masks_dev, noise_out, seed, counter_dev, counter_offset, mu, logvar, z, kl, variant):
+def poe_fwd_draw(mus, lvs, masks_dev, noise_out, seed, counter_dev, counter_offset, mu, logvar, z, kl, variant,
+                 rows=None):
     ld = _expert_ld(mus, lvs)
     _need_gpu(masks_dev, noise_out, counter_dev, mu, logvar, z, kl); _f32c(noise_out, mu, logvar, z, kl)
     T, B, D = mu.shape
     ex = _experts(mus, lvs)
+    if rows is not None:
+        er = _expert_rows(rows, len(mus), B)
+        check(_lib.lib().mvae_poe_fwd_draw_rows(ctypes.byref(ex), ctypes.byref(er), ld, len(mus), _ptr(masks_dev), T,
+                                                _ptr(noise_out), seed, _ptr(counter_dev), int(counter_offset), _ptr(mu),
+                                                _ptr(logvar), _ptr(z), _ptr(kl), B, D, _lib.POE_VARIANT[variant],
+                                                _stream()), 'mvae_poe_fwd_draw_rows')
+        return
     check(_lib.lib().mvae_poe_fwd_draw(ctypes.byref(ex), ld, len(mus), _ptr(masks_dev), T, _ptr(noise_out), seed,
                                        _ptr(counter_dev), int(counter_offset), _ptr(mu), _ptr(logvar), _ptr(z),
                                        _ptr(kl), B, D, _lib.POE_VARIANT[variant], _stream()), 'mvae_poe_fwd_draw')
 
 
 def poe_bwd(mus, lvs, masks_dev, noise, mu, logvar, dz, dmu, dlogvar, dkl, g_mus, g_lvs, variant,
-            dkl_per_term=False):
+            dkl_per_term=False, rows=None):
     ld = _expert_ld(mus, lvs)
     ldg = _expert_ld(g_mus, g_lvs)
     _need_gpu(masks_dev, noise, mu, logvar, dz, dmu, dlogvar, dkl)
@@ -588,6 +618,13 @@
     for i, (m, v) in enumerate(zip(g_mus, g_lvs)):
         gr.dmu[i] = m.data_ptr()
         gr.dlogvar[i] = v.data_ptr()
+    if rows is not None:
+        er = _expert_rows(rows, len(mus), B)
+        check(_lib.lib().mvae_poe_bwd_rows(ctypes.byref(ex), ctypes.byref(er), ld, len(mus), _ptr(masks_dev), T,
+                                           _ptr(noise), _ptr(mu), _ptr(logvar), _ptr(dz), _ptr(dmu), _ptr(dlogvar),
+                                           _ptr(dkl), 1 if dkl_per_term else 0, ctypes.byref(gr), ldg, B, D,
+                                           _lib.POE_VARIANT[variant], _stream()), 'mvae_poe_bwd_rows')
+        return
     check(_lib.lib().mvae_poe_bwd(ctypes.byref(ex), ld, len(mus), _ptr(masks_dev), T, _ptr(noise), _ptr(mu),
                                   _ptr(logvar), _ptr(dz), _ptr(dmu), _ptr(dlogvar), _ptr(dkl),
                                   1 if dkl_per_term else 0, ctypes.byref(gr), ldg, B, D, _lib.POE_VARIANT[variant], _stream()),
@@ -595,7 +632,7 @@
 
 
 def poe_bwd_split(mus, lvs, masks_dev, noise, mu, logvar, dz_a, slots_a, dz_b, slots_b, dkl, g_mus, g_lvs, variant,
-                  dkl_per_term=False):
+                  dkl_per_term=False, rows=None):
     ld = _expert_ld(mus, lvs)
     ldg = _expert_ld(g_mus, g_lvs)
     _need_gpu(masks_dev, noise, mu, logvar, dz_a, dz_b, dkl)
@@ -613,10 +650,65 @@
         gr.dlogvar[i] = v.data_ptr()
     sa = (ctypes.c_int * T)(*[int(x) for x in slots_a])
     sb = (ctypes.c_int * T)(*[int(x) for x in slots_b])
+    if rows is not None:
+        er = _expert_rows(rows, len(mus), B)
+        check(_lib.lib().mvae_poe_bwd_split_rows(ctypes.byref(ex), ctypes.byref(er), ld, len(mus), _ptr(masks_dev), T,
+                                                 _ptr(noise), _ptr(mu), _ptr(logvar), _ptr(dz_a), sa, _ptr(dz_b), sb,
+                                                 _ptr(dkl), 1 if dkl_per_term else 0, ctypes.byref(gr), ldg, B, D,
+                                                 _lib.POE_VARIANT[variant], _stream()), 'mvae_poe_bwd_split_rows')
+        return
     check(_lib.lib().mvae_poe_bwd_split(ctypes.byref(ex), ld, len(mus), _ptr(masks_dev), T, _ptr(noise), _ptr(mu),
                                         _ptr(logvar), _ptr(dz_a), sa, _ptr(dz_b), sb, _ptr(dkl),
                                         1 if dkl_per_term else 0, ctypes.byref(gr), ldg, B, D,
                                         _lib.POE_VARIANT[variant], _stream()), 'mvae_poe_bwd_split')
+
+
+def class_sum(idx, g, out):
+    _need_gpu(idx, g, out); _f32c(out)
+    if idx.dtype != torch.int64 or not idx.is_contiguous() or g.dtype != torch.float32 or g.dim() != 2 or g.stride(1) != 1:
+        raise RuntimeError('class_sum: int64 contiguous index, fp32 [R, W] gradient with unit column stride')
+    R, W = g.shape
+    if idx.numel() != R or out.dim() != 2 or out.shape[1] != W:
+        raise RuntimeError('class_sum: shapes %s %s %s' % (tuple(idx.shape), tuple(g.shape), tuple(out.shape)))
+    check(_lib.lib().mvae_class_sum(_ptr(idx), _ptr(g), g.stride(0), _ptr(out), R, out.shape[0], W, _stream()),
+          'mvae_class_sum')
+
+
+def table_linear_fwd(x, w, bias, pre=None, act=None, x_swish=False, x_act=None):
+    _need_gpu(x, w, bias, pre, act, x_act); _f32c(x, w, bias, pre, act, x_act)
+    M, K = x.shape
+    N = w.shape[0]
+    for t in (pre, act):
+        if t is not None and tuple(t.shape) != (M, N):
+            raise RuntimeError('table_linear_fwd: output %s for M%d N%d' % (tuple(t.shape), M, N))
+    if w.shape[1] != K or (x_act is not None and x_act.shape != x.shape) or (bias is not None and bias.numel() != N):
+        raise RuntimeError('table_linear_fwd: shapes')
+    check(_lib.lib().mvae_table_linear_fwd(_ptr(x), 1 if x_swish else 0, _ptr(x_act), _ptr(w), _ptr(bias), _ptr(pre),
+                                           _ptr(act), M, N, K, _stream()), 'mvae_table_linear_fwd')
+
+
+def table_linear_dgrad(dy, w, dx, pre_in=None, accumulate=False):
+    _need_gpu(dy, w, dx, pre_in); _f32c(dy, w, dx, pre_in)
+    M, N = dy.shape
+    K = w.shape[1]
+    if w.shape[0] != N or tuple(dx.shape) != (M, K) or (pre_in is not None and tuple(pre_in.shape) != (M, K)):
+        raise RuntimeError('table_linear_dgrad: shapes')
+    check(_lib.lib().mvae_table_linear_dgrad(_ptr(dy), _ptr(w), _ptr(pre_in), _ptr(dx), M, N, K,
+                                             ACCUMULATE if accumulate else 0, _stream()), 'mvae_table_linear_dgrad')
+
+
+def table_linear_wgrad(items):
+    items = list(items)
+    arr = (_lib.WgradItem * len(items))()
+    for q, (dy, x, dw, db, acc) in enumerate(items):
+        _need_gpu(dy, x, dw, db); _f32c(dw, db)
+        M, N = dy.shape
+        if x.shape[0] != M or tuple(dw.shape) != (N, x.shape[1]) or dy.stride(1) != 1 or x.stride(1) != 1 \
+                or dy.dtype != torch.float32 or x.dtype != torch.float32:
+            raise RuntimeError('table wgrad item %d: shapes %s %s %s' % (q, tuple(dy.shape), tuple(x.shape), tuple(dw.shape)))
+        arr[q] = _lib.WgradItem(_ptr(dy), dy.stride(0), _ptr(x), x.stride(0), _ptr(dw), _ptr(db), M, N, x.shape[1],
+                                ACCUMULATE if acc else 0)
+    check(_lib.lib().mvae_table_linear_wgrad(arr, len(items), _stream()), 'mvae_table_linear_wgrad')
 
 
 def kl_rows_fwd(mu, logvar, kl):
diff --git a/multimodal-vae-public_amd/profiler.py b/multimodal-vae-public_amd/profiler.py
--- a/multimodal-vae-public_amd/profiler.py
+++ b/multimodal-vae-public_amd/profiler.py
@@ -96,7 +96,13 @@
     return 2.0 * x.numel() * w.shape[1] * 16, '%dx%dx%dx%d' % (B, w.shape[1], OH, OW)
 
 
+def _table_wgrad_cost(items, *a, **kw):
+    fl = sum(2.0 * dy.shape[0] * dy.shape[1] * x.shape[1] for dy, x, _, _, _ in items)
+    return fl, 'M%d %d layers' % (items[0][0].shape[0], len(items))
+
+
 GEMM_COSTS = {
+    'table_linear_fwd': _lin_cost('fwd'), 'table_linear_dgrad': _lin_cost('dgrad'), 'table_linear_wgrad': _table_wgrad_cost,
     'convT2d_fwd_stats': _convT_stats_cost,
     'linear_wgrad_batched': _wgrad_batched_cost,
     'linear_fwd_grouped': _lin_grouped_cost('fwd'), 'linear_dgrad_grouped': _lin_grouped_cost('dgrad'),
@@ -153,7 +159,7 @@
            'dropout_fanout_fwd', 'dropout_fanin_bwd', 'bce_elem_fwd', 'bce_elem_bwd', 'embedding_swish_fwd_grouped',
            'embedding_swish_bwd_grouped', 'block_gather', 'block_scatter_add', 'elbo_reduce', 'philox_fill',
            'adam_apply', 'sigmoid_fwd', 'affine_fwd', 'scatter_sums', 'poe_fwd_draw', 'poe_bwd_split', 'adam_apply_at',
-           'counter_add', 'conv_repack_batched', 'bn_stats_merge']
+           'counter_add', 'conv_repack_batched', 'bn_stats_merge', 'class_sum']
 
 
 class KernelProfile(object):
```

New measurement: 1.969 million images/sec (median of 3 runs). +1.0%, better.
